# pritykinlab/guidescan-cli

Hardware: AMD Instinct MI355X
Metric: guides/sec off-target enum, <=3 mismatches (higher is better)
Workload: dtype u32

## Files before the change

guidescan-cli_amd/api.py:

```python
from __future__ import annotations

import ctypes as C
import os
import subprocess
from pathlib import Path

import numpy as np

PKG = Path(__file__).resolve().parent
LIB_PATH = Path(os.environ.get("GS_LIB_PATH", str(PKG / "libgsamd.so")))

GS_FLAG_PAM_AT_START = 1
GS_FLAG_FAITHFUL_WALK = 2
GS_FLAG_COUNT_REQUESTS = 4
GS_FLAG_RAW_COUNTS = 8
GS_FLAG_NO_NEW_TABLES = 16


class GsError(RuntimeError):
    def __init__(self, status, msg):
        super().__init__(f"gs_status {status}: {msg}")
        self.status = status


# ... 151 lines not shown
    L.gs_decode_sequence_ex.restype = i32
    L.gs_decode_sequence_ex.argtypes = [vp, C.c_char_p]
    L.gs_enumerate_general.restype = i32
    L.gs_enumerate_general.argtypes = [vp, vp, u64, u32, vp, u32, C.c_char_p, u32, u32, u32, u32, u32,
                                       C.POINTER(vp)]
    L.gs_enumerate_general_pams.restype = i32
    L.gs_enumerate_general_pams.argtypes = [vp, vp, u64, u32, vp, u32, C.c_char_p, vp, u32, u32, u32, u32, u32,
                                            C.POINTER(vp)]
    L.gs_debug_general_last.restype = i32
    L.gs_debug_general_last.argtypes = [vp, C.POINTER(u64)]
    L.gs_debug_bulge_last.restype = i32
    L.gs_debug_bulge_last.argtypes = [vp, C.POINTER(u64)]
    L.gs_debug_bulge_seeds.restype = i32
    L.gs_debug_bulge_seeds.argtypes = [C.c_char_p, u32, u32, u32, u32, u32, u32, u32, u32, vp, u64, C.POINTER(u64)]
    L.gs_debug_bulge_verify.restype = i32
    L.gs_debug_bulge_verify.argtypes = [u32, vp, u64, C.c_char_p, u32, C.c_char_p, u32, C.c_char_p, vp, u32, u32, u32, u32,
                                        u32, u32, vp, u64, C.POINTER(u64)]
    L.gs_index_last_guide_flags.restype = i32
    L.gs_index_last_guide_flags.argtypes = [vp, C.POINTER(vp), C.POINTER(u64)]
    L.gs_format_guide_ex.restype = i32
    L.gs_format_guide_ex.argtypes = [C.POINTER(GsGenomeStructure), C.POINTER(GsKmer), vp, u64, u32, u32,
                                     C.c_int64, C.POINTER(vp), C.POINTER(C.c_size_t)]
    L.gs_score_device.restype = i32
    L.gs_score_device.argtypes = [vp, vp, u64, u32, u32, u32, C.c_int64, C.POINTER(GsGenomeStructure), vp, vp,
                                  vp, vp, vp]
    L.gs_score.restype = i32
    L.gs_score.argtypes = [vp, vp, u64, u32, u32, u32, C.c_int64, C.POINTER(GsGenomeStructure), vp, vp, vp, vp]
    L.gs_format_device.restype = i32
    L.gs_format_device.argtypes = [vp, C.POINTER(GsGenomeStructure), vp, u64, u32, vp, u32, vp, vp, vp, vp, vp, vp, vp, u32, u32,
                                   C.c_int64, vp, C.POINTER(vp), C.POINTER(u64)]
    L.gs_enumerate_text.restype = i32
    L.gs_enumerate_text.argtypes = [vp, vp, u64, u32, vp, u32, C.c_char_p, u32, u32, u32, C.c_int64,
                                    C.POINTER(GsGenomeStructure), vp, vp, vp, vp, C.POINTER(vp), C.POINTER(u64),
                                    C.POINTER(GsResultView)]
    L.gs_index_last_text_offsets.restype = i32
    L.gs_index_last_text_offsets.argtypes = [vp, vp, u64]
    L.gs_kmers_generate.restype = i32
    L.gs_kmers_generate.argtypes = [i32, vp, u64, i32, C.c_char_p, u32, u32, vp, C.POINTER(vp)]
    L.gs_kmers_get.restype = i32
    L.gs_kmers_get.argtypes = [vp, i32, C.POINTER(u64), C.POINTER(vp), C.POINTER(vp), C.POINTER(vp),
                               C.POINTER(vp)]
    L.gs_kmers_free.argtypes = [vp]
    L.gs_format_device_ids.restype = i32
    L.gs_format_device_ids.argtypes = L.gs_format_device.argtypes
    L.gs_enumerate_text_device.restype = i32
    L.gs_enumerate_text_device.argtypes = [vp, vp, u64, u32, vp, u32, C.c_char_p, u32, u32, u32, C.c_int64,
                                           C.POINTER(GsGenomeStructure), vp, vp, vp, vp, C.POINTER(vp), C.POINTER(u64),
                                           C.POINTER(GsResultView), vp]
    L.gs_kmers_encode_ids.restype = i32
    L.gs_kmers_encode_ids.argtypes = [vp, C.c_char_p, C.c_char_p, vp]
    L.gs_kmers_get_ids.restype = i32
    L.gs_kmers_get_ids.argtypes = [vp, i32, C.POINTER(vp), C.POINTER(vp), C.POINTER(vp)]
    L.gs_kmers_csv.restype = i32
    L.gs_kmers_csv.argtypes = [vp, C.c_char_p, C.c_char_p, C.POINTER(vp), C.POINTER(u64)]
    L.gs_kmers_concat.restype = i32
    L.gs_kmers_concat.argtypes = [vp, u32, C.POINTER(vp)]
    L.gs_decoder_open.restype = i32
    L.gs_decoder_open.argtypes = [i32, vp, u64, C.POINTER(GsGenomeStructure), vp, vp, C.POINTER(vp)]
    L.gs_decoder_close.argtypes = [vp]
    L.gs_decode_records.restype = i32
    L.gs_decode_records.argtypes = [vp, C.POINTER(GsDecodeBatch), u32, u64, C.POINTER(vp), C.POINTER(u64), C.POINTER(u64)]
    L.gs_decode_records_device.restype = i32
    L.gs_decode_records_device.argtypes = L.gs_decode_records.argtypes
    L.gs_decode_sam.restype = i32
    L.gs_decode_sam.argtypes = [vp, vp, u64, u32, u64, C.POINTER(vp), C.POINTER(u64), C.POINTER(u64)]
    L.gs_debug_repr_doubles.restype = i32
    L.gs_debug_repr_doubles.argtypes = [vp, u64, vp]
    L.gs_bgzf_compress_device.restype = i32
    L.gs_bgzf_compress_device.argtypes = [vp, vp, u64, vp, C.POINTER(vp), C.POINTER(u64)]
    L.gs_bgzf_compress.restype = i32
    L.gs_bgzf_compress.argtypes = [vp, vp, u64, C.POINTER(vp), C.POINTER(u64)]
    L.gs_bgzf_inflate.restype = i32
    L.gs_bgzf_inflate.argtypes = [i32, vp, u64, C.POINTER(vp), C.POINTER(u64)]
    L.gs_bgzf_inflate_device.restype = i32
    L.gs_bgzf_inflate_device.argtypes = [vp, vp, u64, u64, C.POINTER(vp), C.POINTER(u64), C.POINTER(u64)]
    L.gs_bgzf_inflate_base.restype = i32
    L.gs_bgzf_inflate_base.argtypes = [vp, u64, u64]
    L.gs_debug_inflate_member.restype = i32
    L.gs_debug_inflate_member.argtypes = [vp, u64, vp, u64, C.POINTER(u64), C.POINTER(u32)]
    L.gs_debug_bgzf_members.restype = i32
    L.gs_debug_bgzf_members.argtypes = [vp, u64, vp, vp, u64, C.POINTER(u64), C.POINTER(u32)]
    L.gs_decode_bam.restype = i32
    L.gs_decode_bam.argtypes = [vp, vp, u64, u64, vp, u32, u32, u64, C.POINTER(vp), C.POINTER(u64), C.POINTER(u64), C.POINTER(u64)]
    L.gs_decode_bam_device.restype = i32
    L.gs_decode_bam_device.argtypes = L.gs_decode_bam.argtypes
    L.gs_debug_decode_bam_last.restype = i32
    L.gs_debug_decode_bam_last.argtypes = [vp, vp, vp]
    L.gs_debug_huffman_lengths.restype = i32
    L.gs_debug_huffman_lengths.argtypes = [vp, u32, u32, vp]
    L.gs_debug_sp_float.restype = C.c_float
    L.gs_debug_sp_float.argtypes = [u32]
    L.gs_debug_decode_tables.restype = i32
    L.gs_debug_decode_tables.argtypes = [vp, vp]
    L.gs_fasta_parse.restype = i32
    L.gs_fasta_parse.argtypes = [i32, vp, u64, u32, C.POINTER(vp)]
    L.gs_fasta_parse_file.restype = i32
    L.gs_fasta_parse_file.argtypes = [i32, C.c_char_p, u32, C.POINTER(vp)]
    L.gs_fasta_parse_device.restype = i32
    L.gs_fasta_parse_device.argtypes = [i32, vp, u64, u32, vp, C.POINTER(vp)]
    L.gs_fasta_info.restype = i32
    L.gs_fasta_info.argtypes = [vp, C.POINTER(u64), C.POINTER(u64), C.POINTER(u64)]
    L.gs_fasta_records.restype = i32
    L.gs_fasta_records.argtypes = [vp, vp, vp, vp, vp, vp, vp, vp]
    L.gs_fasta_text.restype = i32
    L.gs_fasta_text.argtypes = [vp, i32, C.POINTER(vp)]
    L.gs_fasta_free.restype = None
    L.gs_fasta_free.argtypes = [vp]
    L.gs_decoder_open_fasta.restype = i32
    L.gs_decoder_open_fasta.argtypes = [i32, vp, C.POINTER(GsGenomeStructure), C.POINTER(vp)]
    L.gs_debug_fasta_tile_bytes.restype = u64
    L.gs_debug_fasta_tile_bytes.argtypes = []
    L.gs_debug_fasta_host.restype = i32
    L.gs_debug_fasta_host.argtypes = [vp, u64, u32, u64, C.POINTER(vp)]
    L.gs_debug_fasta_chunk_bytes.restype = u64
    L.gs_debug_fasta_chunk_bytes.argtypes = [u64]
    L.gs_debug_fasta_ms.restype = i32
    L.gs_debug_fasta_ms.argtypes = [vp, vp]
    L.gs_kmers_parse.restype = i32
    L.gs_kmers_parse.argtypes = [i32, vp, u64, C.POINTER(vp), C.POINTER(GsKmersReport)]
    L.gs_kmers_parse_file.restype = i32
    L.gs_kmers_parse_file.argtypes = [i32, C.c_char_p, C.POINTER(vp), C.POINTER(GsKmersReport)]
    L.gs_kmers_parse_device.restype = i32
    L.gs_kmers_parse_device.argtypes = [i32, vp, u64, vp, C.POINTER(vp), C.POINTER(GsKmersReport)]
    L.gs_debug_kmers_tile_bytes.restype = u64
    L.gs_debug_kmers_tile_bytes.argtypes = []
    L.gs_debug_kmers_chunk_bytes.restype = u64
    L.gs_debug_kmers_chunk_bytes.argtypes = [u64]
    L.gs_debug_kmers_host.restype = i32
    L.gs_debug_kmers_host.argtypes = [vp, u64, u64, C.POINTER(vp), C.POINTER(GsKmersReport)]
    L.gs_status_string.restype = C.c_char_p
    L.gs_status_string.argtypes = [i32]
    L.gs_version.restype = C.c_char_p
    _lib = L
    return L


EXPORTS = ["gs_index_build", "gs_index_build_with_sa", "gs_index_open_sdsl", "gs_index_close",
           "gs_index_genome_length", "gs_index_device_bytes", "gs_enumerate", "gs_enumerate_device",
           "gs_result_get", "gs_result_free", "gs_decode_sequence", "gs_rank_bwt4", "gs_resolve",
           "gs_index_meta", "gs_index_copy_sa", "gs_calculate_cfd", "gs_status_string", "gs_version",
           "gs_format_guide", "gs_format_header", "gs_free", "gs_sdsl_extract_text",
           "gs_enumerate_bulges", "gs_result_ex_get", "gs_result_ex_free", "gs_decode_sequence_ex",
           "gs_format_guide_ex", "gs_score_device", "gs_score", "gs_kmers_generate", "gs_kmers_get",
           "gs_kmers_free", "gs_format_guide_scored", "gs_index_verify_sa", "gs_index_last_counters", "gs_index_last_launch", "gs_enumerate_general",
           "gs_index_last_guide_flags", "gs_enumerate_general_pams", "gs_index_save_sa", "gs_index_open_sa", "gs_format_guides_scored", "gs_result_ex_raw_hits",
           "gs_debug_seed_recipes", "gs_debug_choose_thresholds", "gs_debug_tile_plan", "gs_debug_search_form", "gs_debug_guide_descriptor", "gs_debug_general_last", "gs_index_lock", "gs_index_unlock",
           "gs_index_last_sharing", "gs_index_set_option", "gs_index_get_option", "gs_index_prepare",
           "gs_index_save_sdsl", "gs_debug_sdsl_sections", "gs_debug_sdsl_export_scratch",
           "gs_format_device", "gs_enumerate_text", "gs_index_last_text_offsets",
           "gs_format_device_ids", "gs_enumerate_text_device", "gs_kmers_encode_ids", "gs_kmers_get_ids", "gs_kmers_csv",
           "gs_kmers_concat", "gs_decoder_open", "gs_decoder_close", "gs_decode_records", "gs_decode_records_device",
           "gs_decode_sam", "gs_debug_repr_doubles", "gs_debug_decode_tables",
           "gs_index_last_spaced", "gs_debug_seed_recipes_a8", "gs_debug_spaced_rows",
           "gs_debug_bulge_last", "gs_debug_bulge_seeds", "gs_debug_bulge_verify",
           "gs_bgzf_compress_device", "gs_bgzf_compress", "gs_debug_huffman_lengths", "gs_debug_sp_float",
           "gs_bgzf_inflate", "gs_bgzf_inflate_device", "gs_bgzf_inflate_base", "gs_debug_inflate_member", "gs_debug_bgzf_members",
           "gs_decode_bam", "gs_decode_bam_device", "gs_debug_decode_bam_last",
           "gs_fasta_parse", "gs_fasta_parse_file", "gs_fasta_parse_device", "gs_fasta_info", "gs_fasta_records", "gs_fasta_text",
           "gs_fasta_free", "gs_decoder_open_fasta", "gs_debug_fasta_tile_bytes", "gs_debug_fasta_host",
           "gs_debug_fasta_chunk_bytes", "gs_debug_fasta_ms",
           "gs_kmers_parse", "gs_kmers_parse_file", "gs_kmers_parse_device", "gs_debug_kmers_tile_bytes",
           "gs_debug_kmers_chunk_bytes", "gs_debug_kmers_host"]


def _check(rc):
    if rc != 0:
        raise GsError(rc, lib().gs_status_string(rc).decode())


BULGE_SEED_DTYPE = np.dtype([("index", "<u4"), ("state", "<u4"), ("seq", "S32")])
BULGE_MATCH_DTYPE = np.dtype([("state", "<u4"), ("consumed", "<u4"), ("seq", "S32")])


def bulge_state(word):
    word = int(word)
    return dict(t=word & 63, mismatches=(word >> 6) & 7, dna_bulges=(word >> 9) & 7, rna_bulges=(word >> 12) & 7,
                bulge_state=(word >> 15) & 3, bulge_size=(word >> 17) & 1, seq_len=(word >> 18) & 63)


def bulge_seeds(guide, k, mismatches=0, rna_bulges=0, dna_bulges=0, start=False, prefix_len=0, prefix=0, count_only=False):
    g = guide.encode() if isinstance(guide, str) else bytes(guide)
    flags = GS_FLAG_PAM_AT_START if start else 0
    n = C.c_uint64(0)
    _check(lib().gs_debug_bulge_seeds(g, len(g), k, mismatches, rna_bulges, dna_bulges, flags, prefix_len, prefix, None, 0,
                                      C.byref(n)))
    if count_only:
        return int(n.value)
    out = np.zeros(n.value, dtype=BULGE_SEED_DTYPE)
    _check(lib().gs_debug_bulge_seeds(g, len(g), k, mismatches, rna_bulges, dna_bulges, flags, prefix_len, prefix,
                                      out.ctypes.data, out.size, C.byref(n)))
    assert n.value == out.size
    return out


def bulge_verify(state, seq, ctx_nibbles, guide, pam, k, alt_pams=(), mismatches=0, rna_bulges=0, dna_bulges=0, start=False):
    g = guide.encode() if isinstance(guide, str) else bytes(guide)
    p = pam.encode() if isinstance(pam, str) else bytes(pam)
    sq = np.frombuffer(bytes(seq).ljust(32, b"\0"), dtype=np.uint8).copy()
    alts = "".join(alt_pams).encode()
    lens = np.array([len(a) for a in alt_pams], dtype=np.uint32)
    flags = GS_FLAG_PAM_AT_START if start else 0

    def call(out, cap, n):
        _check(lib().gs_debug_bulge_verify(int(state), sq.ctypes.data, int(ctx_nibbles), g, len(g), p if p else None, len(p),
                                           alts if alt_pams else None, lens.ctypes.data if alt_pams else None,
                                           len(alt_pams), k, mismatches, rna_bulges, dna_bulges, flags, out, cap, C.byref(n)))
    n = C.c_uint64(0)
    call(None, 0, n)
    out = np.zeros(n.value, dtype=BULGE_MATCH_DTYPE)
    call(out.ctypes.data, out.size, n)
    assert n.value == out.size
    return out


def seed_recipes(k, L, P, m, n_x, astar=None, deep=False):
    L_ = lib()
    L_.gs_debug_seed_recipes.restype = C.c_int
    L_.gs_debug_seed_recipes.argtypes = [C.c_uint32] * 5 + [C.c_void_p, C.c_uint32, C.c_void_p, C.c_uint64, C.c_void_p]
    a = None
    if astar is not None:
        a = (C.c_uint32 * 8)(*(list(astar) + [15] * 8)[:8])
    counts = (C.c_uint64 * 3)()
    _check(L_.gs_debug_seed_recipes(k, L, P, m, n_x, a, 1 if deep else 0, None, 0, counts))
    n = sum(counts)
    out = np.zeros(n, dtype=np.uint64)
    _check(L_.gs_debug_seed_recipes(k, L, P, m, n_x, a, 1 if deep else 0, out.ctypes.data, n, counts))
    c0, c1 = int(counts[0]), int(counts[1])
    return out[:c0], out[c0:c0 + c1], out[c0 + c1:]


def seed_recipes_a8(k, m, n_x, astar, trimmed=False):
    L_ = lib()
    L_.gs_debug_seed_recipes_a8.restype = C.c_int
    L_.gs_debug_seed_recipes_a8.argtypes = [C.c_uint32] * 3 + [C.c_void_p, C.c_uint32, C.c_void_p, C.c_uint64, C.c_void_p]
    a = (C.c_uint32 * 8)(*(list(astar) + [15] * 8)[:8])
    n = C.c_uint64()
    _check(L_.gs_debug_seed_recipes_a8(k, m, n_x, a, 1 if trimmed else 0, None, 0, C.byref(n)))
    out = np.zeros(int(n.value), dtype=np.uint64)
    _check(L_.gs_debug_seed_recipes_a8(k, m, n_x, a, 1 if trimmed else 0, out.ctypes.data, out.shape[0], C.byref(n)))
    return out


def guide_descriptor(q: int, pams, L: int, P: int, k: int, x_len: int, codes=(0, 0xFFFFFFFF), n_pt: int = 1, valid: bool = True):
    L_ = lib()
    L_.gs_debug_guide_descriptor.restype = C.c_int
    L_.gs_debug_guide_descriptor.argtypes = [C.c_uint64, C.c_void_p, C.c_uint32, C.c_uint32, C.c_uint32, C.c_uint32, C.c_uint32,
                                             C.c_uint32, C.c_uint32, C.c_void_p, C.c_void_p]
    pam = (C.c_uint32 * 4)(*(list(pams) + [0] * (4 - len(pams))))
    code = (C.c_uint32 * 2)(*codes)
    out = (C.c_uint32 * 16)()
    _check(L_.gs_debug_guide_descriptor(q, pam, len(pams), 1 if valid else 0, L, P, k, x_len, n_pt, code, out))
    names = ("q_lo", "q_hi", "pam0", "pam1", "pam2", "pam3", "meta", "pidx0", "pidxg", "qrem_b", "bsel_z", "bsel_w", "qhot",
             "key_a", "key_b", "guide")
    return dict(zip(names, (int(x) for x in out)))


def choose_thresholds(m, n_x, n_o, n_r, pam_expansions=4.0, verify_a=1.5, verify_b=1.9):
    L_ = lib()
    L_.gs_debug_choose_thresholds.restype = None
    L_.gs_debug_choose_thresholds.argtypes = [C.c_uint32] * 4 + [C.c_double] * 3 + [C.c_void_p]
    out = (C.c_uint32 * 8)()
    L_.gs_debug_choose_thresholds(m, n_x, n_o, n_r, pam_expansions, verify_a, verify_b, out)
    return list(out)


def tile_plan(records):
    L_ = lib()
    L_.gs_debug_tile_plan.restype = None
    L_.gs_debug_tile_plan.argtypes = [C.c_uint32, C.c_void_p]
    out = (C.c_uint32 * 5)()
    L_.gs_debug_tile_plan(records, out)
    return dict(buckets=out[0], slot=out[1], per=out[2], wave_tile=out[3], max_buckets=out[4])


SEARCH_FORM_IN = ("items", "cus", "share_min", "backoff", "main", "walk", "one_chunk", "counting", "spec", "m", "est_heavy",
                  "est_max", "last_hpass", "last_items", "heavy", "split_share", "split_from", "seed_form")


def search_form(**kw):
    L_ = lib()
    L_.gs_debug_search_form.restype = None
    L_.gs_debug_search_form.argtypes = [C.c_void_p, C.c_void_p]
    vals = dict(heavy=-1, split_share=-1, seed_form=-1, split_from=1 << 19)
    vals.update(kw)
    unknown = set(vals) - set(SEARCH_FORM_IN)
    if unknown:
        raise TypeError(f"unknown inputs {sorted(unknown)}")
    inp = (C.c_int64 * len(SEARCH_FORM_IN))(*[int(vals.get(k, 0)) for k in SEARCH_FORM_IN])
    out = (C.c_uint32 * 6)()
    L_.gs_debug_search_form(inp, out)
    return dict(zip(("estimate", "thresh", "heavy", "split", "seed_form", "form"), (int(x) for x in out)))


def make_genome_structure(names, lengths):
    arr_n = (C.c_char_p * len(names))(*[n.encode() for n in names])
    arr_l = (C.c_uint64 * len(lengths))(*lengths)
    g = GsGenomeStructure(arr_n, arr_l, len(names))
    g._keep = (arr_n, arr_l)
    return g


def format_header(gs, sam=False, complete=True) -> str:
    out, n = C.c_void_p(), C.c_size_t()
    flags = (GS_TEXT_SAM if sam else 0) | (GS_TEXT_COMPLETE if complete else 0)
    _check(lib().gs_format_header(C.byref(gs), flags, C.byref(out), C.byref(n)))
    s = C.string_at(out, n.value).decode()
    lib().gs_free(out)
    return s


def format_guide(gs, gid, sequence, pam, sense_positive, hits, mismatches, sam=False, complete=True,
                 start=False, max_off_targets=-1, specificity=None) -> str:
    hits = np.ascontiguousarray(hits, dtype=HIT_DTYPE)
    k = GsKmer(gid.encode(), sequence.encode(), pam.encode(), int(sense_positive))
    out, n = C.c_void_p(), C.c_size_t()
    flags = ((GS_TEXT_SAM if sam else 0) | (GS_TEXT_COMPLETE if complete else 0) |
             (GS_FLAG_PAM_AT_START if start else 0))
    if specificity is None:
        _check(lib().gs_format_guide(C.byref(gs), C.byref(k), hits.ctypes.data, hits.shape[0], mismatches,
                                     flags, max_off_targets, C.byref(out), C.byref(n)))
    else:
        _check(lib().gs_format_guide_scored(C.byref(gs), C.byref(k), hits.ctypes.data, hits.shape[0],
                                            mismatches, flags, max_off_targets, float(specificity),
                                            C.byref(out), C.byref(n)))
    s = C.string_at(out, n.value).decode()
    lib().gs_free(out)
    return s


def format_guides(gs, ids, seqs, pams, senses_positive, offsets, hits, specificity, mismatches, sam=False,
                  complete=True, start=False, max_off_targets=-1, skip=None) -> bytes:
    n = len(ids)
    arr = (GsKmer * n)(*[GsKmer(ids[i].encode(), seqs[i].encode(), pams[i].encode(), int(senses_positive[i]))
                         for i in range(n)])
    offsets = np.ascontiguousarray(offsets, dtype=np.uint64)
    hits = np.ascontiguousarray(hits, dtype=HIT_DTYPE)
    spec = np.ascontiguousarray(specificity, dtype=np.float32)
    sk = None if skip is None else np.ascontiguousarray(skip, dtype=np.uint8)
    out, ln = C.c_void_p(), C.c_size_t()
    flags = ((GS_TEXT_SAM if sam else 0) | (GS_TEXT_COMPLETE if complete else 0) |
             (GS_FLAG_PAM_AT_START if start else 0))
    _check(lib().gs_format_guides_scored(C.byref(gs), arr, n, offsets.ctypes.data,
                                         hits.ctypes.data if hits.shape[0] else None, spec.ctypes.data,
                                         sk.ctypes.data if sk is not None else None, mismatches, flags,
                                         max_off_targets, C.byref(out), C.byref(ln)))
    s = C.string_at(out, ln.value)
    lib().gs_free(out)
    return s


def _id_blob(ids):
    enc = [i.encode() if isinstance(i, str) else bytes(i) for i in ids]
    off = np.zeros(len(enc) + 1, dtype=np.uint64)
    if enc:
        off[1:] = np.cumsum([len(e) for e in enc], dtype=np.uint64)
    return b"".join(enc), off


def _bytes_or_none(x, n):
    if x is None:
        return None
    a = np.ascontiguousarray(np.asarray(x) != 0, dtype=np.uint8)
    if a.shape != (n,):
        raise ValueError("one entry per guide")
    return a


class DeviceKmers:

    def __init__(self, handle, k, P):
        self._h, self.k, self.P = handle, k, P
        n, a, b, c, d = C.c_uint64(), C.c_void_p(), C.c_void_p(), C.c_void_p(), C.c_void_p()
        _check(lib().gs_kmers_get(handle, 1, C.byref(n), C.byref(a), C.byref(b), C.byref(c), C.byref(d)))
        self.n = int(n.value)
        self.seqs_ptr, self.pams_ptr, self.pos_ptr, self.sense_ptr = a.value, b.value, c.value, d.value

    @classmethod
    def parse(cls, src, device=0):
        h, rep = C.c_void_p(), GsKmersReport()
        if isinstance(src, (str, os.PathLike)):
            rc = lib().gs_kmers_parse_file(device, os.fsencode(src), C.byref(h), C.byref(rep))
        else:
            raw = np.frombuffer(src, dtype=np.uint8) if isinstance(src, (bytes, bytearray, memoryview)) else np.ascontiguousarray(src, dtype=np.uint8)
            rc = lib().gs_kmers_parse(device, raw.ctypes.data if raw.size else None, raw.size, C.byref(h), C.byref(rep))
        return cls._parsed(rc, h, rep)

    @classmethod
    def parse_device(cls, d_raw_ptr, length, device=0, stream=None):
        h, rep = C.c_void_p(), GsKmersReport()
        rc = lib().gs_kmers_parse_device(device, d_raw_ptr if length else None, length, stream, C.byref(h), C.byref(rep))
        return cls._parsed(rc, h, rep)

    @classmethod
# ... 872 lines not shown
```

guidescan-cli_amd/csrc/gs_common.h:

```cpp
#ifndef GS_COMMON_H
#define GS_COMMON_H

#include <hip/hip_runtime.h>
#include <stdint.h>
#include <string.h>

#include <array>
#include <atomic>
#include <map>
#include <mutex>
#include <string>
#include <vector>

#include "guidescan_amd.h"

#define ARENA_SHIFT 10u
#define ARENA_CHUNK (1u << ARENA_SHIFT)

#define GS_BLOCK_ROWS 128u
#define GS_BLOCK_SHIFT 7u

#define GS_PT_BIG 63u
struct gs_pairtab_dev {
  const uint2 *tab;
  const uint2 *rot;
  const uint16_t *c16;
  const uint32_t *ctx;
  const uint32_t *rowid;
  uint32_t rot_first;
  uint32_t code;
  const uint4 *deep;
  const uint32_t *sp_off;
  const uint2 *sp_rows;
  uint32_t sp_rem;
};
struct gs_strand_dev {
  const uint4 *blocks;
  const uint32_t *sa;
  const uint32_t *run_start;
  const uint32_t *run_cum;
  uint32_t n;
  uint32_t nruns;
  uint32_t C[4];
  uint32_t CN;
  uint32_t has_n;
  const uint4 *ptab;
  uint32_t mask_off;
  const uint4 *ptab_rot;
  uint32_t rot_first;
  const uint32_t *ctx;
  const uint16_t *ctx16;
  const uint32_t *isa;
  const uint32_t *exc_row;
  const uint64_t *exc_sym;
  uint32_t n_exc;
  const uint32_t *xr_start;
  const uint32_t *xr_cum;
  const uint2 *xr_seg;
  const uint32_t *C256;
};

struct gs_strand {
  gs_strand_dev d{};
  void *blocks = nullptr, *sa = nullptr, *run_start = nullptr, *run_cum = nullptr, *ptab = nullptr, *ctx = nullptr, *ctx16 = nullptr, *ptab_rot = nullptr, *isa = nullptr, *exc_row = nullptr, *exc_sym = nullptr, *xr_start = nullptr, *xr_cum = nullptr, *xr_seg = nullptr, *C256 = nullptr;
  bool has_sym[256] = {false};
  uint32_t rot_plan_first = 31, rot_plan_n = 0, rot_k = 0;
  uint64_t n = 0;
  uint64_t C_acgtn[5] = {0, 0, 0, 0, 0};
  uint64_t bytes = 0;
};

#define GS_NRUN_FLANK 40
struct gs_nrun {
  uint64_t start, len;
  uint8_t left[GS_NRUN_FLANK];
  uint8_t right[GS_NRUN_FLANK];
};

struct gs_buffer {
  void *p = nullptr;
  size_t cap = 0;
};

struct gs_pairtab_host {
  bool valid = false;
  uint32_t v_rem = 0, code = 0, rot_first = 31;
  gs_pairtab_dev d[2]{};
  void *mem[2][8] = {{nullptr}, {nullptr}};
  bool deep = false;
  uint32_t deep_P = 0, deep_kb = 0;
  bool spaced = false;
  uint32_t sp_x = 0, sp_g = 0;
  uint64_t sp_bytes = 0, sp_rows[2] = {0, 0};
  uint64_t n_slots[2] = {0, 0};
  double sp_build_ms = 0;
  uint64_t bytes = 0, used = 0;
};

struct gs_recipe_set {
  gs_buffer buf;
  uint64_t key[2] = {0, 0};
  bool valid = false;
  uint32_t n_full = 0, n_a = 0, n_b = 0, n_a8 = 0;
  uint32_t n_a8s = 0;
  uint32_t a_rot_first = 31;
};

struct gs_index {
  std::map<std::string, std::string> opts;
  mutable std::recursive_mutex mtx;
  int device = 0;
  uint64_t genome_length = 0;
  gs_strand strand[2];
  gs_buffer w_guides, w_slots, w_counts, w_nmatch, w_nhits, w_offsets, w_hits, w_misc, w_blocksums,
      w_grec, w_flags, w_raw, w_ovf_list, w_grec2, w_slots2, w_counts2, w_nmatch2, w_nhits2, w_h_off, w_h_tmp,
      w_b_src, w_b_cnt, w_b_prefix, w_b_recs, w_b_w0, w_b_w0b, w_b_idx, w_b_idxb, w_b_keep, w_b_keeps,
      w_b_rows, w_b_rowss, w_b_redo_pos, w_b_s, w_b_tab,
      w_score, w_score_io, w_score_tmp,
      w_arena, w_arena_meta, w_nchunk,
      w_shq, w_sh_meta,
      w_cls, w_desc, w_sched,
      w_t_plan, w_t_tiles, w_t_buckets, w_t_chunkof, w_t_big, w_t_rel, w_t_tab, w_t_excl, w_t_spill, w_b_redo_pos2,
      w_text_in, w_text_tmp, w_text_hex, w_text, w_text_spec, w_text_goff ,
      w_bgzf_in, w_bgzf_tmp, w_bgzf_out;
  uint32_t share_backoff = 0;
  bool share_timed_out = false;
  uint32_t opt_share_min = 512, opt_share_max = 2048;
  unsigned long long last_share[8] = {0, 0, 0, 0, 0, 0, 0, 0};
  uint64_t shq_packages = 16384;
  uint64_t arena_chunks = 4096;
  struct seen_t {
    double mean = -1, max = 0;
    uint64_t hpass = 0, items = 0;
    uint64_t key = 0;
  };
  std::array<seen_t, 8> seen;
  bool last_raw_valid = false;
  uint64_t last_unsupported = 0;
  hipEvent_t ev[4] = {nullptr, nullptr, nullptr, nullptr};
  hipEvent_t ev_tile = nullptr;
  hipStream_t st_help = nullptr;
  hipEvent_t ev_help[2] = {nullptr, nullptr};
  uint32_t *h_pin = nullptr;
  std::atomic<uint64_t> lock_owner{0};
  uint32_t lock_depth = 0;
  uint32_t pt_k = 0;
  unsigned long long last_counters[16] = {0};
  unsigned long long last_launch[8] = {0, 0, 0, 0, 0, 0, 0, 0};
  unsigned long long last_general[8] = {0, 0, 0, 0, 0, 0, 0, 0};
  unsigned long long last_bulge[8] = {0, 0, 0, 0, 0, 0, 0, 0};
  std::vector<gs_nrun> nruns_text;
  gs_buffer w_cand;
  uint64_t cand_key = ~0ull;
  uint32_t cand_n[2] = {0, 0};
  size_t cand_bidx[2] = {0, 0};
  gs_recipe_set rec[2];
  uint32_t rec_cur = 0;
  uint32_t pairtab_nofit = 0;
  gs_pairtab_host pairtab[2];
  bool pairtab_off = false;
  bool spaced_off = false;
  unsigned long long last_spaced[4] = {0, 0, 0, 0};
  bool rot_off = false;
  uint32_t dbg_nomem = 0;
  bool tile_order_off = false;
  uint64_t tile_order_off_key = 0;
  uint64_t tx_n = 0;
  bool big_long_runs = false;
};

gs_status gs_pairtab_ensure(gs_index *ix, uint32_t slot, uint32_t v_rem, uint32_t code, uint32_t rot_first, double share,
                            hipStream_t st);
gs_status gs_pairtab_ensure_deep(gs_index *ix, uint32_t slot, uint32_t P, uint32_t kb, hipStream_t st);
void gs_pairtab_free(gs_index *ix, uint32_t slot);
gs_status gs_pairtab_ensure_spaced(gs_index *ix, uint32_t slot, uint32_t x_len, uint32_t g, hipStream_t st);
bool gs_pairtab_free_spaced(gs_index *ix, uint32_t slot);
gs_status gs_strand_rot_ensure(gs_index *ix, hipStream_t st);
bool gs_strand_rot_release(gs_index *ix);

struct gs_tileorder_in {
  uint32_t n_set;
  const uint32_t *list;
  const uint32_t *redo_pos;
  const uint32_t *counts;
  const uint32_t *cls;
  const uint4 *slots;
  uint32_t cap;
  const uint4 *arena;
  const uint32_t *chunk_item, *chunk_seq;
  uint32_t n_used;
  uint32_t *nhits;
  const uint64_t *offsets;
  gs_hit *hits;
  uint32_t L, P, m, v_rem;
};
struct gs_tileorder_state {
  uint32_t n_it = 0, n_tiles = 0, n_btiles = 0, n_chunks = 0, n_big = 0, n_deal = 0;
  uint32_t spill_units = 0, spill_cap = 0;
  uint32_t n_excl = 0;
  uint64_t n_records = 0;
};
bool gs_tileorder_fits(uint32_t L, uint32_t P, uint32_t m);
gs_status gs_tileorder_plan(gs_index *ix, const gs_tileorder_in &in, hipStream_t st, gs_tileorder_state &S, bool *usable);
gs_status gs_tileorder_run(gs_index *ix, const gs_tileorder_in &in, gs_tileorder_state &S, hipStream_t st, uint32_t *violations);

#define GS_HANDLE_LOCK(ix)                               \
  std::unique_lock<std::recursive_mutex> handle_lock__; \
  if (ix) handle_lock__ = std::unique_lock<std::recursive_mutex>((ix)->mtx)

#define GS_HIP(expr)                                                              \
  do {                                                                            \
    hipError_t e__ = (expr);                                                      \
    if (e__ != hipSuccess) {                                                      \
      gs_set_error(std::string(#expr) + ": " + hipGetErrorString(e__));           \
      return GS_ERR_DEVICE;                                                       \
    }                                                                             \
  } while (0)

void gs_set_error(const std::string &s);
const char *gs_opt(const gs_index *ix, const char *key);
void gs_opts_from_env(gs_index *ix);
extern std::atomic<int> gs_debug_any;
gs_status gs_reserve(gs_buffer &b, size_t bytes);
gs_status gs_text_to_host(const void *d_text, uint64_t tl, char **text);
size_t gs_buffer_free(gs_buffer &b);

gs_status gs_device_suffix_array(const uint8_t *d_text, uint64_t n, uint32_t *d_sa, hipStream_t st);
gs_status gs_strand_from_device(const uint8_t *d_text, uint32_t *d_sa_owned, uint64_t n,
                                gs_strand *out, hipStream_t st);
void gs_strand_free(gs_strand *s);
gs_status gs_count_bad_sa_rows(const uint32_t *d_sa, uint64_t n, hipStream_t st, uint64_t *bad);

gs_status gs_sdsl_read(const char *path, std::vector<uint8_t> &bwt, std::vector<uint64_t> &sa_samples,
                       uint64_t C256[257]);

gs_status gs_device_suffix_array_discarding(const uint8_t *d_text, uint64_t n, uint32_t *d_sa, hipStream_t st, bool debug);

static inline __host__ __device__ uint32_t gs_lane_group(uint32_t n_guides) {
  uint32_t g = 64;
  while (g > 1 && (n_guides + g - 1) / g < 8192u) g >>= 1;
  return g;
}

#endif
```

guidescan-cli_amd/csrc/gs_enumerate.hip:

```cpp
#include "gs_kernels.h"

__global__ void k_estimate_heavy(const gs_guide_rec *guides, uint32_t n, const uint4 *ptab0, const uint4 *ptab1, uint32_t k,
                                 uint32_t thresh, uint32_t *out);

#include <cmath>

static uint64_t shape_key(uint32_t L, uint32_t P, uint32_t n_alt, uint32_t flags) {
  return ((uint64_t)L << 32) | ((uint64_t)P << 16) | (n_alt << 8) | (flags & GS_FLAG_PAM_AT_START);
}

struct switches {
  bool debug, no_form_estimate, no_bidir, no_pairtab, no_deep, no_spec, no_cand_buckets, no_tile_order, no_arena;
  bool dbg_share_timeout;
  uint32_t share_min, share_max;
  uint32_t max_pt;
  bool has_deep_symbols;
  uint32_t deep_symbols;
  uint32_t n_astar, astar[8];
  double pairtab_reserve;
  bool has_index_budget;
  double index_budget;
  uint32_t cand_from;
  bool has_arena_chunks;
  uint64_t arena_chunks;
// ... 601 lines not shown
}

struct search_pass {
  const gs_guide_rec *guides;
  uint32_t ng;
  uint4 *slots;
  uint32_t *counts;
  uint32_t cap;
  const uint64_t *slot_off;
  bool with_arena;
};
static void fill_search_args(const batch &b, const search_pass &p, gs_search_args &sa) {
  const gs_index *ix = b.ix;
  memset(&sa, 0, sizeof(sa));
  sa.sd[0] = ix->strand[0].d;
  sa.sd[1] = ix->strand[1].d;
  sa.slots = p.slots;
  sa.slot_off = p.slot_off;
  sa.counts = p.counts;
  sa.work = b.d_work;
  sa.stats = b.d_stats;
  sa.n_items = 2 * p.ng;
  sa.L = b.L;
  sa.P = b.P;
  sa.m = b.m;
  sa.cap = p.cap;
  if (p.with_arena) {
    sa.arena = (uint4 *)ix->w_arena.p;
    sa.arena_next = b.d_work + WK_ARENA_NEXT;
    sa.chunk_item = (uint32_t *)ix->w_arena_meta.p;
    sa.chunk_seq = sa.chunk_item + b.arena_chunks;
    sa.nchunk = (uint2 *)ix->w_nchunk.p;
    sa.cls = (uint32_t *)ix->w_cls.p;
    sa.arena_chunks = b.arena_chunks;
    sa.chunk_fill = sa.chunk_item + 2 * (size_t)b.arena_chunks;
  }
  const uint64_t waves = (uint64_t)b.cus * 32u;
  uint64_t take = (2ull * p.ng) / (waves * 64u);
  take = take < 1 ? 1 : take > 4 ? 4 : take;
  if (b.sw.search_take) take = b.sw.search_take;
  sa.take = (uint32_t)take;
  sa.max_iter = b.sw.max_iter;
  sa.err = b.d_work + WK_SEARCH_ERR;
  sa.hpass = b.d_work + WK_HPASS;
  sa.v_max = b.sw.v_max;
  sa.dbg_skip = b.sw.dbg_skip;
  sa.cnt_shift = b.sw.cnt_shift;
  sa.astar = 0xFFFFFFFFu;
  if (b.table_seeding) {
    sa.pt_k = ix->pt_k;
    sa.v_rem = b.v_rem;
    sa.x_len = b.x_len;
    sa.bdeep = b.deep ? 1u : 0u;
    const gs_recipe_set &R = ix->rec[ix->rec_cur];
    sa.rec_full = (const uint2 *)R.buf.p;
    sa.n_rec_full = R.n_full;
    if (b.bidir) {
      sa.bidir = 1;
      sa.astar = b.astar_packed;
      sa.rec_a = sa.rec_full + R.n_full;
      sa.n_rec_a = R.n_a;
      sa.rec_b = sa.rec_a + R.n_a;
      sa.n_rec_b = R.n_b;
      sa.rec_a8 = sa.rec_b + R.n_b;
      sa.n_rec_a8 = R.n_a8;
      sa.n_pt = b.n_pt;
      for (uint32_t i = 0; i < b.n_pt; i++) {
        sa.pt[i][0] = ix->pairtab[b.pt_slot[i]].d[0];
        sa.pt[i][1] = ix->pairtab[b.pt_slot[i]].d[1];
      }
      for (uint32_t s = 0; s < 2; s++) {
        sa.cand[s] = b.d_cand[s];
        sa.n_cand[s] = b.n_cand[s];
        sa.cand_off[s] = b.d_cand_off[s];
        sa.cand_ids[s] = b.d_cand_ids[s];
      }
    }
  }
  if (sa.dbg_skip & 4u) sa.n_rec_full = sa.n_rec_a = sa.n_rec_b = sa.n_rec_a8 = 0u;
}

static void launch_helpers(const gs_search_args &sh, uint32_t sh_grid, bool spec, hipStream_t hs) {
  if (spec)
    hipLaunchKernelGGL(k_search_heavy_pd, dim3(sh_grid), dim3(WAVE * SEARCH_WAVES), 0, hs, sh);
  else
    hipLaunchKernelGGL(k_search_heavy, dim3(sh_grid), dim3(WAVE * SEARCH_WAVES), 0, hs, sh);
}
static bool helper_stream(gs_index *ix) {
  if (ix->st_help) return true;
  int lo = 0, hi = 0;
  hipStream_t hs = nullptr;
  bool ok = hipDeviceGetStreamPriorityRange(&lo, &hi) == hipSuccess && hipStreamCreateWithPriority(&hs, hipStreamNonBlocking, lo) == hipSuccess;
  for (hipEvent_t &e : ix->ev_help) ok = ok && hipEventCreateWithFlags(&e, hipEventDisableTiming) == hipSuccess;
  if (ok) {
    ix->st_help = hs;
    return true;
  }
  (void)hipGetLastError();
  if (hs) (void)hipStreamDestroy(hs);
  for (hipEvent_t &e : ix->ev_help) {
    if (e) (void)hipEventDestroy(e);
    e = nullptr;
  }
  return false;
}
struct search_launch {
  bool walk, spec;
  uint32_t grid, seed_grid, heavy_per_cu;
  form_out f;
  gs_search_args sh_args;
  uint32_t sh_grid = 0;
};
static gs_status launch_search(batch &b, const search_pass &p, gs_search_args &sa, search_launch &k) {
  gs_index *ix = b.ix;
  hipStream_t st = b.st;
  const dim3 blk(WAVE * SEARCH_WAVES);
  for (uint32_t c = 0; c < b.n_chunks; c++) {
    sa.guides = p.guides + (size_t)c * p.ng;
    sa.append = c ? 1u : 0u;
    if (c) GS_HIP(hipMemsetAsync(b.d_work + WK_ITEMS, 0, 4, st));
    if (k.walk)
      hipLaunchKernelGGL(k_search_walk, dim3(k.grid), blk, 0, st, sa);
    else if (k.spec && b.count_req && !k.f.seed_form)
      hipLaunchKernelGGL(k_search_count_pd, dim3(k.grid), blk, 0, st, sa);
    else if (k.f.split && sa.shq != nullptr) {
      k.sh_args = sa;
      k.sh_args.helper_only = 1u;
      k.sh_args.work = b.d_work + WK_HELPER_ITEMS;
      k.sh_grid = (uint32_t)b.cus * k.heavy_per_cu;
      const bool side = k.f.split == 2u && helper_stream(ix);
      if (side) {
        GS_HIP(hipEventRecord(ix->ev_help[0], st));
        GS_HIP(hipStreamWaitEvent(ix->st_help, ix->ev_help[0], 0));
      }
      if (k.f.split == 3u) launch_helpers(k.sh_args, k.sh_grid, k.spec, st);
      if (k.spec)
        hipLaunchKernelGGL(k_search_pub_pd, dim3(k.grid), blk, 0, st, sa);
      else
        hipLaunchKernelGGL(k_search_pub, dim3(k.grid), blk, 0, st, sa);
      if (k.f.split != 3u) launch_helpers(k.sh_args, k.sh_grid, k.spec, side ? ix->st_help : st);
      if (side) {
        GS_HIP(hipEventRecord(ix->ev_help[1], ix->st_help));
        GS_HIP(hipStreamWaitEvent(st, ix->ev_help[1], 0));
      }
    } else if (k.spec && sa.shq != nullptr)
      hipLaunchKernelGGL(k_search_heavy_pd, dim3(k.grid), blk, 0, st, sa);
    else if (sa.shq != nullptr)
      hipLaunchKernelGGL(k_search_heavy, dim3(k.grid), blk, 0, st, sa);
    else if (k.f.seed_form) {
      gs_search_args sb;
      gs_status r2 = gs_seed_describe(ix, sa, p.ng, k.f.seed_form >= 2u && p.ng >= b.sw.seed_sort_from, st, &sb);
      sb.seed_opt = b.sw.seed_opt;
      sb.take = b.sw.seed_take;
      if (r2 == GS_OK) r2 = gs_seed_launch(sb, k.seed_grid, b.count_req, st);
      if (r2 != GS_OK) return r2;
    } else if (k.spec)
      hipLaunchKernelGGL(k_search_fast_pd, dim3(k.grid), blk, 0, st, sa);
    else if (b.count_req)
      hipLaunchKernelGGL(k_search_count, dim3(k.grid), blk, 0, st, sa);
    else
      hipLaunchKernelGGL(k_search_fast, dim3(k.grid), blk, 0, st, sa);
  }
  return GS_OK;
}
static gs_status share_fix(batch &b, const search_pass &p, const gs_search_args &sa, gs_misc_readback &rb) {
  gs_index *ix = b.ix;
  hipStream_t st = b.st;
  gs_share_args fa;
  memset(&fa, 0, sizeof(fa));
  fa.ctl = sa.shq_ctl;
  fa.sh_list = sa.sh_list;
  fa.sh_acc = sa.sh_acc;
  fa.counts = p.counts;
  fa.nchunk = sa.nchunk;
  fa.cls = sa.cls;
  fa.chunk_item = sa.chunk_item;
  fa.chunk_seq = sa.chunk_seq;
  fa.chunk_fill = sa.chunk_fill;
  fa.arena_next = b.d_work + WK_ARENA_NEXT;
  fa.slots = p.slots;
  fa.arena = sa.arena;
  fa.dbase = sa.sh_acc + 16 * (size_t)sa.sh_max;
  fa.dir = sa.chunk_item + 3 * (size_t)b.arena_chunks;
  fa.stats = b.d_stats;
  fa.sh_max = sa.sh_max;
  fa.cap = p.cap;
  fa.arena_chunks = b.arena_chunks;
  const uint32_t n_sh = (uint32_t)ix->last_share[0];
  hipLaunchKernelGGL(k_share_scan, dim3(1), dim3(1024), 0, st, fa);
  hipLaunchKernelGGL(k_share_dir, dim3((b.arena_chunks + 255) / 256), dim3(256), 0, st, fa);
  hipLaunchKernelGGL((k_share_fix<SH_SMALLSEG>), dim3(n_sh), dim3(256), 0, st, fa);
  hipLaunchKernelGGL((k_share_fix<SH_MAXSEG>), dim3(std::min<uint32_t>(n_sh, (uint32_t)b.cus * 3u)), dim3(256), 0, st, fa);
  GS_HIP(hipEventRecord(ix->ev[2], st));
  GS_HIP(hipMemcpyAsync(&rb, b.d_stats, sizeof(rb), hipMemcpyDeviceToHost, st));
  GS_HIP(hipStreamSynchronize(st));
  GS_HIP(hipGetLastError());
  return GS_OK;
}
static gs_status reserve_share_queue(batch &b, const search_pass &p, gs_search_args &sa, uint32_t grid) {
  gs_index *ix = b.ix;
  uint64_t qcap = b.sw.share_queue ? b.sw.share_queue : ix->shq_packages;
  if (qcap > (1ull << 20)) qcap = 1ull << 20;
  const uint32_t sh_max = std::min<uint32_t>(2 * p.ng, 1u << 18);
  const size_t meta = 512 + 4 * (size_t)qcap + 4 * (size_t)sh_max + 64 * (size_t)sh_max;
  if (gs_reserve(ix->w_shq, 16 * (size_t)SHQ_PKG * qcap) != GS_OK || gs_reserve(ix->w_sh_meta, meta + 4 * ((size_t)sh_max + 2)) != GS_OK) {
    (void)hipGetLastError();
    return GS_OK;
  }
  uint32_t *d_shctl = (uint32_t *)ix->w_sh_meta.p;
  sa.shq = (uint4 *)ix->w_shq.p;
  sa.shq_ctl = d_shctl;
  sa.shq_ready = d_shctl + 128;
  sa.sh_list = sa.shq_ready + qcap;
  sa.sh_acc = sa.sh_list + sh_max;
  sa.shq_cap = (uint32_t)qcap;
  sa.sh_max = sh_max;
  sa.share_min = b.sw.share_min;
  sa.share_max = std::max(128u, b.sw.share_max);
  sa.n_waves = grid * SEARCH_WAVES;
  sa.sh_prof = b.sw.debug ? 1u : 0u;
  GS_HIP(hipMemsetAsync(d_shctl, 0, meta, b.st));
  if (sa.sh_prof) GS_HIP(hipMemsetAsync(d_shctl + 104, 0xFF, 8, b.st));
  return GS_OK;
}
static gs_status pick_form(batch &b, const search_pass &p, bool walk, bool spec, form_out &f) {
  gs_index *ix = b.ix;
  const gs_index::seen_t &seen = ix->seen[b.m < 8 ? b.m : 0];
  const bool seen_last = b.m < 8 && seen.key == shape_key(b.L, b.P, b.n_alt, b.flags) && seen.hpass != 0;
  form_in fi;
  fi.items = 2 * p.ng;
  fi.cus = (uint32_t)b.cus;
  fi.share_min = b.sw.share_min;
  fi.backoff = ix->share_backoff;
  fi.main = p.with_arena;
  fi.walk = walk;
  fi.one_chunk = b.n_chunks == 1;
  fi.counting = b.count_req;
  fi.spec = spec;
  fi.m = b.m;
  fi.est[0] = fi.est[1] = 0;
  fi.last_hpass = seen_last ? seen.hpass : 0;
  fi.last_items = seen_last ? seen.items : 0;
  fi.heavy = b.sw.heavy;
  fi.split_share = b.sw.split_share;
  fi.seed_form = b.sw.seed_form;
  fi.split_from = b.sw.split_from;
  if (p.with_arena && ix->share_backoff != 0) ix->share_backoff--;
  f = choose_form(fi);
  if (f.want_estimate && !b.sw.no_form_estimate) {
    if (b.pre_est_ran && p.with_arena) {
      fi.est[0] = b.pre_est[0];
      fi.est[1] = b.pre_est[1];
    } else {
      const gs_status er = gs_estimate_heavy(ix, p.guides, p.ng, f.est_thresh, b.d_work + WK_SCRATCH2, b.st, fi.est);
      if (er != GS_OK) return er;
    }
    if (b.sw.debug) fprintf(stderr, "[gs] form estimate: %u guides with a heavy k-mer of their own, the largest interval %u rows\n", fi.est[0], fi.est[1]);
    f = choose_form(fi);
  }
  ix->last_share[7] = fi.est[0];
  return GS_OK;
}
static gs_status run_search(batch &b, const search_pass &p, unsigned long long h_stats[2]) {
  gs_index *ix = b.ix;
  hipStream_t st = b.st;
  GS_HIP(hipMemsetAsync(ix->w_misc.p, 0, 16, st));
  GS_HIP(hipMemsetAsync(b.d_stats + ST_ARENA_FAIL, 0, 8, st));
  GS_HIP(hipMemsetAsync(b.d_work + WK_ITEMS, 0, 4, st));
  GS_HIP(hipMemsetAsync(b.d_work + WK_SEARCH_ERR, 0, 4, st));
  GS_HIP(hipMemsetAsync(b.d_work + WK_HPASS, 0, 4, st));
  GS_HIP(hipMemsetAsync(b.d_work + WK_HELPER_ITEMS, 0x80, 4, st));
  if (p.with_arena) {
    GS_HIP(hipMemsetAsync(b.d_work + WK_ARENA_NEXT, 0, 4, st));
    GS_HIP(hipMemsetAsync((uint32_t *)ix->w_arena_meta.p + b.arena_chunks, 0xFF, 4 * (size_t)b.arena_chunks, st));
    GS_HIP(hipMemsetAsync(ix->w_arena_meta.p, 0, 4 * (size_t)b.arena_chunks, st));
    for (int i = 0; i < 7; i++) ix->last_share[i] = 0;
  }
  gs_search_args sa;
  fill_search_args(b, p, sa);
  search_launch k;
  k.walk = sa.pt_k == 0 || sa.v_rem == 0;
  const size_t lds_wg = sizeof(uint4) * (k.walk ? WAVE_LDS_ENTRIES : WAVE_LDS_FAST) * SEARCH_WAVES;
  uint32_t per_cu = (uint32_t)(160u * 1024u / lds_wg);
  k.spec = !k.walk && sa.bidir && sa.bdeep && b.n_pt != 0 && b.n_pt == b.n_codes && b.h_pairs[16] == 0 && !b.sw.no_spec;
  sa.share_min = b.sw.share_min ? b.sw.share_min : 0xFFFFFFFFu;
  gs_status rc;
  if ((rc = pick_form(b, p, k.walk, k.spec, k.f)) != GS_OK) return rc;
  const bool sharing = k.f.heavy || k.f.split;
  const uint32_t weu = k.walk ? GS_WAVES_EU : k.f.heavy ? GS_WAVES_EU_HEAVY : k.spec ? GS_WAVES_EU_PD : GS_WAVES_EU_FAST;
  if (per_cu > weu) per_cu = weu;
  k.heavy_per_cu = std::min<uint32_t>((uint32_t)(160u * 1024u / lds_wg), GS_WAVES_EU_HEAVY);
  if (sharing) {
    int occ = 0;
    hipError_t oe = k.spec ? hipOccupancyMaxActiveBlocksPerMultiprocessor(&occ, k_search_heavy_pd, WAVE * SEARCH_WAVES, 0)
                           : hipOccupancyMaxActiveBlocksPerMultiprocessor(&occ, k_search_heavy, WAVE * SEARCH_WAVES, 0);
    if (oe != hipSuccess) (void)hipGetLastError();
    if (oe == hipSuccess && occ > 0 && (uint32_t)occ < k.heavy_per_cu) k.heavy_per_cu = (uint32_t)occ;
    if (k.f.heavy && per_cu > k.heavy_per_cu) per_cu = k.heavy_per_cu;
  }
  k.grid = (uint32_t)b.cus * per_cu;
  const uint32_t need = (2 * p.ng + SEARCH_WAVES - 1) / SEARCH_WAVES;
  if (k.grid > need) k.grid = need;
  if (b.sw.debug) {
    int occ = 0;
    (void)hipOccupancyMaxActiveBlocksPerMultiprocessor(&occ, k.walk ? k_search_walk : k_search_fast, WAVE * SEARCH_WAVES, 0);
    fprintf(stderr, "[gs] k_search (%s): grid %u x %u threads, LDS %zu B per workgroup, %d workgroups per CU resident\n",
            k.walk ? "walk" : "table", k.grid, WAVE * SEARCH_WAVES, lds_wg, occ);
  }
  if (sharing && (rc = reserve_share_queue(b, p, sa, k.grid)) != GS_OK) return rc;
  const uint32_t *d_shctl = sa.shq_ctl;
  k.seed_grid = 0;
  if (k.f.seed_form) {
    const size_t lds_seed = sizeof(uint4) * (VQ_CAP + 32 + 24 + 6) * SEARCH_WAVES;
    k.seed_grid = (uint32_t)b.cus * std::min<uint32_t>((uint32_t)(160u * 1024u / lds_seed), GS_WAVES_EU_SEED);
    if (k.seed_grid > need) k.seed_grid = need;
  }
  if (p.with_arena) ix->last_share[6] = sharing && d_shctl == nullptr ? 0u : k.f.form;
  if (p.with_arena) {
    const bool seed_launches = k.f.seed_form != 0u && !k.walk && sa.shq == nullptr;
    const unsigned long long ll[8] = {k.walk ? 1u : 0u, k.spec ? 1u : 0u, sa.bdeep, sa.take, seed_launches ? b.sw.seed_take : 0u, sa.n_pt, sa.x_len,
                                      ix->strand[0].ptab_rot ? ix->strand[0].rot_plan_n : 0u};
    memcpy(ix->last_launch, ll, sizeof(ll));
  }
  bool spaced = b.spaced_wanted && k.f.seed_form != 0u && !k.walk && sa.shq == nullptr;
  if (spaced) {
    const bool frozen = (b.flags & GS_FLAG_NO_NEW_TABLES) != 0;
    for (uint32_t i = 0; i < b.n_pt; i++) {
      if (!frozen && !ix->spaced_off && (rc = gs_pairtab_ensure_spaced(ix, b.pt_slot[i], b.x_len, b.L - ix->pt_k, st)) != GS_OK) return rc;
      const gs_pairtab_host &pt = ix->pairtab[b.pt_slot[i]];
      spaced = spaced && pt.spaced && pt.sp_x == b.x_len && pt.sp_g == b.L - ix->pt_k;
      sa.pt[i][0] = pt.d[0];
      sa.pt[i][1] = pt.d[1];
    }
  }
  if (spaced) {
    const gs_recipe_set &R = ix->rec[ix->rec_cur];
    sa.spaced = 1u;
    sa.spaced_ctr = b.d_work + WK_SPACED;
    sa.rec_a8 = sa.rec_a8 + R.n_a8;
    sa.n_rec_a8 = (sa.dbg_skip & 4u) ? 0u : R.n_a8s;
  }
  GS_HIP(hipEventRecord(ix->ev[1], st));
  if ((rc = launch_search(b, p, sa, k)) != GS_OK) return rc;
  GS_HIP(hipEventRecord(ix->ev[2], st));
  gs_misc_readback rb;
  uint32_t h_ctl[128] = {0};
  GS_HIP(hipMemcpyAsync(&rb, b.d_stats, sizeof(rb), hipMemcpyDeviceToHost, st));
  if (d_shctl) GS_HIP(hipMemcpyAsync(h_ctl, d_shctl, sizeof(h_ctl), hipMemcpyDeviceToHost, st));
  GS_HIP(hipStreamSynchronize(st));
  GS_HIP(hipGetLastError());
  if (d_shctl && k.f.split && k.sh_grid != 0u && h_ctl[32] < std::min(h_ctl[0], sa.shq_cap) && rb.work[WK_SEARCH_ERR] == 0u) {
    launch_helpers(k.sh_args, k.sh_grid, k.spec, st);
    GS_HIP(hipEventRecord(ix->ev[2], st));
    GS_HIP(hipMemcpyAsync(&rb, b.d_stats, sizeof(rb), hipMemcpyDeviceToHost, st));
    GS_HIP(hipMemcpyAsync(h_ctl, d_shctl, sizeof(h_ctl), hipMemcpyDeviceToHost, st));
    GS_HIP(hipStreamSynchronize(st));
    GS_HIP(hipGetLastError());
    ix->last_share[5]++;
  }
  if (d_shctl && sa.sh_prof) {
    const unsigned long long *pr = (const unsigned long long *)(h_ctl + 104);
    const double us = 0.01, nw = (double)sa.n_waves;
    fprintf(stderr, "[gs] heavy launch: %u waves; the last wave left its items after %.0f us, the last exit after %.0f us; per wave: items %.0f us, "
            "helper episodes %.0f us (%.1f episodes), waiting for a package %.0f us; shared items %u, packages %u (queue %u)\n",
            sa.n_waves, us * (double)(pr[1] - pr[0]), us * (double)(pr[2] - pr[0]), us * (double)pr[3] / nw, us * (double)pr[4] / nw,
            (double)pr[6] / nw, us * (double)pr[5] / nw, h_ctl[96], h_ctl[0], sa.shq_cap);
  }
  if (d_shctl) {
    ix->last_share[0] = std::min(h_ctl[96], sa.sh_max);
    ix->last_share[1] = h_ctl[0];
    ix->last_share[2] = sa.shq_cap;
    ix->last_share[3] = h_ctl[32];
    if (!b.sw.share_queue && (uint64_t)h_ctl[0] + h_ctl[0] / 4 + 64 > ix->shq_packages) ix->shq_packages = (uint64_t)h_ctl[0] + h_ctl[0] / 4 + 64;
    if (h_ctl[96] != 0u && rb.work[WK_SEARCH_ERR] == 0u && (rc = share_fix(b, p, sa, rb)) != GS_OK) return rc;
  }
  h_stats[0] = rb.stats[0];
  h_stats[1] = rb.stats[1];
  if (p.with_arena) b.arena_fail = rb.stats[ST_ARENA_FAIL];
  if (p.with_arena) b.arena_raw = rb.work[WK_ARENA_NEXT];
  if (p.with_arena && b.m < 8) {
    ix->seen[b.m].hpass = rb.work[WK_HPASS];
    ix->seen[b.m].items = 2 * (uint64_t)p.ng;
  }
  if (sa.shq != nullptr && b.sw.dbg_share_timeout) rb.work[WK_SEARCH_ERR] |= 2u;
  if (rb.work[WK_SEARCH_ERR] != 0u) {
    if ((rb.work[WK_SEARCH_ERR] & 2u) != 0u && sa.shq != nullptr) {
      ix->share_timed_out = true;
      gs_set_error("internal: a wave gave up waiting for a shared verification pass (the launch was not resident as a whole)");
      return GS_ERR_DEVICE;
    }
    gs_set_error("internal: an item of the search passed its iteration bound (GS_SEARCH_MAX_ITER)");
    return GS_ERR_DEVICE;
  }
  float ms = 0.f;
  hipEventElapsedTime(&ms, ix->ev[1], ix->ev[2]);
  b.ms_search += ms;
  return GS_OK;
}

static gs_status run_order(const batch &b, uint4 *slots, const uint32_t *counts, uint32_t *nmatch, uint32_t *nhits, uint32_t ng,
                           uint32_t cap_, uint32_t max_item) {
  gs_order_args oa;
  oa.slots = slots;
  oa.counts = counts;
  oa.nmatch = nmatch;
  oa.nhits = nhits;
  oa.stats = b.d_stats;
  oa.n = ng;
  oa.cap = cap_;
  if (cap_ > 128) {
    uint32_t nmax = 256;
    while (nmax < 2u * max_item && nmax < 2u * cap_) nmax <<= 1;
    const size_t lds = sizeof(uint4) * (size_t)nmax;
    if (lds > 64 * 1024)
      GS_HIP(hipFuncSetAttribute((const void *)k_order_wg, hipFuncAttributeMaxDynamicSharedMemorySize, (int)lds));
    uint32_t grid = ng;
    const uint32_t gmax = (uint32_t)b.cus * (uint32_t)(lds > 80 * 1024 ? 1 : lds > 40 * 1024 ? 3 : 6);
    if (grid > gmax) grid = gmax;
    if (grid == 0) grid = 1;
    hipLaunchKernelGGL(k_order_wg, dim3(grid), dim3(256), lds, b.st, oa, nmax);
    return GS_OK;
  }
  const uint32_t ow = ORDER_WAVES;
  const size_t lds = sizeof(uint4) * (2 * (size_t)cap_ + ORDER_SMALL) * ow;
  const uint32_t gsz = gs_lane_group(ng);
  uint32_t grid = ((ng + gsz - 1) / gsz + ow - 1) / ow;
  const uint32_t gmax = (uint32_t)b.cus * 16u;
  if (grid > gmax) grid = gmax;
  if (grid == 0) grid = 1;
  hipLaunchKernelGGL(k_order, dim3(grid), dim3(WAVE * ow), lds, b.st, oa);
  return GS_OK;
}
static void run_locate(const batch &b, const uint4 *matches, const uint32_t *nmatch, const uint32_t *gmap, uint32_t ng, uint32_t cap_) {
  const gs_index *ix = b.ix;
  gs_locate_args la;
  la.sd[0] = ix->strand[0].d;
  la.sd[1] = ix->strand[1].d;
  la.matches = matches;
  la.nmatch = nmatch;
  la.offsets = (const uint64_t *)ix->w_offsets.p;
  la.gmap = gmap;
  la.hits = (gs_hit *)ix->w_hits.p;
  la.genome_length = ix->genome_length;
  la.n = ng;
  la.cap = cap_;
  la.v_rem = b.v_rem;
  const size_t lds = sizeof(uint32_t) * (2 * (size_t)cap_ + 1);
  const uint32_t gsz = gs_lane_group(ng);
  hipLaunchKernelGGL(k_locate, dim3((ng + gsz - 1) / gsz), dim3(WAVE), lds, b.st, la);
}

static gs_status main_pass(batch &b) {
  gs_index *ix = b.ix;
  hipStream_t st = b.st;
  gs_status rc;
  if ((rc = gs_reserve(ix->w_slots, sizeof(uint4) * (size_t)b.cap * 2 * b.n)) != GS_OK) return rc;
  const search_pass p = {(const gs_guide_rec *)ix->w_grec.p, b.n32, (uint4 *)ix->w_slots.p, (uint32_t *)ix->w_counts.p, b.cap,
                         nullptr, b.arena_chunks != 0};
  if ((rc = run_search(b, p, b.h_stats)) != GS_OK) return rc;
  if (b.arena_chunks == 0 || b.arena_fail == 0 || b.sw.has_arena_chunks || b.n_chunks != 1) return GS_OK;
  uint32_t *d_need = b.d_work + WK_SCRATCH2, h_need = 0;
  GS_HIP(hipMemsetAsync(d_need, 0, 4, st));
  hipLaunchKernelGGL(k_need_chunks, dim3(std::min<uint32_t>((2 * b.n32 + 255) / 256, 1024u)), dim3(256), 0, st,
                     (const uint32_t *)ix->w_counts.p, 2 * b.n32, b.cap, d_need);
  GS_HIP(hipMemcpyAsync(&h_need, d_need, 4, hipMemcpyDeviceToHost, st));
  GS_HIP(hipStreamSynchronize(st));
// ... 605 lines not shown
```

guidescan-cli_amd/csrc/gs_index.hip:

```cpp
#include "gs_common.h"
#include "gs_scratch.h"

#include <rocprim/rocprim.hpp>

#include <algorithm>
#include <functional>
#include <system_error>
#include <thread>
#include <cstdlib>
#include <cstring>

__device__ __forceinline__ uint32_t sym_class(uint8_t c) {
  switch (c) {
    case 'A': return 0;
    case 'C': return 1;
    case 'G': return 2;
    case 'T': return 3;
    case 'N': return 4;
    default: return 5;
  }
}
__device__ __forceinline__ uint8_t bwt_at(const uint8_t *text, const uint32_t *sa, uint64_t n,
                                          uint64_t row) {
  const uint32_t s = sa[row];
// ... 720 lines not shown
extern "C" gs_status gs_index_build(const uint8_t *text, uint64_t len, int device, gs_index **out) {
  try {
    return build_common(text, len, nullptr, nullptr, device, out);
  } catch (const std::bad_alloc &) {
    return GS_ERR_NOMEM;
  }
}
gs_status gs_build_from_device_sa(const uint8_t *text, uint64_t len, const uint32_t *d_sa_fwd, const uint32_t *d_sa_rev, int device, gs_index **out) {
  if (!d_sa_fwd || !d_sa_rev) return GS_ERR_ARG;
  try {
    return build_common(text, len, d_sa_fwd, d_sa_rev, device, out, GS_ERR_FORMAT, true);
  } catch (const std::bad_alloc &) {
    return GS_ERR_NOMEM;
  }
}
extern "C" gs_status gs_index_build_with_sa(const uint8_t *text, uint64_t len, const uint32_t *sa_fwd,
                                            const uint32_t *sa_rev, int device, gs_index **out) {
  if (!sa_fwd || !sa_rev) return GS_ERR_ARG;
  try {
    return build_common(text, len, sa_fwd, sa_rev, device, out);
  } catch (const std::bad_alloc &) {
    return GS_ERR_NOMEM;
  }
}

struct gs_sa_header {
  char magic[8];
  uint64_t n;
  uint64_t text_hash;
  uint64_t sa_hash[2];
  uint64_t reserved[3];
};
static uint64_t sa_hash_update(uint64_t h, const uint32_t *p, size_t m) {
  size_t i = 0;
  for (; i + 2 <= m; i += 2) {
    uint64_t w;
    memcpy(&w, p + i, 8);
    h = (h ^ w) * 0xFF51AFD7ED558CCDull;
    h ^= h >> 32;
  }
  if (i < m) h = (h ^ p[i]) * 1099511628211ull;
  return h;
}
static uint64_t text_fingerprint(const uint8_t *text, uint64_t len) {
  uint64_t h = 0x9E3779B97F4A7C15ull ^ len;
  uint64_t i = 0;
  for (; i + 8 <= len; i += 8) {
    uint64_t w;
    memcpy(&w, text + i, 8);
    h = (h ^ w) * 0xFF51AFD7ED558CCDull;
    h ^= h >> 32;
  }
  for (; i < len; i++) h = (h ^ text[i]) * 1099511628211ull;
  return h;
}
extern "C" gs_status gs_index_save_sa(gs_index *ix, const uint8_t *text, uint64_t len, const char *path) {
  GS_HANDLE_LOCK(ix);
  if (!ix || !text || !path || len != ix->genome_length) return GS_ERR_ARG;
  GS_HIP(hipSetDevice(ix->device));
  FILE *f = fopen(path, "wb");
  if (!f) {
    gs_set_error(std::string("cannot write ") + path);
    return GS_ERR_IO;
  }
  gs_sa_header h;
  memset(&h, 0, sizeof(h));
  memcpy(h.magic, "GSAMDSA2", 8);
  h.n = ix->strand[0].n;
  h.text_hash = text_fingerprint(text, len);
  h.sa_hash[0] = h.sa_hash[1] = 0x9E3779B97F4A7C15ull;
  bool ok = fwrite(&h, sizeof(h), 1, f) == 1;
  const size_t chunk = 64u << 20;
  std::vector<uint32_t> buf;
  try {
    buf.resize(chunk);
  } catch (const std::bad_alloc &) {
    fclose(f);
    return GS_ERR_NOMEM;
  }
  for (int s = 0; s < 2 && ok; s++)
    for (uint64_t at = 0; at < h.n && ok; at += chunk) {
      const size_t m = (size_t)std::min<uint64_t>(chunk, h.n - at);
      if (hipMemcpy(buf.data(), (const uint32_t *)ix->strand[s].sa + at, 4 * m, hipMemcpyDeviceToHost) != hipSuccess) {
        fclose(f);
        gs_set_error("copying the suffix array back failed");
        return GS_ERR_DEVICE;
      }
      ok = fwrite(buf.data(), 4, m, f) == m;
      h.sa_hash[s] = sa_hash_update(h.sa_hash[s], buf.data(), m);
    }
  ok = ok && fseek(f, 0, SEEK_SET) == 0 && fwrite(&h, sizeof(h), 1, f) == 1;
  ok = fclose(f) == 0 && ok;
  if (!ok) {
    gs_set_error(std::string("short write to ") + path);
    return GS_ERR_IO;
  }
  return GS_OK;
}
extern "C" gs_status gs_index_open_sa(const uint8_t *text, uint64_t len, const char *path, int device,
                                      gs_index **out) {
  if (!text || !path || !out || len < 1) return GS_ERR_ARG;
  FILE *f = fopen(path, "rb");
  if (!f) {
    gs_set_error(std::string("cannot read ") + path);
    return GS_ERR_IO;
  }
  gs_sa_header h;
  const uint64_t n = len + 1;
  bool ok = fread(&h, sizeof(h), 1, f) == 1 && (!memcmp(h.magic, "GSAMDSA2", 8) || !memcmp(h.magic, "GSAMDSA1", 8)) &&
            h.n == n && h.text_hash == text_fingerprint(text, len);
  const bool summed = ok && h.magic[7] == '2';
  std::vector<uint32_t> sa[2];
  try {
    for (int s = 0; s < 2 && ok; s++) {
      sa[s].resize(n);
      ok = fread(sa[s].data(), 4, n, f) == n;
    }
  } catch (const std::bad_alloc &) {
    fclose(f);
    return GS_ERR_NOMEM;
  }
  fclose(f);
  if (ok && summed) {
    uint64_t got[2] = {0, 0};
    auto sum = [&](int s) { got[s] = sa_hash_update(0x9E3779B97F4A7C15ull, sa[s].data(), (size_t)n); };
    try {
      std::thread t1(sum, 1);
      sum(0);
      t1.join();
    } catch (const std::system_error &) {
      sum(0);
      sum(1);
    }
    ok = got[0] == h.sa_hash[0] && got[1] == h.sa_hash[1];
  }
  if (!ok) {
    gs_set_error(std::string(path) + " is not the suffix-array file of this genome text (or is damaged)");
    return GS_ERR_FORMAT;
  }
  return build_common(text, len, sa[0].data(), sa[1].data(), device, out, GS_ERR_FORMAT);
}

extern "C" void gs_index_close(gs_index *ix) {
  if (!ix) return;
  hipSetDevice(ix->device);
  gs_strand_free(&ix->strand[0]);
  gs_strand_free(&ix->strand[1]);
  gs_buffer *bufs[] = {&ix->w_guides, &ix->w_slots, &ix->w_counts, &ix->w_nmatch, &ix->w_nhits,
                       &ix->w_offsets, &ix->w_hits, &ix->w_misc, &ix->w_blocksums, &ix->w_grec, &ix->w_flags, &ix->w_raw,
                       &ix->w_ovf_list, &ix->w_grec2, &ix->w_slots2, &ix->w_counts2, &ix->w_nmatch2,
                       &ix->w_nhits2, &ix->w_h_off, &ix->w_h_tmp, &ix->w_b_src, &ix->w_b_cnt, &ix->w_b_prefix,
                       &ix->w_b_recs, &ix->w_b_w0, &ix->w_b_w0b, &ix->w_b_idx, &ix->w_b_idxb,
                       &ix->w_b_keep, &ix->w_b_keeps, &ix->w_b_rows, &ix->w_b_rowss, &ix->w_b_redo_pos, &ix->w_b_s, &ix->w_b_tab,
                       &ix->w_cand, &ix->rec[0].buf, &ix->rec[1].buf, &ix->w_score, &ix->w_score_io, &ix->w_score_tmp, &ix->w_arena, &ix->w_arena_meta, &ix->w_nchunk, &ix->w_shq, &ix->w_sh_meta,
                       &ix->w_cls, &ix->w_desc, &ix->w_sched, &ix->w_t_plan, &ix->w_t_tiles, &ix->w_t_buckets, &ix->w_t_chunkof, &ix->w_t_big, &ix->w_t_rel, &ix->w_t_tab, &ix->w_t_excl, &ix->w_t_spill, &ix->w_b_redo_pos2,
                       &ix->w_text_in, &ix->w_text_tmp, &ix->w_text_hex, &ix->w_text, &ix->w_text_spec, &ix->w_text_goff,
                       &ix->w_bgzf_in, &ix->w_bgzf_tmp, &ix->w_bgzf_out};
  for (gs_buffer *b : bufs) gs_buffer_free(*b);
  for (int i = 0; i < 4; i++)
    if (ix->ev[i]) hipEventDestroy(ix->ev[i]);
  if (ix->ev_tile) hipEventDestroy(ix->ev_tile);
  for (hipEvent_t e : ix->ev_help)
    if (e) hipEventDestroy(e);
  if (ix->st_help) hipStreamDestroy(ix->st_help);
  if (ix->h_pin) hipHostFree(ix->h_pin);
  gs_pairtab_free(ix, 0);
  gs_pairtab_free(ix, 1);
  delete ix;
}
static uint64_t this_thread_tag() { return (uint64_t)std::hash<std::thread::id>()(std::this_thread::get_id()) | 1ull; }
extern "C" gs_status gs_index_lock(gs_index *ix) {
  if (!ix) return GS_ERR_ARG;
  ix->mtx.lock();
  ix->lock_owner.store(this_thread_tag());
  ix->lock_depth++;
  return GS_OK;
}
extern "C" gs_status gs_index_unlock(gs_index *ix) {
  if (!ix) return GS_ERR_ARG;
  if (ix->lock_owner.load() != this_thread_tag() || ix->lock_depth == 0) return GS_ERR_ARG;
  if (--ix->lock_depth == 0) ix->lock_owner.store(0);
  ix->mtx.unlock();
  return GS_OK;
}
extern "C" gs_status gs_index_last_guide_flags(const gs_index *ix, const void **d_flags, uint64_t *n_unsupported) {
  GS_HANDLE_LOCK(ix);
  if (!ix) return GS_ERR_ARG;
  if (d_flags) *d_flags = ix->w_flags.p;
  if (n_unsupported) *n_unsupported = ix->last_unsupported;
  return GS_OK;
}
extern "C" gs_status gs_index_last_counters(const gs_index *ix, uint64_t out[16]) {
  GS_HANDLE_LOCK(ix);
  if (!ix || !out) return GS_ERR_ARG;
  for (int i = 0; i < 16; i++) out[i] = ix->last_counters[i];
  return GS_OK;
}
extern "C" gs_status gs_index_last_launch(const gs_index *ix, uint64_t out[8]) {
  GS_HANDLE_LOCK(ix);
  if (!ix || !out) return GS_ERR_ARG;
  for (int i = 0; i < 8; i++) out[i] = ix->last_launch[i];
  return GS_OK;
}
extern "C" gs_status gs_index_last_spaced(const gs_index *ix, uint64_t out[6]) {
  GS_HANDLE_LOCK(ix);
  if (!ix || !out) return GS_ERR_ARG;
  for (int i = 0; i < 4; i++) out[i] = ix->last_spaced[i];
  out[4] = ix->pairtab[0].sp_bytes + ix->pairtab[1].sp_bytes;
  out[5] = (uint64_t)(1e3 * (ix->pairtab[0].sp_build_ms + ix->pairtab[1].sp_build_ms));
  return GS_OK;
}
extern "C" uint64_t gs_index_genome_length(const gs_index *ix) { return ix ? ix->genome_length : 0; }
extern "C" uint64_t gs_index_device_bytes(const gs_index *ix) {
  return ix ? ix->strand[0].bytes + ix->strand[1].bytes + ix->pairtab[0].bytes + ix->pairtab[1].bytes : 0;
}
extern "C" gs_status gs_index_meta(const gs_index *ix, int strand, uint64_t C_acgtn[5],
                                   uint64_t *size) {
  if (!ix || strand < 0 || strand > 1) return GS_ERR_ARG;
  if (C_acgtn)
    for (int k = 0; k < 5; k++) C_acgtn[k] = ix->strand[strand].C_acgtn[k];
  if (size) *size = ix->strand[strand].n;
  return GS_OK;
}
extern "C" gs_status gs_index_copy_sa(gs_index *ix, int strand, uint32_t *out) {
  GS_HANDLE_LOCK(ix);
  if (!ix || strand < 0 || strand > 1 || !out) return GS_ERR_ARG;
  GS_HIP(hipSetDevice(ix->device));
  GS_HIP(hipMemcpy(out, ix->strand[strand].sa, 4 * ix->strand[strand].n, hipMemcpyDeviceToHost));
  return GS_OK;
}

gs_status gs_reserve(gs_buffer &b, size_t bytes) {
  if (b.cap >= bytes && b.p) return GS_OK;
  if (bytes > ((size_t)1 << 30) && gs_debug_any.load(std::memory_order_relaxed))
    fprintf(stderr, "[gs] workspace buffer grows from %.2f to %.2f GiB\n", (double)b.cap / (1 << 30), (double)bytes / (1 << 30));
  const bool again = b.p != nullptr && b.cap > ((size_t)1 << 30);
  if (b.p) hipFree(b.p);
  b.p = nullptr;
  b.cap = 0;
  size_t want = bytes + (bytes > ((size_t)1 << 30) ? (again ? bytes / 8 : bytes / 16) : bytes / 4) + 256;
  if (hipMalloc(&b.p, want) != hipSuccess) {
    (void)hipGetLastError();
    if (hipMalloc(&b.p, bytes) != hipSuccess) {
      (void)hipGetLastError();
      b.p = nullptr;
      gs_set_error("out of device memory");
      return GS_ERR_NOMEM;
    }
    want = bytes;
  }
  b.cap = want;
  return GS_OK;
}
size_t gs_buffer_free(gs_buffer &b) {
  const size_t freed = b.p ? b.cap : 0;
  if (b.p) (void)hipFree(b.p);
  b.p = nullptr;
  b.cap = 0;
  return freed;
}
```

guidescan-cli_amd/csrc/gs_kernels.h:

```cpp
#pragma once
#include "gs_device.h"

#define SEARCH_WAVES 4
#ifndef STACK_ENTRIES
#define STACK_ENTRIES 224
#endif
#ifndef VQ_CAP
#define VQ_CAP 128
#endif
#ifndef VQ_DRAIN
#define VQ_DRAIN 64
#endif
#define WAVE_LDS_FAST (VQ_CAP + 32 + DTAB + 5)
#define WAVE_LDS_ENTRIES (STACK_ENTRIES + WAVE_LDS_FAST)
#define MAX_FANOUT 5

#define META_T(m) ((uint32_t)((m) >> 59))
#define META_K(m) ((uint32_t)(((m) >> 56) & 7))
#define META_FAN(m) ((uint32_t)(((m) >> 54) & 1))
#define META_PAM(m) ((uint32_t)(((m) >> 52) & 3))
#define PATH_MASK ((1ull << 52) - 1)

enum : uint32_t {
  ST_MATCHES = 2,
  ST_ARENA_FAIL = 6,
  ST_COUNT_SUM = 14,
  WK_ITEMS = 0,
  WK_INVALID = 1,
  WK_NLIST = 2,
  WK_BIG_ERR = 3,
  WK_ARENA_NEXT = 4,
  WK_SEARCH_ERR = 5,
  WK_BIG_SCRATCH = 6,
  WK_HPASS = 8,
  WK_HELPER_ITEMS = 9,
  WK_SCRATCH2 = 10,
  WK_SPACED = 12,
  MISC_PAIR_HIST = 256,
};
static inline unsigned long long *gs_misc_stats(void *misc) { return (unsigned long long *)misc; }
static inline uint32_t *gs_misc_work(void *misc) { return (uint32_t *)((char *)misc + 128); }
struct gs_misc_readback {
  unsigned long long stats[16];
  uint32_t work[16];
};


struct gs_search_args {
  gs_strand_dev sd[2];
  const gs_guide_rec *guides;
  uint4 *slots;
  const uint64_t *slot_off;
  uint32_t *counts;
  uint4 *arena;
  uint32_t *arena_next;
  uint32_t *chunk_item, *chunk_seq;
  uint2 *nchunk;
  uint32_t arena_chunks;
  uint32_t *cls;
  uint32_t max_iter;
  uint32_t *err;
  uint32_t *work;
  uint32_t take;
  unsigned long long *stats;
  uint32_t n_items, L, P, m, cap;
  const uint2 *rec_full, *rec_a, *rec_b;
  uint32_t n_rec_full, n_rec_a, n_rec_b;
  const uint2 *rec_a8;
  uint32_t n_rec_a8;
  gs_pairtab_dev pt[2][2];
  uint32_t n_pt;
  uint32_t bdeep, x_len;
  uint32_t pt_k;
  uint32_t v_rem;
  uint32_t v_max;
  uint32_t dbg_skip;
  uint32_t cnt_shift;
  uint32_t append;
  uint32_t bidir, astar;
  const uint4 *cand[2];
  uint32_t n_cand[2];
  const uint32_t *cand_off[2], *cand_ids[2];
  uint4 *shq;
  uint32_t *shq_ctl;
  uint32_t *shq_ready;
  uint32_t *sh_list;
  uint32_t *sh_acc;
  uint32_t *chunk_fill;
  uint32_t shq_cap, sh_max, share_min, share_max, n_waves;
  uint32_t *hpass;
  uint32_t sh_prof;
  uint32_t helper_only;
  const struct gs_guide_desc *desc_a, *desc_b;
  uint32_t *xwork;
  uint32_t seed_opt;
  uint32_t spaced;
  uint32_t *spaced_ctr;
};
struct gs_guide_desc {
  uint32_t q_lo, q_hi;
  uint32_t pam[4];
  uint32_t meta;
  uint32_t pidx0;
  uint32_t pidxg;
  uint32_t qrem_b;
  uint32_t bsel_z, bsel_w;
  uint32_t qhot;
  uint32_t key_a, key_b;
  uint32_t guide;
};
struct gs_describe_args {
  const gs_guide_rec *guides;
  gs_guide_desc *desc;
  uint32_t *hist;
  uint32_t n, L, P, k, x_len, n_pt;
  uint32_t code[2];
  const uint4 *cand[2];
  const uint32_t *cand_off[2], *cand_ids[2];
  uint32_t n_cand[2];
  uint32_t m;
};
#define SHQ_PKG 72u
#define SH_NONE 0xFFFFFFFFu
#define SH_HELPER_SEQ 0x40000000u
typedef uint32_t __attribute__((address_space(1))) gs_gu32;
typedef unsigned long long __attribute__((address_space(1))) gs_gu64;
__device__ __forceinline__ uint32_t ld_agent(const uint32_t *p) {
  return __hip_atomic_load((const gs_gu32 *)p, __ATOMIC_RELAXED, __HIP_MEMORY_SCOPE_AGENT);
}
__device__ __forceinline__ void st_agent(uint32_t *p, uint32_t v) {
  __hip_atomic_store((gs_gu32 *)p, v, __ATOMIC_RELAXED, __HIP_MEMORY_SCOPE_AGENT);
}
__device__ __forceinline__ void st16_agent(uint4 *p, const uint4 v) {
  __hip_atomic_store((gs_gu64 *)p, ((unsigned long long)v.y << 32) | v.x, __ATOMIC_RELAXED, __HIP_MEMORY_SCOPE_AGENT);
  __hip_atomic_store((gs_gu64 *)p + 1, ((unsigned long long)v.w << 32) | v.z, __ATOMIC_RELAXED, __HIP_MEMORY_SCOPE_AGENT);
}
__device__ __forceinline__ uint4 ld16_agent(const uint4 *p) {
  const unsigned long long lo = __hip_atomic_load((const gs_gu64 *)p, __ATOMIC_RELAXED, __HIP_MEMORY_SCOPE_AGENT);
  const unsigned long long hi = __hip_atomic_load((const gs_gu64 *)p + 1, __ATOMIC_RELAXED, __HIP_MEMORY_SCOPE_AGENT);
  return make_uint4((uint32_t)lo, (uint32_t)(lo >> 32), (uint32_t)hi, (uint32_t)(hi >> 32));
}
#define DSC_LO 27u
#define DSC_EXC 30u

#define VERIFY_MAX_DEFAULT 1023u
#define DTAB 88u

#ifndef GS_VU
#define GS_VU 4u
#endif
#define SEED_LOW_MAX 128


#ifndef GS_WAVES_EU
#define GS_WAVES_EU 5
#endif
#ifndef GS_WAVES_EU_FAST
#define GS_WAVES_EU_FAST 8
#endif
#ifndef GS_WAVES_EU_PD
#define GS_WAVES_EU_PD 8
#endif
#ifndef GS_WAVES_EU_HEAVY
#define GS_WAVES_EU_HEAVY 8
#endif
#ifndef GS_WAVES_EU_SEED
#define GS_WAVES_EU_SEED 8
#endif

struct gs_order_args {
  uint4 *slots;
  const uint32_t *counts;
  uint32_t *nmatch;
  uint32_t *nhits;
  unsigned long long *stats;
  uint32_t n, cap;
};
#define ORDER_WAVES 4
#define ORDER_SMALL 128u
#define SCAN_BLOCK 1024
struct gs_locate_args {
  gs_strand_dev sd[2];
  const uint4 *matches;
  const uint32_t *nmatch;
  const uint64_t *offsets;
  const uint32_t *gmap;
  gs_hit *hits;
  uint64_t genome_length;
  uint32_t n, cap;
  uint32_t v_rem;
};
struct gs_agather_args {
  const uint4 *slots, *arena;
  const uint32_t *counts;
  const uint32_t *chunk_item, *chunk_seq;
  const uint32_t *list;
  const uint32_t *redo_pos;
  const uint64_t *dst_off;
  uint4 *dst;
  uint32_t n_o, cap, cap2, n_used;
};
struct gs_share_args {
  const uint32_t *ctl;
  const uint32_t *sh_list;
  const uint32_t *sh_acc;
  uint32_t *counts;
  uint2 *nchunk;
  uint32_t *cls;
  const uint32_t *chunk_item;
  uint32_t *chunk_seq;
  const uint32_t *chunk_fill;
  const uint32_t *arena_next;
  uint4 *slots, *arena;
  uint32_t *dbase;
  uint32_t *dir;
  unsigned long long *stats;
  uint32_t sh_max, cap, arena_chunks;
};
#define SH_MAXSEG 4096u
#define SH_SMALLSEG 254u
__global__ void k_order(gs_order_args a);
__global__ void k_order_wg(gs_order_args a, uint32_t nmax);
__global__ void k_scan_partial(const uint32_t *in, uint64_t *blocksum,
                                                             uint32_t n);
__global__ void k_scan_blocksums(uint64_t *blocksum, uint32_t nb);
__global__ void k_scan_final(const uint32_t *in, const uint64_t *blocksum,
                                                           uint64_t *out, uint32_t n, uint32_t nb);
__global__ void k_locate(gs_locate_args a);
__global__ void k_rank4(gs_strand_dev sd, const uint64_t *rows, uint64_t n, uint64_t *out);
__global__ void k_resolve(gs_strand_dev sd, const uint64_t *rows, uint64_t n, uint64_t *out);
__global__ void k_collect_overflow(const uint32_t *counts, uint32_t n, uint32_t cap, uint32_t *list,
                                   uint32_t *n_list);
__global__ void k_gather_guides(const gs_guide_rec *in, const uint32_t *list, uint32_t n_o,
                                gs_guide_rec *out);
__global__ void k_gather_counts(const uint32_t *counts, const uint32_t *list, uint32_t n_o, uint32_t *out);
__global__ void k_patch_overflow(const uint32_t *list, uint32_t n_o, const uint32_t *nhits2,
                                 uint32_t *nhits);
__global__ void k_arena_gather(gs_agather_args a);
__global__ void k_share_scan(gs_share_args a);
__global__ void k_share_dir(gs_share_args a);
template <uint32_t MAXSEG>
__global__ void k_share_fix(gs_share_args a);
__global__ void k_raw_counts(const uint4 *slots, const uint32_t *counts, uint32_t n, uint32_t cap,
                                                    uint32_t *raw);
__global__ void k_count_stats(const uint32_t *counts, uint32_t n_items, unsigned long long *out);
__global__ void k_need_chunks(const uint32_t *counts, uint32_t n_items, uint32_t cap, uint32_t *out);

struct gs_big_src {
  uint64_t off;
  uint32_t alt;
};
struct gs_big2_tab {
  unsigned long long n[32][8];
  unsigned long long base[16];
};
struct gs_big2_compact_args {
  const uint4 *slots_main, *slots_alt;
  const gs_big_src *src;
  const uint4 *arena;
  const uint32_t *chunk_item, *chunk_seq, *counts;
  const uint32_t *list, *redo_pos;
  uint32_t cap, n_used, from_arena;
  const unsigned long long *prefix;
  const gs_big2_tab *tab;
  uint4 *recs;
  unsigned long long *W;
  uint32_t *rowkey, *idx;
  unsigned long long pam_mul;
  uint32_t n_items, L, P, rbits;
  uint32_t row_bits;
  uint32_t row_off;
};
struct gs_blocate3_args {
  gs_strand_dev sd[2];
  const uint4 *S2;
  const unsigned long long *W;
  const uint32_t *keep;
  const unsigned long long *row_scan;
  const unsigned long long *prefix;
  const uint32_t *gmap;
  const uint64_t *offsets;
  gs_hit *hits;
  uint64_t genome_length, T;
  uint32_t v_rem, gshift;
};
__global__ void k_big_totals(const unsigned long long *prefix, const uint32_t *keep_scan,
                             const unsigned long long *row_scan, uint32_t n_set, uint32_t *nmatch,
                             uint32_t *nhits, uint32_t *err);
__global__ void k_big2_compact(gs_big2_compact_args a);
__global__ void k_big2_counts(const uint32_t *counts, const uint32_t *list, uint32_t n_items, unsigned long long *cnt64);
__global__ void k_big2_gather(const uint4 *recs, const uint32_t *idx, uint64_t T, uint4 *out);
__global__ void k_big2_gather_w(const unsigned long long *W, const uint32_t *idx, uint64_t T, unsigned long long *out);
__global__ void k_big2_runs(const unsigned long long *W, const uint32_t *idx_in, const uint4 *recs,
                                                   uint64_t T, uint32_t short_max, uint32_t *idx_out, uint32_t *long_run);
__global__ void k_max_u64(const unsigned long long *v, uint32_t n, unsigned long long *out);
__global__ void k_big2_comp(const unsigned long long *W, const uint32_t *rowkey, uint64_t T, uint32_t row_bits,
                            uint32_t row_off, unsigned long long *Wc);
__global__ void k_big2_wraps(const uint4 *S2, const unsigned long long *Wc, uint64_t T, uint32_t row_bits, uint32_t *list,
                             uint32_t *n_list);
__global__ void k_big2_fixruns(uint4 *S2, uint4 *tmp, const unsigned long long *Wc, uint64_t T,
                                                      uint32_t row_bits, uint32_t row_off, const uint32_t *list, uint32_t n,
                                                      uint32_t *claimed);
__global__ void k_iota_u32(uint32_t *p, uint64_t n);
__global__ void k_big2_flags(const uint4 *S2, const unsigned long long *W, uint64_t T, uint32_t *keep,
                             unsigned long long *rows, uint32_t wshift);
__global__ void k_big2_locate(gs_blocate3_args a);
__global__ void k_big_sources(const uint32_t *counts_main, const uint32_t *redo_pos, const uint64_t *slot_off2,
                              const uint32_t *counts2, uint32_t n_items, uint32_t cap, gs_big_src *src,
                              unsigned long long *cnt64);
__global__ void k_fill_u32(uint32_t *p, uint32_t v, uint32_t n);
__global__ void k_mark_redo(const uint32_t *list, uint32_t n_o, uint32_t *redo_pos);

struct gs_bigorder_in {
  uint32_t n_set;
  const uint32_t *counts_main, *redo_pos, *counts2;
  uint32_t cap_main;
  const uint64_t *slot_off2;
  bool from_arena;
  const uint32_t *arena_list, *arena_redo_pos;
  uint32_t n_used, arena_chunks, cap;
  uint32_t *nmatch, *nhits;
  uint32_t L, P, m;
};
struct gs_bigorder_out {
  uint64_t T = 0;
  void *s2 = nullptr;
  const unsigned long long *wfinal = nullptr;
  uint32_t gshift = 0;
  bool comp = false;
  uint32_t fixed = 0;
};
bool gs_bigorder_fits(uint32_t L, uint32_t P, uint32_t m, uint32_t n_set);
gs_status gs_bigorder_run(gs_index *ix, const gs_bigorder_in &in, hipStream_t st, gs_bigorder_out &out);
void gs_bigorder_locate(gs_index *ix, const gs_bigorder_out &o, const uint32_t *gmap, uint32_t v_rem, hipStream_t st);
gs_status gs_add_matches(gs_index *ix, unsigned long long add);

__global__ void k_search_walk(gs_search_args a);
__global__ void k_search_fast(gs_search_args a);
__global__ void k_search_count(gs_search_args a);
__global__ void k_search_fast_pd(gs_search_args a);
__global__ void k_search_count_pd(gs_search_args a);
__global__ void k_search_heavy(gs_search_args a);
__global__ void k_search_heavy_pd(gs_search_args a);
__global__ void k_search_pub(gs_search_args a);
__global__ void k_search_pub_pd(gs_search_args a);
__global__ void k_prepare(gs_prep_args a);

__global__ void k_seed_b(gs_search_args a);
__global__ void k_seed_a(gs_search_args a);
__global__ void k_seed_count_b(gs_search_args a);
__global__ void k_seed_count_a(gs_search_args a);
gs_status gs_seed_describe(gs_index *ix, const gs_search_args &sa, uint32_t ng, bool sorted, hipStream_t st, gs_search_args *out);
gs_status gs_seed_launch(const gs_search_args &sa, uint32_t grid, bool count_req, hipStream_t st);
gs_status gs_estimate_heavy(gs_index *ix, const gs_guide_rec *guides, uint32_t n, uint32_t thresh, uint32_t *d_out, hipStream_t st,
                            uint32_t n_heavy[2]);

void gs_choose_astar(uint32_t m, uint32_t nX, uint32_t nO, uint32_t nR, double epam, uint32_t astar[8], double verify_a = 1.5,
                     double verify_b = 1.9);
gs_status gs_recipes_for(gs_index *ix, uint32_t L, uint32_t P, uint32_t m, uint32_t v_rem, const uint32_t *astar, bool deep,
                         hipStream_t st);
```

guidescan-cli_amd/csrc/gs_recipes.hip:

```cpp
#include "gs_kernels.h"

#include <algorithm>
#include <cmath>
#include <vector>

void gs_choose_astar(uint32_t m, uint32_t nX, uint32_t nO, uint32_t nR, double epam, uint32_t astar[8], double verify_a,
                     double verify_b) {
  auto binom3 = [](uint32_t n, uint32_t j) -> double {
    if (j > n) return 0.0;
    double v = 1;
    for (uint32_t i = 0; i < j; i++) v = v * (n - i) / (i + 1) * 3.0;
    return v;
  };
  static const double pass[4] = {0.17, 0.86, 1.0, 1.0};
  auto seed_cost = [&](uint32_t budget_left, double verify) -> double {
    return 0.35 + pass[budget_left < 3 ? budget_left : 3] * verify;
  };
  for (uint32_t o = 0; o < 8; o++) {
    astar[o] = 15;
    if (o > m || o > nO) continue;
    const uint32_t M = m - o;
    double best = -1;
    for (uint32_t as = 0; as <= M + 1; as++) {
      double c = 0;
// ... 52 lines not shown
        continue;
      }
      uint32_t eb = 0;
      while (eb < 2 && j + eb + 1 <= m && mine(ax, o0 + eb + 1)) eb++;
      uint32_t steps[8], ns = 0, plast = 0;
      for (uint32_t t = 0; t < kp; t++)
        if ((mk >> t) & 1u) steps[ns++] = plast = t;
      uint32_t ndig = 1;
      for (uint32_t i = 0; i < j; i++) ndig *= 3;
      for (uint32_t dc = 0; dc < ndig; dc++) {
        uint32_t f[8], x = dc;
        for (uint32_t i = j; i-- > 0;) {
          f[i] = (steps[i] << 2) | (x % 3);
          x /= 3;
        }
        auto emit = [&](uint32_t e2, uint32_t e1, bool r, uint32_t rs) {
          uint32_t n = j;
          if (e2) f[n++] = ((k - 2) << 2) | (e2 - 1);
          if (e1) f[n++] = ((k - 1) << 2) | (e1 - 1);
          if (n > m || n > 7 || !mine(ax, o0 + (n - j))) return;
          if (no_xo && ax == 0u && n == m) return;
          out.push_back(recipe_word(n, 0, r, rs, f));
        };
        if (eb >= 2) {
          for (uint32_t e2 = 0; e2 < 4; e2++)
            for (uint32_t e1 = 0; e1 < 4; e1++) emit(e2, e1, false, 0);
        } else if (eb == 1) {
          for (uint32_t e1 = 0; e1 < 4; e1++) emit(0, e1, false, 0);
          for (uint32_t e2 = 1; e2 < 4; e2++) emit(e2, 0, rot && !pair8, k - 2);
        } else {
          emit(0, 0, rot && j >= 1, plast);
        }
      }
    }
}
static void build_recipes_b(std::vector<uint64_t> &out, uint32_t k, uint32_t L, uint32_t P, uint32_t m, uint32_t nX,
                            const uint32_t *astar, bool rot, bool deep) {
  const uint32_t nO = k - nX, nR = L - k, ylo = L - k, nY = L - nX, step0 = deep ? 0 : P, kd = deep ? nY : k;
  for (uint32_t o = 0; o <= m && o <= nO && o < 8; o++)
    for (uint32_t b = 0; b <= nR && astar[o] + o + b <= m; b++) {
      if (astar[o] > nX || o + b > 7) continue;
      const uint32_t jb = o + b;
      uint32_t ndig = 1;
      for (uint32_t i = 0; i < jb; i++) ndig *= 3;
      for (uint32_t mo = 0; mo < (1u << nO); mo++) {
        if ((uint32_t)__builtin_popcount(mo) != o) continue;
        for (uint32_t mr = 0; mr < (1u << nR); mr++) {
          if ((uint32_t)__builtin_popcount(mr) != b) continue;
          const uint32_t mk = (mo << ylo) | mr;
          uint32_t ys[8], ns = 0, ymax = 0;
          for (uint32_t y = 0; y < nY; y++)
            if ((mk >> y) & 1u) ys[ns++] = ymax = y;
          const uint32_t slast = step0 + ymax;
          const bool r = rot && !deep && jb >= 1 && slast + 2 <= kd;
          for (uint32_t dc = 0; dc < ndig; dc++) {
            uint32_t f[8], x = dc;
            for (uint32_t i = jb; i-- > 0;) {
              f[i] = (ys[i] << 2) | (x % 3);
              x /= 3;
            }
            out.push_back(recipe_word(jb, astar[o] > 7 ? 7u : astar[o], r, slast, f));
          }
        }
      }
    }
}
extern "C" gs_status gs_debug_seed_recipes(uint32_t k, uint32_t L, uint32_t P, uint32_t m, uint32_t n_x,
                                           const uint32_t *astar, uint32_t deep, uint64_t *out, uint64_t cap,
                                           uint64_t counts[3]) {
  if (k < 4 || k > 16 || L < k || L > 31 || m > 7 || n_x + 1 > k || !counts) return GS_ERR_ARG;
  try {
    std::vector<uint64_t> all;
    build_recipes_a(all, k, m, n_x, nullptr, true);
    counts[0] = all.size();
    counts[1] = counts[2] = 0;
    if (astar) {
      build_recipes_a(all, k, m, n_x, astar, true);
      counts[1] = all.size() - counts[0];
      build_recipes_b(all, k, L, P, m, n_x, astar, true, deep != 0);
      counts[2] = all.size() - counts[0] - counts[1];
    }
    for (uint64_t i = 0; i < all.size() && i < cap && out; i++) out[i] = all[i];
  } catch (const std::bad_alloc &) {
    return GS_ERR_NOMEM;
  }
  return GS_OK;
}
extern "C" gs_status gs_debug_seed_recipes_a8(uint32_t k, uint32_t m, uint32_t n_x, const uint32_t *astar, uint32_t trimmed, uint64_t *out,
                                              uint64_t cap, uint64_t *count) {
  if (k < 4 || k > 16 || m > 7 || n_x + 1 > k || !astar || !count) return GS_ERR_ARG;
  try {
    std::vector<uint64_t> all;
    build_recipes_a(all, k, m, n_x, astar, true, true, trimmed != 0);
    *count = all.size();
    for (uint64_t i = 0; i < all.size() && i < cap && out; i++) out[i] = all[i];
  } catch (const std::bad_alloc &) {
    return GS_ERR_NOMEM;
  }
  return GS_OK;
}
extern "C" void gs_debug_choose_thresholds(uint32_t m, uint32_t n_x, uint32_t n_o, uint32_t n_r, double pam_expansions,
                                           double verify_a, double verify_b, uint32_t astar[8]) {
  gs_choose_astar(m, n_x, n_o, n_r, pam_expansions, astar, verify_a, verify_b);
}

gs_status gs_recipes_for(gs_index *ix, uint32_t L, uint32_t P, uint32_t m, uint32_t v_rem, const uint32_t *astar,
                                bool deep, hipStream_t st) {
  const uint32_t k = ix->pt_k;
  const bool rot = true;
  uint64_t key[2] = {((uint64_t)L << 48) | ((uint64_t)P << 40) | ((uint64_t)m << 32) | ((uint64_t)k << 24) |
                         ((uint64_t)v_rem << 16) | (deep ? 4u : 0u) | (rot ? 2u : 0u) | (astar ? 1u : 0u),
                     0};
  if (astar)
    for (uint32_t o = 0; o < 8; o++) key[1] |= (uint64_t)(astar[o] > 15 ? 15u : astar[o]) << (4 * o);
  for (uint32_t i = 0; i < 2; i++)
    if (ix->rec[i].valid && ix->rec[i].key[0] == key[0] && ix->rec[i].key[1] == key[1]) {
      ix->rec_cur = i;
      return GS_OK;
    }
  std::vector<uint64_t> all;
  build_recipes_a(all, k, m, v_rem, nullptr, rot);
  const size_t n_full = all.size();
  size_t n_a = 0, n_b = 0;
  size_t n_a8 = 0;
  if (astar) {
    build_recipes_a(all, k, m, v_rem, astar, rot);
    n_a = all.size() - n_full;
    build_recipes_b(all, k, L, P, m, v_rem, astar, rot, deep);
    n_b = all.size() - n_full - n_a;
    build_recipes_a(all, k, m, v_rem, astar, rot, true);
    n_a8 = all.size() - n_full - n_a - n_b;
    if (m < 8 && astar[m] > 0) build_recipes_a(all, k, m, v_rem, astar, rot, true, true);
  }
  const size_t n_a8s = all.size() - n_full - n_a - n_b - n_a8;
  if (all.size() >= (1ull << 31)) {
    gs_set_error("seed plan too large for this mismatch budget");
    return GS_ERR_UNSUPPORTED;
  }
  const uint32_t slot = !ix->rec[ix->rec_cur].valid ? ix->rec_cur : ix->rec_cur ^ 1u;
  gs_recipe_set &R = ix->rec[slot];
  R.valid = false;
  gs_status rc = gs_reserve(R.buf, 8 * all.size() + 64);
  if (rc != GS_OK) return rc;
  GS_HIP(hipMemcpyAsync(R.buf.p, all.data(), 8 * all.size(), hipMemcpyHostToDevice, st));
  GS_HIP(hipStreamSynchronize(st));
  R.n_full = (uint32_t)n_full;
  R.n_a = (uint32_t)n_a;
  R.n_b = (uint32_t)n_b;
  R.n_a8 = (uint32_t)n_a8;
  R.n_a8s = (uint32_t)n_a8s;
  R.a_rot_first = 31;
  for (size_t i = n_full + n_a + n_b; i < n_full + n_a + n_b + n_a8; i++)
    if (all[i] & 64u) R.a_rot_first = std::min(R.a_rot_first, (uint32_t)(all[i] >> 7) & 31u);
  R.key[0] = key[0];
  R.key[1] = key[1];
  R.valid = true;
  ix->rec_cur = slot;
  if (gs_opt(ix, "GS_DEBUG"))
    fprintf(stderr, "[gs] seed recipes: %zu one-sided, %zu + %zu two-sided (%.1f MB)\n", n_full, n_a, n_b, 8e-6 * all.size());
  return GS_OK;
}
```

guidescan-cli_amd/csrc/gs_seed.hip:

```cpp
#include "gs_kernels.h"

#define SEED_VQ VQ_CAP
#define SEED_LDS (SEED_VQ + 32 + 24 + 6)

__device__ __forceinline__ uint32_t seed_xcc_id() {
  return (uint32_t)__builtin_amdgcn_s_getreg(20 | (0 << 6) | ((4 - 1) << 11)) & 7u;
}
template <typename T>
__device__ __forceinline__ const T *seed_sgprs(const T *p) {
  uint32_t lo = __builtin_amdgcn_readfirstlane((uint32_t)(uintptr_t)p);
  uint32_t hi = __builtin_amdgcn_readfirstlane((uint32_t)((uintptr_t)p >> 32));
  asm volatile("" : "+s"(lo), "+s"(hi));
  return (const T *)(const T __attribute__((address_space(1))) *)(((uint64_t)hi << 32) | lo);
}
__device__ __forceinline__ uint32_t seed_codes16(const uint32_t T, const uint32_t Q) {
  const uint32_t x = T ^ Q;
  const uint32_t ne = (x | (x >> 1)) & 0x55555555u;
  const uint32_t nq = ~T & Q;
  const uint32_t lt = ((nq >> 1) | ((~x >> 1) & nq)) & 0x55555555u;
  return (T + lt) & (ne * 3u);
}
__device__ __forceinline__ uint32_t seed_rev16(const uint32_t x) {
  const uint32_t r = __brev(x);
  return ((r >> 1) & 0x55555555u) | ((r & 0x55555555u) << 1);
}

struct gs_describe_shape {
  uint32_t L, P, k, x_len, n_pt;
  uint32_t code[2];
};
__host__ __device__ inline gs_guide_desc gs_describe_one(const gs_guide_rec &r, const gs_describe_shape &a, uint32_t g) {
  gs_guide_desc d;
  const uint64_t q = r.q;
  const uint32_t L = a.L, P = a.P, k = a.k, sx = a.x_len, nYb = L - sx;
  auto sym = [&](uint32_t t) -> uint32_t { return (uint32_t)(q >> (2u * t)) & 3u; };
  d.q_lo = (uint32_t)q;
  d.q_hi = (uint32_t)(q >> 32);
  for (uint32_t j = 0; j < 4; j++) d.pam[j] = r.pam[j];
  const uint32_t npams = r.valid ? (r.npams < 4u ? r.npams : 4u) : 0u;
  uint32_t pslots = 0, bits = 0;
  for (uint32_t pj = 0; pj < npams; pj++) {
    const uint32_t pw = r.pam[pj];
    const uint32_t c0 = (pw >> (3u * (P - 2u))) & 7u, c1 = (pw >> (3u * (P - 1u))) & 7u, cn = pw & 7u;
    const uint32_t code = c0 | (c1 << 2);
    const uint32_t bslot = (a.n_pt > 1u && code == a.code[1]) ? 1u : 0u;
    pslots |= 1u << bslot;
    bits |= bslot << (8u + pj);
    bits |= (cn == 4u ? 15u : 1u << (3u - cn)) << (12u + 4u * pj);
  }
  uint32_t bsel_z = 0, bsel_w = 0, n_bpairs = 0;
  for (uint32_t j = 0; j < 4u; ++j) {
    const uint32_t o = 2u * j;
    if (o + 1u < sx) {
      const uint32_t v = (3u - sym(sx - 1u - o)) | ((3u - sym(sx - 2u - o)) << 2);
      if (j < 2u)
        bsel_z |= 1u << (16u * j + v);
      else
        bsel_w |= 1u << (16u * (j - 2u) + v);
      n_bpairs++;
    }
  }
  d.meta = npams | (pslots << 3) | (n_bpairs << 5) | bits;
  uint32_t pidx0 = 0;
  for (uint32_t t = 0; t < k; ++t) pidx0 |= sym(t) << (2u * (k - 1u - t));
  d.pidx0 = pidx0;
  uint32_t pidxg = 0;
  for (uint32_t y = 0; y < nYb; ++y) pidxg |= (3u - sym(L - 1u - y)) << (2u * (nYb - 1u - y));
  d.pidxg = pidxg;
  uint32_t qrem_b = 0;
  for (uint32_t j = 0; j < sx; ++j) qrem_b |= (3u - sym(sx - 1u - j)) << (2u * j);
  d.qrem_b = qrem_b;
  d.bsel_z = bsel_z;
  d.bsel_w = bsel_w;
  const uint32_t gA = L - k, gmaskA = gA >= 16u ? 0xFFFFFFFFu : ((1u << (2u * gA)) - 1u);
  const uint32_t qremA = (uint32_t)(q >> (2u * k)) & gmaskA;
  uint32_t qhot = 0;
  for (uint32_t j = 0; j < 6u && j < gA; ++j) qhot |= 1u << (4u * j + ((qremA >> (2u * j)) & 3u));
  d.qhot = qhot;
  const uint32_t xa = sx < 8u ? sx : 8u, rb = (L - k) < 8u ? (L - k) : 8u;
  d.key_a = xa ? pidx0 >> (2u * (k - xa)) : 0u;
  d.key_b = (rb && rb <= nYb) ? pidxg >> (2u * (nYb - rb)) : 0u;
  d.guide = g;
  return d;
}
__global__ void k_describe(gs_describe_args a) {
  const uint32_t g = blockIdx.x * blockDim.x + threadIdx.x;
  if (g >= a.n) return;
  gs_describe_shape sh;
  sh.L = a.L;
  sh.P = a.P;
  sh.k = a.k;
  sh.x_len = a.x_len;
  sh.n_pt = a.n_pt;
  sh.code[0] = a.code[0];
  sh.code[1] = a.code[1];
  gs_guide_desc d = gs_describe_one(a.guides[g], sh, g);
  if ((d.meta & 7u) != 0u) {
    const uint64_t q = ((uint64_t)d.q_hi << 32) | d.q_lo, lmask = (1ull << (2u * a.L)) - 1ull;
    for (uint32_t s = 0; s < 2u; ++s) {
      bool any = false;
      const uint32_t nc = a.n_cand[s];
      if (a.cand_ids[s] != nullptr) {
        for (uint32_t sg = 0; sg < 4u && !any; ++sg) {
          const uint32_t *off = a.cand_off[s] + 1025u * sg + ((uint32_t)(q >> (10u * sg)) & 1023u);
          for (uint32_t c = off[0]; c < off[1] && !any; ++c) {
            const uint4 ce = a.cand[s][a.cand_ids[s][(size_t)sg * nc + c]];
            const uint64_t x = ((((uint64_t)ce.y << 32) | ce.x) ^ q);
            any = (uint32_t)__popcll((x | (x >> 1)) & 0x5555555555555555ull & lmask) <= a.m;
          }
        }
      } else {
        for (uint32_t c = 0; c < nc && !any; ++c) {
          const uint4 ce = a.cand[s][c];
          const uint64_t x = ((((uint64_t)ce.y << 32) | ce.x) ^ q);
          any = (uint32_t)__popcll((x | (x >> 1)) & 0x5555555555555555ull & lmask) <= a.m;
        }
      }
      if (any) d.meta |= 1u << (28u + s);
    }
  }
  a.desc[g] = d;
  if (a.hist != nullptr) {
    atomicAdd(&a.hist[d.key_a], 1u);
    atomicAdd(&a.hist[65536u + d.key_b], 1u);
  }
}
extern "C" gs_status gs_debug_guide_descriptor(uint64_t q, const uint32_t pam[4], uint32_t npams, uint32_t valid, uint32_t L, uint32_t P,
                                               uint32_t k, uint32_t x_len, uint32_t n_pt, const uint32_t code[2], uint32_t out[16]) {
  if (!pam || !code || !out || L < 1 || L > 31 || k < 4 || k > 16 || k > L || x_len < 1 || x_len >= L || P < 2 || P > 8) return GS_ERR_ARG;
  gs_guide_rec r;
  r.q = q;
  for (int j = 0; j < 4; j++) r.pam[j] = pam[j];
  r.npams = npams;
  r.valid = valid;
  gs_describe_shape sh;
  sh.L = L;
  sh.P = P;
  sh.k = k;
  sh.x_len = x_len;
  sh.n_pt = n_pt;
  sh.code[0] = code[0];
  sh.code[1] = code[1];
  const gs_guide_desc d = gs_describe_one(r, sh, 0u);
  static_assert(sizeof(gs_guide_desc) == 64, "one descriptor is sixteen words");
  memcpy(out, &d, 64);
  return GS_OK;
}
__global__ void __launch_bounds__(1024) k_sched_scan(uint32_t *hist) {
  __shared__ uint32_t part[1024];
  uint32_t *h = hist + 65536u * blockIdx.x;
  const uint32_t t = threadIdx.x;
  uint32_t s = 0;
  for (uint32_t i = 0; i < 64u; i++) s += h[64u * t + i];
  part[t] = s;
  __syncthreads();
  for (uint32_t o = 1; o < 1024u; o <<= 1) {
    const uint32_t v = t >= o ? part[t - o] : 0u;
    __syncthreads();
    part[t] += v;
    __syncthreads();
  }
  uint32_t run = part[t] - s;
  for (uint32_t i = 0; i < 64u; i++) {
    const uint32_t c = h[64u * t + i];
    h[64u * t + i] = run;
    run += c;
  }
}
__global__ void k_sched_scatter(const gs_guide_desc *desc, uint32_t n, uint32_t *cursor, gs_guide_desc *desc_a, gs_guide_desc *desc_b) {
  const uint32_t g = blockIdx.x * blockDim.x + threadIdx.x;
  if (g >= n) return;
  const gs_guide_desc d = desc[g];
  desc_a[atomicAdd(&cursor[d.key_a], 1u)] = d;
  desc_b[atomicAdd(&cursor[65536u + d.key_b], 1u)] = d;
}

__global__ void k_estimate_heavy(const gs_guide_rec *guides, uint32_t n, const uint4 *ptab0, const uint4 *ptab1, uint32_t k,
                                 uint32_t thresh, uint32_t *out) {
  const uint32_t g = blockIdx.x * blockDim.x + threadIdx.x;
  bool heavy = false;
  uint32_t most = 0;
  if (g < n && guides[g].valid) {
    const uint64_t q = guides[g].q;
    uint32_t pidx = 0;
    for (uint32_t t = 0; t < k; ++t) pidx |= ((uint32_t)(q >> (2u * t)) & 3u) << (2u * (k - 1u - t));
    const uint32_t c0 = ptab0[pidx].y & 0x7FFFFFFFu, c1 = ptab1[pidx].y & 0x7FFFFFFFu;
    heavy = c0 >= thresh || c1 >= thresh;
    most = c0 > c1 ? c0 : c1;
  }
  const uint64_t b = __ballot(heavy);
  if (b) {
    if (lane_id() == 0) atomicAdd(out, (uint32_t)__popcll(b));
    if (heavy) atomicMax(out + 1, most);
  }
}
gs_status gs_estimate_heavy(gs_index *ix, const gs_guide_rec *guides, uint32_t n, uint32_t thresh, uint32_t *d_out, hipStream_t st,
                            uint32_t n_heavy[2]) {
  n_heavy[0] = n_heavy[1] = 0;
  if (!ix->pt_k || !ix->strand[0].ptab || !ix->strand[1].ptab || !n) return GS_OK;
  GS_HIP(hipMemsetAsync(d_out, 0, 8, st));
  hipLaunchKernelGGL(k_estimate_heavy, dim3((n + 255) / 256), dim3(256), 0, st, guides, n, (const uint4 *)ix->strand[0].ptab,
                     (const uint4 *)ix->strand[1].ptab, ix->pt_k, thresh, d_out);
  GS_HIP(hipMemcpyAsync(n_heavy, d_out, 8, hipMemcpyDeviceToHost, st));
  GS_HIP(hipStreamSynchronize(st));
  return GS_OK;
}

template <bool CNT, int SIDE>
__device__ __forceinline__ void k_seed_body(const gs_search_args &a, uint4 *lds) {
  constexpr bool modeB = SIDE == 0;
  constexpr uint32_t PB = 7u, KSH = 61u, PSG = 50u + PB, PSP = 49u + PB;
  constexpr uint64_t PMASK = (1ull << (52u + PB)) - 1ull;
  const uint32_t lane = lane_id();
  uint4 *const vq = lds;
  uint2 *const own2 = (uint2 *)(vq + SEED_VQ);
  uint32_t *const own = (uint32_t *)own2;
  uint32_t *const dtab = (uint32_t *)(vq + SEED_VQ + 32);
  uint32_t *const wmisc = dtab + 96;
  const uint32_t L = a.L, P = a.P, m = a.m, k = a.pt_k, sx = a.x_len;
  const bool k_arena = a.arena != nullptr;
  const bool k_append = modeB ? a.append != 0u : true;
  const uint64_t *const k_slot_off = a.slot_off;
  const uint32_t k_cap = a.cap, n_items = a.n_items, ng = n_items >> 1;
  uint32_t *const xwork = a.xwork + (modeB ? 0u : 256u);
  unsigned long long n_ovf = 0;
  uint32_t n_fail = 0, n_hpass = 0, n_two = 0;
  bool bailed = false;
  uint32_t n_sp_items = 0, n_sp_rows = 0, n_sp_max = 0, n_sp_hits = 0;
  uint32_t c_tab = 0, c_c16 = 0, c_ctx = 0, c_isa = 0, c_rec = 0;
  auto count_lines = [&](uint32_t &acc, bool act, const void *p) __attribute__((always_inline)) {
    if constexpr (CNT) {
      const uint32_t line = (uint32_t)((uintptr_t)p >> a.cnt_shift);
      const uint32_t prev = (uint32_t)__shfl_up((int)line, 1);
      const int pact = __shfl_up((int)act, 1);
      const bool fresh = act && (lane == 0u || !pact || prev != line);
      acc += (uint32_t)__popcll(__ballot(fresh));
    }
  };
  if (lane == 0) {
    wmisc[16] = 0u;
    wmisc[17] = 0u;
    wmisc[18] = 1u;
  }
  __builtin_amdgcn_fence(__ATOMIC_RELEASE, "wavefront");

  const gs_guide_desc *const descs = modeB ? a.desc_b : a.desc_a;
  uint32_t cur = seed_xcc_id(), tried = 0;
  uint32_t item_next = 0, item_end = 0;
  uint32_t pend = 0xFFFFFFFFu;
  bool pending = false;
  for (;;) {
    if (item_next == item_end) {
      bool none = false;
      for (;;) {
        const uint32_t lo = (uint32_t)(((uint64_t)cur * n_items) >> 3), hi = (uint32_t)(((uint64_t)(cur + 1u) * n_items) >> 3);
        if (!pending) {
          pend = 0xFFFFFFFFu;
          if (lane == 0 && (tried == 0u || ld_agent(&xwork[32u * cur]) < hi - lo)) pend = atomicAdd(&xwork[32u * cur], a.take);
        }
        pending = false;
        const uint32_t base = __builtin_amdgcn_readfirstlane(pend);
        if (base < hi - lo) {
          item_next = lo + base;
          item_end = (hi - lo) - base < a.take ? hi : item_next + a.take;
          break;
        }
        cur = (cur + 1u) & 7u;
        if (++tried == 8u) {
          none = true;
          break;
        }
      }
      if (none) break;
    }
    const uint32_t pos = item_next++;
    if (item_next == item_end) {
      pend = 0xFFFFFFFFu;
      if (lane == 0) pend = atomicAdd(&xwork[32u * cur], a.take);
      pending = true;
    }
    const uint32_t strand = pos >= ng ? 1u : 0u;
    typedef uint32_t seed_u32x16 __attribute__((ext_vector_type(16)));
    const seed_u32x16 dp = *(const seed_u32x16 __attribute__((address_space(4))) *)(uintptr_t)(descs + (pos - strand * ng));
    const uint32_t guide = dp[15];
    const uint32_t slot = 2u * guide + strand;
    const uint32_t gw0 = dp[0], gw1 = dp[1];
    const uint64_t gr_q = ((uint64_t)gw1 << 32) | gw0;
    const uint32_t gr_pam0 = dp[2], gr_pam1 = dp[3], gr_pam2 = dp[4], gr_pam3 = dp[5];
    const uint32_t meta = dp[6];
    const uint32_t npams = meta & 7u;
    if (npams == 0u || bailed) {
      if (modeB && !a.append) {
        if (lane == 0) a.counts[slot] = 0;
        if (k_arena && lane < 8u) a.cls[(size_t)slot * 8u + lane] = 0u;
        if (k_arena && lane == 8u) a.nchunk[slot] = make_uint2(0u, 0u);
      }
      continue;
    }
    uint32_t guard_left = a.max_iter;
    const gs_strand_dev &sd = a.sd[strand];
    const gs_strand_dev &sv = a.sd[strand ^ 1u];
    uint4 *out = a.slots + (k_slot_off ? (size_t)k_slot_off[slot] : (size_t)slot * k_cap);
    const uint32_t item_cap = k_slot_off ? (uint32_t)(k_slot_off[slot + 1] - k_slot_off[slot]) : k_cap;
    uint32_t n_match = 0;
    if (k_append) n_match = __builtin_amdgcn_readfirstlane(a.counts[slot]);
    if (k_arena) {
      uint2 nc = make_uint2(0u, 0u);
      if (k_append) nc = a.nchunk[slot];
      if (lane < 3u) wmisc[lane] = lane == 0u ? nc.x : lane == 1u ? nc.y : 0u;
      if (lane >= 4u && lane < 12u) wmisc[lane] = k_append ? a.cls[(size_t)slot * 8u + (lane - 4u)] : 0u;
      __builtin_amdgcn_fence(__ATOMIC_RELEASE, "wavefront");
    }

    auto emit = [&](const bool em, const uint32_t row, const uint64_t cmeta, const uint32_t vflag) __attribute__((always_inline)) {
      const uint64_t be = __ballot(em);
      if (!be) return;
      const uint32_t hi = n_match + (uint32_t)__popcll(be);
      if (k_arena) {
        const uint32_t kk = (uint32_t)((cmeta >> KSH) & 7ull);
        uint32_t add = 0;
        for (uint32_t d = 0; d <= m; ++d) {
          const uint32_t c = (uint32_t)__popcll(__ballot(em && kk == d));
          add = lane == d ? c : add;
        }
        if (add) atomicAdd(&wmisc[4u + lane], add);
      }
      if (hi > item_cap && k_arena) {
        __builtin_amdgcn_fence(__ATOMIC_ACQUIRE, "wavefront");
        uint32_t nch = __builtin_amdgcn_readfirstlane(wmisc[0]);
        const uint32_t need = (hi - item_cap + ARENA_CHUNK - 1u) >> ARENA_SHIFT;
        while (nch < need) {
          uint32_t id = 0;
          if (lane == 0) {
            uint32_t rn = wmisc[16];
            if (rn == wmisc[17]) {
              const uint32_t g = wmisc[18];
              rn = atomicAdd(a.arena_next, g);
              wmisc[17] = rn + g;
              wmisc[18] = g < 16u ? 2u * g : 16u;
            }
            id = rn;
            wmisc[16] = rn + 1u;
          }
          id = __builtin_amdgcn_readfirstlane(id);
          if (id >= a.arena_chunks) break;
          if (lane == 0) {
            a.chunk_item[id] = slot;
            a.chunk_seq[id] = nch;
            wmisc[2] = wmisc[1];
            wmisc[1] = id;
          }
          nch++;
        }
        if (lane == 0) wmisc[0] = nch;
        __builtin_amdgcn_fence(__ATOMIC_RELEASE, "wavefront");
      }
      if (em) {
        const uint32_t idx = n_match + lanes_below(be);
        const uint64_t key = ((uint64_t)((cmeta >> KSH) & 7ull) << 61) | ((uint64_t)strand << 60) | ((cmeta & PMASK) << (8u - PB)) | vflag;
        const uint4 rec = make_uint4((uint32_t)key, (uint32_t)(key >> 32), row, row);
        if (idx < item_cap) {
          out[idx] = rec;
        } else if (k_arena) {
          __builtin_amdgcn_fence(__ATOMIC_ACQUIRE, "wavefront");
          const uint32_t e = idx - item_cap, sq = e >> ARENA_SHIFT;
          const uint32_t nch = wmisc[0];
          if (sq < nch) {
            const uint32_t id = sq + 1u == nch ? wmisc[1] : wmisc[2];
            a.arena[((size_t)id << ARENA_SHIFT) | (e & (ARENA_CHUNK - 1u))] = rec;
          }
        }
      }
      n_match = hi;
    };

    const uint2 *const recs = modeB ? a.rec_b : a.rec_a8;
    const uint32_t nrec = modeB ? a.n_rec_b : a.n_rec_a8;
    auto seed_path = [&](const uint32_t sid) __attribute__((always_inline)) -> uint64_t {
      const uint2 rc = recs[sid & 0xFFFFFFu];
      const uint32_t n = rc.x & 7u;
      uint64_t f = (((uint64_t)rc.y << 32) | rc.x) >> 12;
      uint64_t path = 0;
      for (uint32_t i = 0; i < n; ++i) {
        const uint32_t fld = (uint32_t)f & 127u, s = fld >> 2, d = fld & 3u;
        f >>= 7;
        const uint32_t t = modeB ? L - 1u - s : s;
        const uint32_t qc = (uint32_t)(gr_q >> (2u * t)) & 3u;
        const uint32_t sym = (qc + 1u + d) & 3u;
        path |= (uint64_t)(1u + sym - (sym > qc ? 1u : 0u)) << (PSG - 2u * t);
      }
      if (modeB) {
        const uint32_t bx = (sid >> 24) & 3u, pj = (sid >> 26) & 3u;
        const uint32_t pw = pj == 0 ? gr_pam0 : pj == 1 ? gr_pam1 : pj == 2 ? gr_pam2 : gr_pam3;
        path |= (uint64_t)(bx != 0u ? 3u - bx : 4u) << (PSP - 2u * L);
        for (uint32_t u = 1; u < P; ++u) path |= (uint64_t)(((pw >> (3u * u)) & 7u) < 3u ? ((pw >> (3u * u)) & 7u) : 4u) << (PSP - 2u * L - 3u * u);
      }
      return path;
    };

    const uint16_t *v16 = modeB ? seed_sgprs(sv.ctx16) : nullptr;
    const uint32_t *vctx = modeB ? seed_sgprs(sv.ctx) : nullptr;
    const uint32_t *arow = nullptr;
    const uint32_t g = modeB ? sx : L - k;
    const uint32_t gmask = g >= 16u ? 0xFFFFFFFFu : ((1u << (2u * g)) - 1u);
    const uint32_t qrem = modeB ? dp[9] : ((uint32_t)(gr_q >> (2u * k)) & gmask);

    constexpr uint32_t SEED_HAS_PATH = 0xFFFFFFFFu;
    auto resolve = [&](const bool on, const uint32_t e_x, const uint32_t e_y, const uint32_t w, const uint32_t e_w, const uint64_t given) __attribute__((always_inline)) {
      const uint32_t n = (uint32_t)__popcll(__ballot(on));
      struct {
        uint32_t x, w;
      } const e = {e_x, e_w};
      if constexpr (modeB) {
        uint64_t mmeta = 0;
        uint32_t rowA = 0;
        if (on) {
          const uint32_t pB = sv.sa[e.x];
          const uint64_t sp = seed_path(e_y);
          rowA = sd.isa[(sd.n - 1u) - (pB - g) - (L + P)];
          const uint64_t gpath = (uint64_t)seed_codes16(~w & gmask, ~qrem & gmask) << (52u + PB - 2u * g);
          mmeta = ((uint64_t)e.w << KSH) | sp | gpath;
        }
        if constexpr (CNT) c_isa += 2u * n;
        emit(on, rowA, mmeta, 0u);
      } else {
        uint32_t orow = 0;
        uint64_t base_meta = 0;
        if (on) {
          orow = arow[e.x];
          const uint64_t gpath = ((uint64_t)seed_rev16(seed_codes16(w & gmask, qrem)) << 32) >> (12u - PB + 2u * k);
          const uint64_t sp = e_y == SEED_HAS_PATH ? given : seed_path(e_y);
          base_meta = ((uint64_t)e.w << KSH) | sp | gpath;
        }
        if constexpr (CNT) c_isa += n;
        for (uint32_t pj = 0; pj < npams; ++pj) {
          const uint32_t pw = pj == 0 ? gr_pam0 : pj == 1 ? gr_pam1 : pj == 2 ? gr_pam2 : gr_pam3;
          bool ok = on;
          uint64_t ppath = 0;
          for (uint32_t u = 0; u < P; ++u) {
            const uint32_t pc = (pw >> (3u * u)) & 7u;
            const uint32_t tb = (w >> (2u * (g + u))) & 3u;
            ok = ok && (pc == 4u || pc == tb);
            ppath |= (uint64_t)(tb < 3u ? tb : 4u) << (PSP - 2u * L - 3u * u);
          }
          if (!__ballot(ok)) continue;
          emit(ok, orow, base_meta | ppath, 1u);
        }
      }
    };

    auto verify = [&](const uint32_t take, uint4 *dsrc) __attribute__((always_inline)) {
      __builtin_amdgcn_fence(__ATOMIC_ACQUIRE, "wavefront");
      uint4 mine = make_uint4(0u, 0u, 0u, 0u);
      if (lane < take) mine = dsrc[lane];
      const uint32_t vcnt = (mine.y >> 17) & 0x3FFu;
      const uint32_t vgrp = (vcnt + 7u) >> 3;
      const uint32_t incl = wave_incl_sum(vgrp);
      const uint32_t R = __builtin_amdgcn_readlane(incl, WAVE - 1);
      if (!R) return;
      const uint32_t excl = incl - vgrp;
      if (R >= a.share_min) n_hpass++;
      if (lane < take) dsrc[lane].y = mine.y | excl;
      const uint32_t g8 = g < 8u ? g : 8u;
      const uint32_t gm8 = (1u << (2u * g8)) - 1u;
      const uint32_t q2x = (qrem & gm8) * 0x00010001u, gm2x = gm8 * 0x00010001u;
      for (uint32_t base = 0; base < R; base += 2u * WAVE) {
        own2[lane] = make_uint2(0u, 0u);
        __builtin_amdgcn_fence(__ATOMIC_RELEASE, "wavefront");
        if (vgrp) {
          if (excl >= base && excl < base + 2u * WAVE) own[excl - base] = lane + 1u;
          if (excl < base && excl + vgrp > base) own[0] = lane + 1u;
        }
        __builtin_amdgcn_fence(__ATOMIC_RELEASE, "wavefront");
        __builtin_amdgcn_fence(__ATOMIC_ACQUIRE, "wavefront");
        const uint2 mk = own2[lane];
        uint32_t o0 = mk.x, o1 = mk.y > o0 ? mk.y : o0;
        const uint32_t run = wave_incl_max(o1);
        const uint32_t prev = dpp_or_zero<0x138>(run);
        o0 = o0 > prev ? o0 : prev;
        o1 = o1 > prev ? o1 : prev;
        const uint32_t ow[2] = {o0, o1};
        uint4 wq[2], dsc[2];
        uint32_t row0[2], nrow[2], kkv[2], okm[2];
#pragma unroll
        for (uint32_t jj = 0; jj < 2u; ++jj) {
          const uint32_t grp = base + 2u * lane + jj;
          const bool on = grp < R;
          dsc[jj] = make_uint4(0u, 0u, 0u, 0u);
          if (on) dsc[jj] = dsrc[ow[jj] - 1u];
          const uint32_t r0 = (grp - (dsc[jj].y & 0x3FFFu)) << 3;
          const uint32_t cnt = (dsc[jj].y >> 17) & 0x3FFu;
          row0[jj] = dsc[jj].x + r0;
          nrow[jj] = on ? (cnt - r0 < 8u ? cnt - r0 : 8u) : 0u;
          kkv[jj] = (dsc[jj].y >> 14) & 7u;
          const uint32_t lo = (dsc[jj].y >> DSC_LO) & 7u;
          const uint32_t lo8 = lo > g - g8 ? lo - (g - g8) : 0u;
          okm[jj] = on ? (((2u << (m - kkv[jj])) - 1u) & ~((1u << lo8) - 1u)) : 0u;
          wq[jj] = make_uint4(0u, 0u, 0u, 0u);
          if (on) wq[jj] = load16_a2(v16 + row0[jj]);
        }
        if constexpr (CNT) {
          const bool on0 = nrow[0] != 0u, on1 = nrow[1] != 0u;
          const uint32_t f0 = (uint32_t)((uintptr_t)(v16 + row0[0]) >> 6), l0 = (uint32_t)(((uintptr_t)(v16 + row0[0]) + 15u) >> 6);
          const uint32_t f1 = (uint32_t)((uintptr_t)(v16 + row0[1]) >> 6), l1 = (uint32_t)(((uintptr_t)(v16 + row0[1]) + 15u) >> 6);
          const uint32_t mylast = on1 ? l1 : l0;
          const uint32_t pl = (uint32_t)__shfl_up((int)mylast, 1);
          const int pact = __shfl_up((int)(on0 || on1), 1);
          uint32_t add = 0;
          if (on0) add += ((lane == 0u || !pact || pl != f0) ? 1u : 0u) + (l0 != f0 ? 1u : 0u);
          if (on1) add += ((!on0 || l0 != f1) ? 1u : 0u) + (l1 != f1 ? 1u : 0u);
          for (int o = 32; o > 0; o >>= 1) add += (uint32_t)__shfl_xor((int)add, o);
          c_c16 += add;
        }
        uint32_t cm = 0u;
#pragma unroll
        for (uint32_t jj = 0; jj < 2u; ++jj) {
          const uint32_t wv[4] = {wq[jj].x, wq[jj].y, wq[jj].z, wq[jj].w};
#pragma unroll
          for (uint32_t h = 0; h < 4u; ++h) {
            const uint32_t x = (wv[h] ^ q2x) & gm2x;
            const uint32_t y = (x | (x >> 1)) & 0x55555555u;
            const uint32_t m0 = __popc(y & 0xFFFFu), m1 = __popc(y >> 16);
            cm |= (((okm[jj] >> m0) & 1u) | (((okm[jj] >> m1) & 1u) << 1)) << (8u * jj + 2u * h);
          }
        }
        cm &= ((1u << nrow[0]) - 1u) | (((1u << nrow[1]) - 1u) << 8);
        while (__ballot(cm != 0u)) {
          const bool has = cm != 0u;
          const uint32_t pick = has ? (uint32_t)__builtin_ctz(cm) : 0u;
          cm &= cm - 1u;
          const bool hi = (pick >> 3) != 0u;
          const uint4 dd = hi ? dsc[1] : dsc[0];
          const uint32_t row = (hi ? row0[1] : row0[0]) + (pick & 7u);
          const uint32_t kv = hi ? kkv[1] : kkv[0];
          uint32_t w = 0u;
          if (has) w = vctx[row];
          if constexpr (CNT) c_ctx += (uint32_t)__popcll(__ballot(has));
          bool excbad = false;
          if constexpr (modeB) {
            const bool fl = has && ((dd.y >> DSC_EXC) & 1u) != 0u;
            if (__ballot(fl)) {
              if (fl) {
                uint32_t el = 0, eh = sv.n_exc;
                while (el < eh) {
                  const uint32_t mid = (el + eh) >> 1;
                  if (sv.exc_row[mid] < row)
                    el = mid + 1;
                  else
                    eh = mid;
                }
                if (el < sv.n_exc && sv.exc_row[el] == row) {
                  const uint64_t nb = sv.exc_sym[el];
                  for (uint32_t j = 0; j < g; ++j)
                    if (((uint32_t)(nb >> (4u * j)) & 15u) > 3u) excbad = true;
                }
              }
            }
          }
          const uint32_t xf = (w ^ qrem) & gmask;
          const uint32_t mmv = __popc((xf | (xf >> 1)) & 0x55555555u);
          const bool gok = has && !excbad && kv + mmv <= m && mmv >= ((dd.y >> DSC_LO) & 7u);
          const uint64_t bh = __ballot(gok);
          if (!bh) continue;
          resolve(gok, row, dd.z, w, kv + mmv, 0ull);
        }
      }
    };

    uint32_t qn = 0;
    const uint32_t v_max = a.v_max;
    auto queue_step = [&](uint32_t rem, uint32_t first, const uint32_t ymeta, const uint32_t sid, const bool drain_all) __attribute__((always_inline)) {
      for (;;) {
        if (guard_left == 0u) {
          bailed = true;
          break;
        }
        guard_left--;
        const uint64_t bq = __ballot(rem != 0u);
        if (bq && qn + WAVE <= SEED_VQ) {
          const uint32_t rows = rem < v_max ? rem : v_max;
          if (rem != 0u) {
            uint32_t *e = (uint32_t *)(vq + qn + lanes_below(bq));
            *(uint2 *)e = make_uint2(first, ymeta | (rows << 17));
            e[2] = sid;
          }
          qn += __popcll(bq);
          first += rows;
          rem -= rows;
          __builtin_amdgcn_fence(__ATOMIC_RELEASE, "wavefront");
          continue;
        }
        if (qn >= VQ_DRAIN || (bq && qn != 0u) || (drain_all && qn != 0u)) {
          const uint32_t take = qn < WAVE ? qn : WAVE;
          qn -= take;
          verify(take, vq + qn);
          continue;
        }
        break;
      }
    };
    auto fill_dtab = [&]() __attribute__((always_inline)) {
      const uint32_t nst = modeB ? L - sx : k;
      for (uint32_t e = lane; e < 4u * nst; e += WAVE) {
        const uint32_t s = e >> 2, d = e & 3u;
        const uint32_t t = modeB ? L - 1u - s : s;
        const uint32_t qc = (uint32_t)(gr_q >> (2u * t)) & 3u;
        const uint32_t sym = (qc + 1u + d) & 3u;
        dtab[e] = d == 3u ? 0u : (qc ^ sym) << (2u * (nst - 1u - s));
      }
      __builtin_amdgcn_fence(__ATOMIC_RELEASE, "wavefront");
      __builtin_amdgcn_fence(__ATOMIC_ACQUIRE, "wavefront");
    };
    auto apply_recipe = [&](const uint2 rc, uint32_t pidx) __attribute__((always_inline)) -> uint32_t {
      const uint32_t w0 = __builtin_amdgcn_alignbit(rc.y, rc.x, 12);
      pidx ^= dtab[w0 & 127u] ^ dtab[(w0 >> 7) & 127u] ^ dtab[(w0 >> 14) & 127u];
      if (m > 3u && __ballot((rc.x & 7u) > 3u) != 0ull) {
        const uint32_t w1 = rc.y >> 1;
        pidx ^= dtab[w1 & 127u] ^ dtab[(w1 >> 7) & 127u] ^ dtab[(w1 >> 14) & 127u] ^ dtab[(w1 >> 21) & 127u];
      }
      return pidx;
    };
    const uint32_t keep = (a.dbg_skip & 3u) ? 0u : 0xFFFFFFFFu;

    if constexpr (modeB) {
      {
        const uint32_t ncand = a.n_cand[strand];
        const uint64_t lmask = (1ull << (2u * L)) - 1ull;
        const uint32_t *cids = a.cand_ids[strand];
        const uint32_t nseg = !((meta >> (28u + strand)) & 1u) ? 0u : cids != nullptr ? 4u : 1u;
        for (uint32_t sg = 0; sg < nseg; ++sg) {
          uint32_t s0 = 0, s1 = ncand;
          if (cids != nullptr) {
            const uint32_t *off = a.cand_off[strand] + 1025u * sg + ((uint32_t)(gr_q >> (10u * sg)) & 1023u);
            s0 = __builtin_amdgcn_readfirstlane(off[0]);
            s1 = __builtin_amdgcn_readfirstlane(off[1]);
          }
          for (uint32_t c0 = s0; c0 < s1; c0 += WAVE) {
            bool in = c0 + lane < s1;
            uint4 ce = make_uint4(0u, 0u, 0u, 0u);
            if (in) ce = a.cand[strand][cids != nullptr ? cids[(size_t)sg * ncand + c0 + lane] : c0 + lane];
            const uint64_t cq = ((uint64_t)ce.y << 32) | ce.x;
            const uint64_t x = cq ^ gr_q;
            for (uint32_t e = 0; e < sg; ++e) in = in && ((uint32_t)(x >> (10u * e)) & 1023u) != 0u;
            const uint64_t nz = (x | (x >> 1)) & 0x5555555555555555ull & lmask;
            const uint32_t tot = __popcll(nz);
            const bool mine = in && tot <= m;
            if (!__ballot(mine)) continue;
            uint64_t gpath = 0;
            for (uint32_t t = 0; t < L; ++t) {
              const uint32_t qc = (uint32_t)(gr_q >> (2u * t)) & 3u, tb = (uint32_t)(cq >> (2u * t)) & 3u;
              const uint32_t code = tb == qc ? 0u : 1u + tb - (tb > qc ? 1u : 0u);
              gpath |= (uint64_t)code << (PSG - 2u * t);
            }
            uint32_t rowA = 0;
            if (mine) rowA = sd.isa[ce.w];
            if constexpr (CNT) c_isa += (uint32_t)__popcll(__ballot(mine));
            for (uint32_t pj = 0; pj < npams; ++pj) {
              const uint32_t pw = pj == 0 ? gr_pam0 : pj == 1 ? gr_pam1 : pj == 2 ? gr_pam2 : gr_pam3;
              bool ok = mine;
              uint64_t ppath = 0;
              for (uint32_t u = 0; u < P; ++u) {
                const uint32_t pc = (pw >> (3u * u)) & 7u, tb = (ce.z >> (3u * u)) & 7u;
                ok = ok && (tb == 4u ? pc == 4u : (pc == 4u || pc == tb));
                ppath |= (uint64_t)(tb == 4u ? 3u : (tb < 3u ? tb : 4u)) << (PSP - 2u * L - 3u * u);
              }
              emit(ok, rowA, ((uint64_t)tot << KSH) | gpath | ppath, 0u);
            }
          }
        }
      }
      const uint32_t pidxg = dp[8], bsel_z = dp[10], bsel_w = dp[11], n_bpairs = (meta >> 5) & 7u;
      const uint32_t nlanes = 4u * nrec;
      fill_dtab();
      uint2 rc_next = make_uint2(0u, 0u);
      if (lane < nlanes) rc_next = recs[lane >> 2];
      for (uint32_t bpj = 0; bpj < npams && !bailed; ++bpj) {
        const uint32_t bslot = (meta >> (8u + bpj)) & 1u, bxset = (meta >> (12u + 4u * bpj)) & 15u;
        const uint4 *bdeep = seed_sgprs(a.pt[bslot][strand ^ 1u].deep);
        for (uint32_t bc0 = 0; bc0 < nlanes; bc0 += WAVE) {
          const uint32_t idx = bc0 + lane, ri = idx >> 2, bx = idx & 3u;
          const bool act = idx < nlanes && ((bxset >> bx) & 1u) != 0u;
          const uint2 rc = rc_next;
          {
            const uint32_t nidx = (bc0 + WAVE >= nlanes ? 0u : bc0 + WAVE) + lane;
            rc_next = make_uint2(0u, 0u);
            if (nidx < nlanes) rc_next = recs[nidx >> 2];
          }
          count_lines(c_rec, idx < nlanes, recs + ri);
          const uint32_t jb = rc.x & 7u, lo = (rc.x >> 3) & 7u;
          const uint32_t pidx = apply_recipe(rc, pidxg);
          const uint4 *ep = bdeep + ((size_t)pidx << 2) + bx;
          uint4 ent = make_uint4(0u, 0u, 0u, 0u);
          if (act) ent = *ep;
          count_lines(c_tab, act, ep);
          const uint32_t need = n_bpairs > m - jb ? n_bpairs - (m - jb) : 0u;
          const uint32_t intact = (uint32_t)__popc(ent.z & bsel_z) + (uint32_t)__popc(ent.w & bsel_w);
          const uint32_t y = ((int32_t)ent.y < 0 || intact >= need) ? ent.y & keep : 0u;
          queue_step(y & 0x7FFFFFFFu, ent.x, (jb << 14) | (lo << DSC_LO) | ((y >> 31) << DSC_EXC), ri | (bx << 24) | (bpj << 26),
                     bc0 + WAVE >= nlanes && bpj + 1u == npams);
          if (bailed) break;
        }
      }
    } else {
      const uint32_t pidx0 = dp[7], qhot = dp[12];
      const uint32_t gmask13 = g >= 13u ? 0x3FFFFFFu : gmask;
      uint32_t pslots = (meta >> 3) & 3u;
      const uint32_t obits = 2u * (k - sx), omask = (1u << obits) - 1u;
      const uint32_t sp_key = a.spaced ? ((pidx0 >> obits) << (2u * g)) | qrem : 0u;
      uint2 sp_o0 = make_uint2(0u, 0u), sp_o1 = make_uint2(0u, 0u);
      if (a.spaced) {
        if (pslots & 1u) {
          const uint32_t *o = seed_sgprs(a.pt[0][strand].sp_off) + (sp_key >> a.pt[0][strand].sp_rem);
          sp_o0 = make_uint2(o[0], o[1]);
        }
        if (pslots & 2u) {
          const uint32_t *o = seed_sgprs(a.pt[1][strand].sp_off) + (sp_key >> a.pt[1][strand].sp_rem);
          sp_o1 = make_uint2(o[0], o[1]);
        }
        if constexpr (CNT) c_tab += (pslots & 1u) + (pslots >> 1);
      }
      fill_dtab();
      uint2 rc_ahead = make_uint2(0u, 0u);
      if (lane < nrec) rc_ahead = recs[lane];
      while (pslots != 0u && !bailed) {
        const uint32_t s = (pslots & 1u) ? 0u : 1u;
        pslots &= ~(1u << s);
        const gs_pairtab_dev &p = a.pt[s][strand];
        const uint2 *atab8 = seed_sgprs(p.tab), *arot8 = seed_sgprs(p.rot);
        const uint32_t arot_first = p.rot_first;
        v16 = seed_sgprs(p.c16);
        vctx = seed_sgprs(p.ctx);
        arow = seed_sgprs(p.rowid);
        for (uint32_t spos = 0; spos < nrec; spos += WAVE) {
          const uint32_t l = spos + lane;
          const bool act = l < nrec;
          const uint2 rc = rc_ahead;
          {
            const uint32_t nl = (spos + WAVE >= nrec ? 0u : spos + WAVE) + lane;
            rc_ahead = make_uint2(0u, 0u);
            if (nl < nrec) rc_ahead = recs[nl];
          }
          count_lines(c_rec, act, recs + l);
          const uint32_t kk = rc.x & 7u;
          const uint32_t pidx = apply_recipe(rc, pidx0);
          const uint2 *ep = atab8 + pidx;
          const uint32_t rs = (rc.x >> 7) & 31u;
          const bool rot = (rc.x & 64u) != 0u && rs >= arot_first;
          if (__ballot(rot) != 0ull) {
            if (rot) {
              const uint32_t sh = 2u * (k - 1u - rs);
              const uint32_t ridx = ((pidx >> (sh + 2u)) << (sh + 2u)) | ((pidx & ((1u << sh) - 1u)) << 2) | ((pidx >> sh) & 3u);
              ep = arot8 + (((size_t)(rs - arot_first) << (2u * k)) + ridx);
            }
          }
          uint2 e8 = make_uint2(0u, 0u);
          if (act) e8 = *ep;
          count_lines(c_tab, act, ep);
          uint32_t first = e8.x, ecnt = e8.y & 63u;
          const uint32_t filt = e8.y >> 6, bl = m - kk;
          const uint32_t xf = (filt ^ qrem) & gmask13;
          const uint32_t tw = ecnt == 1u ? ((xf | (xf >> 1)) & 0x55555555u) : (qhot & ~filt);
          const bool hopeless = (uint32_t)__popc(tw) > bl;
          if (__ballot(ecnt == GS_PT_BIG && !hopeless) != 0ull) {
            if (ecnt == GS_PT_BIG && !hopeless) {
              ecnt = arow[first];
              first += 1u;
            }
            if constexpr (CNT) c_isa += (uint32_t)__popcll(__ballot(true));
          }
          const uint32_t rem = hopeless ? 0u : ecnt & keep;
          queue_step(rem, first, kk << 14, l, spos + WAVE >= nrec);
          if (bailed) break;
        }
      }
      if (a.spaced) {
        pslots = (meta >> 3) & 3u;
        for (uint32_t s = 0; s < 2u && !bailed; ++s) {
          if (!((pslots >> s) & 1u)) continue;
          const gs_pairtab_dev &p = a.pt[s][strand];
          const uint32_t lo = __builtin_amdgcn_readfirstlane(s ? sp_o1.x : sp_o0.x), hi = __builtin_amdgcn_readfirstlane(s ? sp_o1.y : sp_o0.y);
          const uint32_t rem = p.sp_rem, remmask = (1u << rem) - 1u;
          const uint2 *sprows = seed_sgprs(p.sp_rows);
          vctx = seed_sgprs(p.ctx);
          arow = seed_sgprs(p.rowid);
          n_sp_items++;
          if (hi > lo) {
            n_sp_rows += hi - lo;
            n_sp_max = hi - lo > n_sp_max ? hi - lo : n_sp_max;
            if (((hi - lo) >> 3) >= a.share_min) n_hpass++;
          }
          for (uint32_t base = lo; base < hi; base += WAVE) {
            if (guard_left == 0u) {
              bailed = true;
              break;
            }
            guard_left--;
            const bool in = base + lane < hi;
            uint2 pr = make_uint2(0u, 0u);
            if (in) pr = sprows[base + lane];
            count_lines(c_ctx, in, sprows + base + lane);
            const uint32_t ox = ((pr.y >> rem) ^ pidx0) & omask;
            const bool hit = in && ((pr.y ^ sp_key) & remmask) == 0u && (uint32_t)__popc((ox | (ox >> 1)) & 0x55555555u) == m;
            const uint64_t bh = __ballot(hit);
            if (!bh) continue;
            uint32_t w = 0u;
            if (hit) w = vctx[pr.x];
            n_sp_hits += (uint32_t)__popcll(bh);
            if constexpr (CNT) c_isa += (uint32_t)__popcll(bh);
            const uint64_t opath = (uint64_t)seed_codes16((pr.y >> rem) & omask, pidx0 & omask) << (PSG + 2u - 2u * k);
            resolve(hit, pr.x, SEED_HAS_PATH, w, m, opath);
          }
        }
      }
      n_two++;
    }

    if (lane == 0) a.counts[slot] = n_match;
    if (!modeB && n_match > item_cap) n_ovf++;
    if (k_arena) {
      __builtin_amdgcn_fence(__ATOMIC_ACQUIRE, "wavefront");
      const uint32_t nch = __builtin_amdgcn_readfirstlane(wmisc[0]), last = __builtin_amdgcn_readfirstlane(wmisc[1]);
      if (lane == 0) a.nchunk[slot] = make_uint2(nch, last);
      if (lane < 8u) a.cls[(size_t)slot * 8u + lane] = wmisc[4u + lane];
      if (!modeB && n_match > item_cap && n_match - item_cap > (nch << ARENA_SHIFT)) n_fail++;
    }
  }
  if (lane == 0) {
    if (n_ovf) atomicAdd(&a.stats[1], n_ovf);
    if (n_fail) atomicAdd(&a.stats[6], (unsigned long long)n_fail);
    if (n_hpass) atomicAdd(a.hpass, n_hpass);
    if (bailed) atomicOr(a.err, 1u);
    if (n_sp_items) {
      atomicAdd(&a.spaced_ctr[0], n_sp_items);
      atomicAdd(&a.spaced_ctr[1], n_sp_rows);
      atomicMax(&a.spaced_ctr[2], n_sp_max);
      atomicAdd(&a.spaced_ctr[3], n_sp_hits);
    }
    if (n_two) {
      atomicAdd(&a.stats[4], (unsigned long long)n_two);
      atomicAdd(&a.stats[7], (unsigned long long)n_two);
    }
    if constexpr (CNT) {
      atomicAdd(&a.stats[8], (unsigned long long)c_tab);
      atomicAdd(&a.stats[9], (unsigned long long)c_c16);
      atomicAdd(&a.stats[10], (unsigned long long)c_ctx);
      atomicAdd(&a.stats[11], (unsigned long long)c_isa);
      atomicAdd(&a.stats[3], (unsigned long long)c_rec);
    }
  }
}

#define GS_DEF_SEED(NAME, CNT, SIDE)                                                                                \
  __global__ __launch_bounds__(WAVE *SEARCH_WAVES) __attribute__((amdgpu_waves_per_eu(GS_WAVES_EU_SEED, GS_WAVES_EU_SEED))) void NAME( \
      gs_search_args a) {                                                                                           \
    __shared__ uint4 s_lds[SEARCH_WAVES][SEED_LDS];                                                                 \
    k_seed_body<CNT, SIDE>(a, s_lds[threadIdx.x / WAVE]);                                                           \
  }
GS_DEF_SEED(k_seed_b, false, 0)
GS_DEF_SEED(k_seed_a, false, 1)
GS_DEF_SEED(k_seed_count_b, true, 0)
GS_DEF_SEED(k_seed_count_a, true, 1)

gs_status gs_seed_describe(gs_index *ix, const gs_search_args &sa, uint32_t ng, bool sorted, hipStream_t st, gs_search_args *out) {
  gs_status rc;
  if ((rc = gs_reserve(ix->w_desc, sizeof(gs_guide_desc) * ((size_t)ng + 1) * (sorted ? 3u : 1u))) != GS_OK) return rc;
  if ((rc = gs_reserve(ix->w_sched, 4 * (2 * 65536 + 512 + 16))) != GS_OK) return rc;
  uint32_t *base = (uint32_t *)ix->w_sched.p;
  uint32_t *xwork = base, *hist = base + 512;
  gs_guide_desc *desc = (gs_guide_desc *)ix->w_desc.p, *desc_a = desc + ng, *desc_b = desc_a + ng;
  gs_describe_args da;
  memset(&da, 0, sizeof(da));
  da.guides = sa.guides;
  da.desc = desc;
  da.n = ng;
  da.L = sa.L;
  da.P = sa.P;
  da.k = sa.pt_k;
  da.x_len = sa.x_len;
  da.n_pt = sa.n_pt;
  da.code[0] = sa.pt[0][0].code;
  da.code[1] = sa.n_pt > 1 ? sa.pt[1][0].code : 0xFFFFFFFFu;
  da.hist = sorted ? hist : nullptr;
  da.m = sa.m;
  for (uint32_t s = 0; s < 2; s++) {
    da.cand[s] = sa.cand[s];
    da.cand_off[s] = sa.cand_off[s];
    da.cand_ids[s] = sa.cand_ids[s];
    da.n_cand[s] = sa.n_cand[s];
  }
  if (sorted) GS_HIP(hipMemsetAsync(hist, 0, 4 * 2 * 65536, st));
  hipLaunchKernelGGL(k_describe, dim3((ng + 255) / 256), dim3(256), 0, st, da);
  if (sorted) {
    hipLaunchKernelGGL(k_sched_scan, dim3(2), dim3(1024), 0, st, hist);
    hipLaunchKernelGGL(k_sched_scatter, dim3((ng + 255) / 256), dim3(256), 0, st, (const gs_guide_desc *)desc, ng, hist, desc_a, desc_b);
  }
  *out = sa;
  out->desc_a = sorted ? desc_a : desc;
  out->desc_b = sorted ? desc_b : desc;
  out->xwork = xwork;
  return GS_OK;
}
gs_status gs_seed_launch(const gs_search_args &sa, uint32_t grid, bool count_req, hipStream_t st) {
  GS_HIP(hipMemsetAsync(sa.xwork, 0, 4 * 512, st));
  if (count_req) {
    hipLaunchKernelGGL(k_seed_count_b, dim3(grid), dim3(WAVE * SEARCH_WAVES), 0, st, sa);
    hipLaunchKernelGGL(k_seed_count_a, dim3(grid), dim3(WAVE * SEARCH_WAVES), 0, st, sa);
  } else {
    hipLaunchKernelGGL(k_seed_b, dim3(grid), dim3(WAVE * SEARCH_WAVES), 0, st, sa);
    hipLaunchKernelGGL(k_seed_a, dim3(grid), dim3(WAVE * SEARCH_WAVES), 0, st, sa);
  }
  return GS_OK;
}
```

include/guidescan_amd.h:

```cpp
#ifndef GUIDESCAN_AMD_H
#define GUIDESCAN_AMD_H

#include <stddef.h>
#include <stdint.h>

#ifdef __cplusplus
extern "C" {
#endif

typedef enum {
  GS_OK = 0,
  GS_ERR_ARG = 1,
  GS_ERR_DEVICE = 2,
  GS_ERR_UNSUPPORTED = 3,
  GS_ERR_NOMEM = 4,
  GS_ERR_IO = 5,
  GS_ERR_FORMAT = 6
} gs_status;

typedef struct gs_index gs_index;

typedef struct {
  int64_t pos;
  uint64_t key;
} gs_hit;

#define GS_KEY_MISMATCHES(key) ((uint32_t)((key) >> 61))
#define GS_KEY_INDEX(key) ((uint32_t)(((key) >> 60) & 1))

#define GS_FLAG_PAM_AT_START 1u
#define GS_FLAG_FAITHFUL_WALK 2u
#define GS_FLAG_COUNT_REQUESTS 4u
#define GS_FLAG_RAW_COUNTS 8u
#define GS_FLAG_NO_NEW_TABLES 16u

typedef struct {
  uint64_t n_guides;
  uint64_t n_hits;
  const uint64_t *guide_offsets;
  const gs_hit *hits;
  uint64_t n_ext;
  uint64_t n_matches;
  float ms_search;
  float ms_total;
  uint64_t n_unsupported;
  const uint8_t *guide_flags;
  const uint32_t *raw_hits;
} gs_result_view;
#define GS_GUIDE_NEEDS_GENERAL 1u

typedef struct gs_result gs_result;


gs_status gs_index_build(const uint8_t *text, uint64_t len, int device, gs_index **out);

gs_status gs_index_build_with_sa(const uint8_t *text, uint64_t len, const uint32_t *sa_fwd,
                                 const uint32_t *sa_rev, int device, gs_index **out);

gs_status gs_index_open_sdsl(const char *prefix, int device, gs_index **out);
gs_status gs_sdsl_extract_text(const char *index_file, uint8_t **text, uint64_t *len);

gs_status gs_index_save_sa(gs_index *ix, const uint8_t *text, uint64_t len, const char *path);
gs_status gs_index_save_sdsl(gs_index *ix, const uint8_t *text, uint64_t len, const char *prefix);
gs_status gs_debug_sdsl_sections(const uint64_t counts[256], uint8_t **tree, uint64_t *tree_len, uint8_t **alphabet,
                                 uint64_t *alphabet_len);
uint64_t gs_debug_sdsl_export_scratch(void);
gs_status gs_index_open_sa(const uint8_t *text, uint64_t len, const char *path, int device, gs_index **out);

void gs_index_close(gs_index *ix);
gs_status gs_index_last_counters(const gs_index *ix, uint64_t out[16]);
gs_status gs_index_last_launch(const gs_index *ix, uint64_t out[8]);
gs_status gs_index_last_spaced(const gs_index *ix, uint64_t out[6]);
gs_status gs_index_last_sharing(const gs_index *ix, uint64_t out[8]);
gs_status gs_index_set_option(gs_index *ix, const char *key, const char *value);
gs_status gs_index_get_option(const gs_index *ix, const char *key, char *out, uint64_t cap);
gs_status gs_index_lock(gs_index *ix);
gs_status gs_index_unlock(gs_index *ix);
uint64_t gs_index_genome_length(const gs_index *ix);
uint64_t gs_index_device_bytes(const gs_index *ix);


gs_status gs_enumerate(gs_index *ix, const char *guides, uint64_t n, uint32_t L,
                       const char *guide_pams, uint32_t P, const char *alt_pams, uint32_t n_alt,
                       uint32_t mismatches, uint32_t flags, gs_result **out);

gs_status gs_enumerate_device(gs_index *ix, const void *d_guides, uint64_t n, uint32_t L,
                              const void *d_guide_pams, uint32_t P, const char *alt_pams,
                              uint32_t n_alt, uint32_t mismatches, uint32_t flags, void *stream,
                              const void **d_offsets, const void **d_hits, gs_result_view *stats);
gs_status gs_index_prepare(gs_index *ix, uint64_t n, uint32_t L, const char *pam, uint32_t P, const char *alt_pams,
                           uint32_t n_alt, uint32_t mismatches, uint32_t flags);

gs_status gs_index_last_guide_flags(const gs_index *ix, const void **d_flags, uint64_t *n_unsupported);
gs_status gs_result_get(const gs_result *r, gs_result_view *view);
void gs_result_free(gs_result *r);

gs_status gs_decode_sequence(const char *guide, uint32_t L, uint32_t P, uint32_t flags,
                             uint64_t key, char *out);


gs_status gs_rank_bwt4(gs_index *ix, int strand, const uint64_t *rows, uint64_t n, uint64_t *out);
gs_status gs_resolve(gs_index *ix, int strand, const uint64_t *rows, uint64_t n, uint64_t *out);
gs_status gs_index_meta(const gs_index *ix, int strand, uint64_t C_acgtn[5], uint64_t *size);
gs_status gs_index_copy_sa(gs_index *ix, int strand, uint32_t *out);
gs_status gs_debug_seed_recipes(uint32_t k, uint32_t L, uint32_t P, uint32_t m, uint32_t n_x, const uint32_t *astar,
                                uint32_t deep, uint64_t *out, uint64_t cap, uint64_t counts[3]);
void gs_debug_choose_thresholds(uint32_t m, uint32_t n_x, uint32_t n_o, uint32_t n_r, double pam_expansions,
                                double verify_a, double verify_b, uint32_t astar[8]);
gs_status gs_debug_seed_recipes_a8(uint32_t k, uint32_t m, uint32_t n_x, const uint32_t *astar, uint32_t trimmed, uint64_t *out,
                                   uint64_t cap, uint64_t *count);
gs_status gs_debug_spaced_rows(gs_index *ix, uint32_t slot, int strand, uint32_t key, uint32_t *out, uint64_t cap, uint64_t *n,
                               uint32_t info[8]);
gs_status gs_debug_guide_descriptor(uint64_t q, const uint32_t pam[4], uint32_t npams, uint32_t valid, uint32_t L, uint32_t P,
                                    uint32_t k, uint32_t x_len, uint32_t n_pt, const uint32_t code[2], uint32_t out[16]);
void gs_debug_tile_plan(uint32_t records, uint32_t out[5]);
void gs_debug_search_form(const int64_t in[18], uint32_t out[6]);
gs_status gs_debug_general_last(const gs_index *ix, uint64_t out[8]);
gs_status gs_debug_bulge_last(const gs_index *ix, uint64_t out[8]);
typedef struct gs_bulge_seed {
  uint32_t index, state;
  uint8_t seq[32];
} gs_bulge_seed;
gs_status gs_debug_bulge_seeds(const char *guide, uint32_t L, uint32_t k, uint32_t mismatches, uint32_t rna_bulges,
                               uint32_t dna_bulges, uint32_t flags, uint32_t prefix_len, uint32_t prefix, gs_bulge_seed *out,
                               uint64_t cap, uint64_t *n);
typedef struct gs_bulge_match {
  uint32_t state, consumed;
  uint8_t seq[32];
} gs_bulge_match;
gs_status gs_debug_bulge_verify(uint32_t state, const uint8_t seq[32], uint64_t ctx_nibbles, const char *guide, uint32_t L,
                                const char *guide_pam, uint32_t P, const char *alt_pams, const uint32_t *alt_lens,
                                uint32_t n_alt, uint32_t k, uint32_t mismatches, uint32_t rna_bulges, uint32_t dna_bulges,
                                uint32_t flags, gs_bulge_match *out, uint64_t cap, uint64_t *n);

typedef struct {
  uint64_t rows;
  uint64_t not_permutation;
  uint64_t sampled;
  uint64_t out_of_order;
  uint64_t undecided;
  uint64_t bwt_mismatch;
} gs_sa_report;
gs_status gs_index_verify_sa(gs_index *ix, int strand, const uint8_t *text, uint64_t len,
                             uint64_t n_samples, uint64_t seed, gs_sa_report *report);
#define GS_VERIFY_ALL_ROWS (~0ull)


typedef struct {
  const char *const *chr_names;
  const uint64_t *chr_lengths;
  uint32_t n_chr;
} gs_genome_structure;

typedef struct {
  const char *id;
  const char *sequence;
  const char *pam;
  int sense_positive;
} gs_kmer;

#define GS_TEXT_SAM 0x100u
#define GS_TEXT_COMPLETE 0x200u
#define GS_TEXT_BAM 0x800u
#define GS_TEXT_BGZF 0x1000u

gs_status gs_format_guide(const gs_genome_structure *gs, const gs_kmer *k, const gs_hit *hits,
                          uint64_t n_hits, uint32_t mismatches, uint32_t flags,
                          int64_t max_off_targets, char **out_text, size_t *out_len);
gs_status gs_format_guide_scored(const gs_genome_structure *gs, const gs_kmer *k, const gs_hit *hits,
                                 uint64_t n_hits, uint32_t mismatches, uint32_t flags,
                                 int64_t max_off_targets, float specificity, char **out_text,
                                 size_t *out_len);
gs_status gs_format_guides_scored(const gs_genome_structure *gs, const gs_kmer *kmers, uint64_t n,
                                  const uint64_t *offsets, const gs_hit *hits, const float *specificity,
                                  const uint8_t *skip, uint32_t mismatches, uint32_t flags,
                                  int64_t max_off_targets, char **out_text, size_t *out_len);
gs_status gs_format_header(const gs_genome_structure *gs, uint32_t flags, char **out_text,
                           size_t *out_len);
void gs_free(void *p);


typedef struct {
  int64_t pos;
  char seq[32];
  uint32_t mismatches;
  uint8_t dna_bulges, rna_bulges;
  uint8_t index;
  uint8_t seq_len;
} gs_hit_ex;

typedef struct gs_result_ex gs_result_ex;

gs_status gs_enumerate_general(gs_index *ix, const char *guides, uint64_t n, uint32_t L,
                               const char *guide_pams, uint32_t P, const char *alt_pams, uint32_t n_alt,
                               uint32_t mismatches, uint32_t rna_bulges, uint32_t dna_bulges,
                               uint32_t flags, gs_result_ex **out);
gs_status gs_enumerate_general_pams(gs_index *ix, const char *guides, uint64_t n, uint32_t L,
                                    const char *guide_pams, uint32_t P, const char *alt_pams,
                                    const uint32_t *alt_lens, uint32_t n_alt, uint32_t mismatches,
                                    uint32_t rna_bulges, uint32_t dna_bulges, uint32_t flags, gs_result_ex **out);
gs_status gs_enumerate_bulges(gs_index *ix, const char *guides, uint64_t n, uint32_t L,
                              const char *guide_pams, uint32_t P, const char *alt_pams, uint32_t n_alt,
                              uint32_t mismatches, uint32_t rna_bulges, uint32_t dna_bulges,
                              uint32_t flags, gs_result_ex **out);
gs_status gs_result_ex_get(const gs_result_ex *r, uint64_t *n_guides, const uint64_t **guide_offsets,
                           const gs_hit_ex **hits);
gs_status gs_result_ex_raw_hits(const gs_result_ex *r, const uint32_t **raw_hits);
void gs_result_ex_free(gs_result_ex *r);
gs_status gs_decode_sequence_ex(const gs_hit_ex *hit, char *out);
gs_status gs_format_guide_ex(const gs_genome_structure *gs, const gs_kmer *k, const gs_hit_ex *hits,
                             uint64_t n_hits, uint32_t mismatches, uint32_t flags,
                             int64_t max_off_targets, char **out_text, size_t *out_len);

float gs_calculate_cfd(const char *sgrna, const char *match_sequence, const char *pam);


gs_status gs_score_device(gs_index *ix, const void *d_guides, uint64_t n, uint32_t L, uint32_t P,
                          uint32_t flags, int64_t max_off_targets, const gs_genome_structure *gs,
                          const void *d_offsets, const void *d_hits, void *stream, void *d_cfd,
                          void *d_specificity);
gs_status gs_score(gs_index *ix, const char *guides, uint64_t n, uint32_t L, uint32_t P, uint32_t flags,
                   int64_t max_off_targets, const gs_genome_structure *gs, const uint64_t *offsets,
                   const gs_hit *hits, float *cfd, float *specificity);


gs_status gs_format_device(gs_index *ix, const gs_genome_structure *gs, const void *d_guides, uint64_t n, uint32_t L,
                           const void *d_guide_pams, uint32_t P, const char *ids, const uint64_t *id_offsets,
                           const uint8_t *senses, const uint8_t *skip, const void *d_offsets, const void *d_hits,
                           const void *d_specificity, uint32_t mismatches, uint32_t flags, int64_t max_off_targets,
                           void *stream, const void **d_text, uint64_t *text_len);
gs_status gs_format_device_ids(gs_index *ix, const gs_genome_structure *gs, const void *d_guides, uint64_t n, uint32_t L,
                               const void *d_guide_pams, uint32_t P, const void *d_ids, const void *d_id_offsets,
                               const void *d_senses, const uint8_t *skip, const void *d_offsets, const void *d_hits,
                               const void *d_specificity, uint32_t mismatches, uint32_t flags, int64_t max_off_targets,
                               void *stream, const void **d_text, uint64_t *text_len);
gs_status gs_index_last_text_offsets(gs_index *ix, uint64_t *out, uint64_t n);
gs_status gs_enumerate_text(gs_index *ix, const char *guides, uint64_t n, uint32_t L, const char *guide_pams, uint32_t P,
                            const char *alt_pams, uint32_t n_alt, uint32_t mismatches, uint32_t flags,
                            int64_t max_off_targets, const gs_genome_structure *gs, const char *ids,
                            const uint64_t *id_offsets, const uint8_t *senses, const uint8_t *skip, char **text,
                            uint64_t *len, gs_result_view *stats);

gs_status gs_enumerate_text_device(gs_index *ix, const void *d_guides, uint64_t n, uint32_t L, const void *d_guide_pams,
                                   uint32_t P, const char *alt_pams, uint32_t n_alt, uint32_t mismatches, uint32_t flags,
                                   int64_t max_off_targets, const gs_genome_structure *gs, const void *d_ids,
                                   const void *d_id_offsets, const void *d_senses, const uint8_t *skip, char **text,
                                   uint64_t *len, gs_result_view *stats, uint32_t *raw_hits);


gs_status gs_bgzf_compress_device(gs_index *ix, const void *d_raw, uint64_t raw_len, void *stream, const void **d_out,
                                  uint64_t *out_len);
gs_status gs_bgzf_compress(gs_index *ix, const void *raw, uint64_t raw_len, uint8_t **out, uint64_t *out_len);
gs_status gs_debug_huffman_lengths(const uint32_t *freq, uint32_t n, uint32_t max_len, uint8_t *len);
float gs_debug_sp_float(uint32_t q);


typedef struct gs_kmers gs_kmers;

gs_status gs_kmers_generate(int device, const uint8_t *chr, uint64_t chr_len, int chr_on_device,
                            const char *pam, uint32_t k, uint32_t flags, void *stream, gs_kmers **out);
gs_status gs_kmers_get(gs_kmers *km, int on_device, uint64_t *n, const void **seqs, const void **pams,
                       const void **positions, const void **senses);
gs_status gs_kmers_encode_ids(gs_kmers *km, const char *prefix, const char *chr_name, void *stream);
// ... 104 lines not shown
```

Before: 63.43 million.

## Precompute seed recipe probes as XOR deltas and per-rotation table copies

Seed recipes are now converted on the host into compact probe words: an XOR delta on the pair-table index plus packed metadata. Rotation handling is folded into the delta and a small per-wave LDS table of base pointers and rotated guide indices. This removes the per-lane dtab lookups, the ballot-guarded rotation index math and the dtab fill from the seed kernel, and adds one-step deeper prefetch of probes and table entries. The cost is extra device buffers, host-side probe generation with synchronous copies when recipes or rotation settings change, and more complex index bookkeeping.

```diff
diff --git a/guidescan-cli_amd/api.py b/guidescan-cli_amd/api.py
--- a/guidescan-cli_amd/api.py
+++ b/guidescan-cli_amd/api.py
@@ -327,6 +327,7 @@
            "gs_kmers_concat", "gs_decoder_open", "gs_decoder_close", "gs_decode_records", "gs_decode_records_device",
            "gs_decode_sam", "gs_debug_repr_doubles", "gs_debug_decode_tables",
            "gs_index_last_spaced", "gs_debug_seed_recipes_a8", "gs_debug_spaced_rows",
+           "gs_debug_seed_probes", "gs_debug_seed_path", "gs_debug_rot_index",
            "gs_debug_bulge_last", "gs_debug_bulge_seeds", "gs_debug_bulge_verify",
            "gs_bgzf_compress_device", "gs_bgzf_compress", "gs_debug_huffman_lengths", "gs_debug_sp_float",
            "gs_bgzf_inflate", "gs_bgzf_inflate_device", "gs_bgzf_inflate_base", "gs_debug_inflate_member", "gs_debug_bgzf_members",
@@ -414,6 +415,37 @@
     out = np.zeros(int(n.value), dtype=np.uint64)
     _check(L_.gs_debug_seed_recipes_a8(k, m, n_x, a, 1 if trimmed else 0, out.ctypes.data, out.shape[0], C.byref(n)))
     return out
+
+
+def seed_probes(k, L, P, m, n_x, astar, side, rot_first=31):
+    L_ = lib()
+    L_.gs_debug_seed_probes.restype = C.c_int
+    L_.gs_debug_seed_probes.argtypes = [C.c_uint32] * 5 + [C.c_void_p, C.c_uint32, C.c_uint32, C.c_void_p, C.c_uint64, C.c_void_p]
+    a = (C.c_uint32 * 8)(*(list(astar) + [15] * 8)[:8])
+    n = C.c_uint64()
+    _check(L_.gs_debug_seed_probes(k, L, P, m, n_x, a, side, rot_first, None, 0, C.byref(n)))
+    out = np.zeros((int(n.value), 2), dtype=np.uint32)
+    _check(L_.gs_debug_seed_probes(k, L, P, m, n_x, a, side, rot_first, out.ctypes.data, out.shape[0], C.byref(n)))
+    return out
+
+
+def seed_path(q: int, word: int, L: int, P: int, nst: int, side_b: bool = False, sid: int = 0, pams=(0, 0, 0, 0)):
+    L_ = lib()
+    L_.gs_debug_seed_path.restype = C.c_int
+    L_.gs_debug_seed_path.argtypes = [C.c_uint64, C.c_void_p, C.c_uint64] + [C.c_uint32] * 5 + [C.c_void_p]
+    pam = (C.c_uint32 * 4)(*(list(pams) + [0] * 4)[:4])
+    out = (C.c_uint64 * 2)()
+    _check(L_.gs_debug_seed_path(q, pam, int(word), sid, 1 if side_b else 0, L, P, nst, out))
+    return int(out[0]), int(out[1])
+
+
+def rot_index(pidx: int, k: int, rs: int) -> int:
+    L_ = lib()
+    L_.gs_debug_rot_index.restype = C.c_int
+    L_.gs_debug_rot_index.argtypes = [C.c_uint32] * 3 + [C.c_void_p]
+    out = C.c_uint32()
+    _check(L_.gs_debug_rot_index(pidx, k, rs, C.byref(out)))
+    return int(out.value)
 
 
 def guide_descriptor(q: int, pams, L: int, P: int, k: int, x_len: int, codes=(0, 0xFFFFFFFF), n_pt: int = 1, valid: bool = True):
diff --git a/guidescan-cli_amd/csrc/gs_common.h b/guidescan-cli_amd/csrc/gs_common.h
--- a/guidescan-cli_amd/csrc/gs_common.h
+++ b/guidescan-cli_amd/csrc/gs_common.h
@@ -104,6 +104,13 @@
   uint32_t n_full = 0, n_a = 0, n_b = 0, n_a8 = 0;
   uint32_t n_a8s = 0;
   uint32_t a_rot_first = 31;
+  gs_buffer prb_b;
+  struct {
+    gs_buffer buf;
+    uint32_t rot_first = 31;
+    bool valid = false;
+  } prb_a[2];
+  std::vector<uint64_t> host_ba;
 };
 
 struct gs_index {
diff --git a/guidescan-cli_amd/csrc/gs_enumerate.hip b/guidescan-cli_amd/csrc/gs_enumerate.hip
--- a/guidescan-cli_amd/csrc/gs_enumerate.hip
+++ b/guidescan-cli_amd/csrc/gs_enumerate.hip
@@ -777,6 +777,7 @@
       gs_status r2 = gs_seed_describe(ix, sa, p.ng, k.f.seed_form >= 2u && p.ng >= b.sw.seed_sort_from, st, &sb);
       sb.seed_opt = b.sw.seed_opt;
       sb.take = b.sw.seed_take;
+      if (r2 == GS_OK) r2 = gs_probes_attach(ix, sb, st);
       if (r2 == GS_OK) r2 = gs_seed_launch(sb, k.seed_grid, b.count_req, st);
       if (r2 != GS_OK) return r2;
     } else if (k.spec)
@@ -936,7 +937,7 @@
   const uint32_t *d_shctl = sa.shq_ctl;
   k.seed_grid = 0;
   if (k.f.seed_form) {
-    const size_t lds_seed = sizeof(uint4) * (VQ_CAP + 32 + 24 + 6) * SEARCH_WAVES;
+    const size_t lds_seed = sizeof(uint4) * SEED_LDS * SEARCH_WAVES;
     k.seed_grid = (uint32_t)b.cus * std::min<uint32_t>((uint32_t)(160u * 1024u / lds_seed), GS_WAVES_EU_SEED);
     if (k.seed_grid > need) k.seed_grid = need;
   }
diff --git a/guidescan-cli_amd/csrc/gs_index.hip b/guidescan-cli_amd/csrc/gs_index.hip
--- a/guidescan-cli_amd/csrc/gs_index.hip
+++ b/guidescan-cli_amd/csrc/gs_index.hip
@@ -896,7 +896,8 @@
                        &ix->w_nhits2, &ix->w_h_off, &ix->w_h_tmp, &ix->w_b_src, &ix->w_b_cnt, &ix->w_b_prefix,
                        &ix->w_b_recs, &ix->w_b_w0, &ix->w_b_w0b, &ix->w_b_idx, &ix->w_b_idxb,
                        &ix->w_b_keep, &ix->w_b_keeps, &ix->w_b_rows, &ix->w_b_rowss, &ix->w_b_redo_pos, &ix->w_b_s, &ix->w_b_tab,
-                       &ix->w_cand, &ix->rec[0].buf, &ix->rec[1].buf, &ix->w_score, &ix->w_score_io, &ix->w_score_tmp, &ix->w_arena, &ix->w_arena_meta, &ix->w_nchunk, &ix->w_shq, &ix->w_sh_meta,
+                       &ix->w_cand, &ix->rec[0].buf, &ix->rec[1].buf, &ix->rec[0].prb_b, &ix->rec[1].prb_b, &ix->rec[0].prb_a[0].buf, &ix->rec[0].prb_a[1].buf,
+                       &ix->rec[1].prb_a[0].buf, &ix->rec[1].prb_a[1].buf, &ix->w_score, &ix->w_score_io, &ix->w_score_tmp, &ix->w_arena, &ix->w_arena_meta, &ix->w_nchunk, &ix->w_shq, &ix->w_sh_meta,
                        &ix->w_cls, &ix->w_desc, &ix->w_sched, &ix->w_t_plan, &ix->w_t_tiles, &ix->w_t_buckets, &ix->w_t_chunkof, &ix->w_t_big, &ix->w_t_rel, &ix->w_t_tab, &ix->w_t_excl, &ix->w_t_spill, &ix->w_b_redo_pos2,
                        &ix->w_text_in, &ix->w_text_tmp, &ix->w_text_hex, &ix->w_text, &ix->w_text_spec, &ix->w_text_goff,
                        &ix->w_bgzf_in, &ix->w_bgzf_tmp, &ix->w_bgzf_out};
diff --git a/guidescan-cli_amd/csrc/gs_kernels.h b/guidescan-cli_amd/csrc/gs_kernels.h
--- a/guidescan-cli_amd/csrc/gs_kernels.h
+++ b/guidescan-cli_amd/csrc/gs_kernels.h
@@ -68,6 +68,7 @@
   uint32_t n_rec_full, n_rec_a, n_rec_b;
   const uint2 *rec_a8;
   uint32_t n_rec_a8;
+  const uint2 *prb_b, *prb_a[2];
   gs_pairtab_dev pt[2][2];
   uint32_t n_pt;
   uint32_t bdeep, x_len;
@@ -143,6 +144,60 @@
 #define DSC_LO 27u
 #define DSC_EXC 30u
 
+#define SEED_VQ VQ_CAP
+#define SEED_COPIES 16u
+#define SEED_LDS (SEED_VQ + 32 + SEED_COPIES + 6)
+#define SEED_PB 7u
+#define SEED_PSG (50u + SEED_PB)
+#define SEED_PSP (49u + SEED_PB)
+__host__ __device__ inline uint32_t gs_recipe_delta(const uint64_t w, const uint32_t nst) {
+  uint32_t delta = 0;
+  uint64_t f = w >> 12;
+  for (uint32_t i = 0; i < 7u; ++i) {
+    const uint32_t fld = (uint32_t)f & 127u, s = fld >> 2, d = fld & 3u;
+    f >>= 7;
+    if (s < nst) delta ^= ((d + 1u) & 3u) << (2u * (nst - 1u - s));
+  }
+  return delta;
+}
+__host__ __device__ inline uint32_t gs_rot_index(const uint32_t pidx, const uint32_t k, const uint32_t rs) {
+  const uint32_t sh = 2u * (k - 1u - rs);
+  const uint32_t top = sh + 2u >= 32u ? 0u : (pidx >> (sh + 2u)) << (sh + 2u);
+  return top | ((pidx & ((1u << sh) - 1u)) << 2) | ((pidx >> sh) & 3u);
+}
+__host__ __device__ inline uint2 gs_probe_b(const uint64_t w, const uint32_t nst) {
+  const uint32_t jb = (uint32_t)w & 7u, lo = (uint32_t)(w >> 3) & 7u;
+  return make_uint2(gs_recipe_delta(w, nst), (jb << 14) | (lo << DSC_LO) | jb);
+}
+__host__ __device__ inline uint2 gs_probe_a(const uint64_t w, const uint32_t k, const uint32_t rot_first) {
+  const uint32_t kk = (uint32_t)w & 7u, rs = (uint32_t)(w >> 7) & 31u;
+  const bool rot = ((uint32_t)w & 64u) != 0u && rs >= rot_first && rs + 2u < k;
+  const uint32_t delta = gs_recipe_delta(w, k);
+  return make_uint2(rot ? gs_rot_index(delta, k, rs) : delta, (kk << 14) | ((rot ? rs - rot_first + 1u : 0u) << 4) | kk);
+}
+__host__ __device__ inline uint64_t gs_seed_path(const uint64_t w, const uint32_t sid, const bool side_b, const uint64_t q, const uint32_t L,
+                                                 const uint32_t P, const uint32_t pam0, const uint32_t pam1, const uint32_t pam2,
+                                                 const uint32_t pam3) {
+  const uint32_t n = (uint32_t)w & 7u;
+  uint64_t f = w >> 12;
+  uint64_t path = 0;
+  for (uint32_t i = 0; i < n; ++i) {
+    const uint32_t fld = (uint32_t)f & 127u, s = fld >> 2, d = fld & 3u;
+    f >>= 7;
+    const uint32_t t = side_b ? L - 1u - s : s;
+    const uint32_t qc = (uint32_t)(q >> (2u * t)) & 3u;
+    const uint32_t sym = qc ^ ((d + 1u) & 3u);
+    path |= (uint64_t)(1u + sym - (sym > qc ? 1u : 0u)) << (SEED_PSG - 2u * t);
+  }
+  if (side_b) {
+    const uint32_t bx = (sid >> 24) & 3u, pj = (sid >> 26) & 3u;
+    const uint32_t pw = pj == 0 ? pam0 : pj == 1 ? pam1 : pj == 2 ? pam2 : pam3;
+    path |= (uint64_t)(bx != 0u ? 3u - bx : 4u) << (SEED_PSP - 2u * L);
+    for (uint32_t u = 1; u < P; ++u) path |= (uint64_t)(((pw >> (3u * u)) & 7u) < 3u ? ((pw >> (3u * u)) & 7u) : 4u) << (SEED_PSP - 2u * L - 3u * u);
+  }
+  return path;
+}
+
 #define VERIFY_MAX_DEFAULT 1023u
 #define DTAB 88u
 
@@ -359,3 +414,4 @@
                      double verify_b = 1.9);
 gs_status gs_recipes_for(gs_index *ix, uint32_t L, uint32_t P, uint32_t m, uint32_t v_rem, const uint32_t *astar, bool deep,
                          hipStream_t st);
+gs_status gs_probes_attach(gs_index *ix, gs_search_args &sa, hipStream_t st);
diff --git a/guidescan-cli_amd/csrc/gs_recipes.hip b/guidescan-cli_amd/csrc/gs_recipes.hip
--- a/guidescan-cli_amd/csrc/gs_recipes.hip
+++ b/guidescan-cli_amd/csrc/gs_recipes.hip
@@ -228,6 +228,15 @@
   R.a_rot_first = 31;
   for (size_t i = n_full + n_a + n_b; i < n_full + n_a + n_b + n_a8; i++)
     if (all[i] & 64u) R.a_rot_first = std::min(R.a_rot_first, (uint32_t)(all[i] >> 7) & 31u);
+  R.host_ba.assign(all.begin() + (n_full + n_a), all.end());
+  for (auto &pa : R.prb_a) pa.valid = false;
+  if (n_b) {
+    std::vector<uint2> pb(n_b);
+    for (size_t i = 0; i < n_b; i++) pb[i] = gs_probe_b(R.host_ba[i], L - v_rem);
+    if ((rc = gs_reserve(R.prb_b, 8 * n_b + 64)) != GS_OK) return rc;
+    GS_HIP(hipMemcpyAsync(R.prb_b.p, pb.data(), 8 * n_b, hipMemcpyHostToDevice, st));
+    GS_HIP(hipStreamSynchronize(st));
+  }
   R.key[0] = key[0];
   R.key[1] = key[1];
   R.valid = true;
@@ -236,3 +245,71 @@
     fprintf(stderr, "[gs] seed recipes: %zu one-sided, %zu + %zu two-sided (%.1f MB)\n", n_full, n_a, n_b, 8e-6 * all.size());
   return GS_OK;
 }
+
+gs_status gs_probes_attach(gs_index *ix, gs_search_args &sa, hipStream_t st) {
+  gs_recipe_set &R = ix->rec[ix->rec_cur];
+  sa.prb_b = nullptr;
+  sa.prb_a[0] = sa.prb_a[1] = nullptr;
+  if (!R.valid || !sa.bidir || R.host_ba.size() != (size_t)R.n_b + R.n_a8 + R.n_a8s) return GS_ERR_ARG;
+  const uint2 *a8 = (const uint2 *)R.buf.p + R.n_full + R.n_a + R.n_b;
+  const size_t off = sa.rec_a8 == a8 ? 0 : R.n_a8;
+  if (sa.rec_a8 != a8 + off || sa.rec_b != a8 - R.n_b) return GS_ERR_ARG;
+  sa.prb_b = (const uint2 *)R.prb_b.p;
+  const size_t n_a = (size_t)R.n_a8 + R.n_a8s;
+  int used = -1;
+  for (uint32_t i = 0; i < sa.n_pt && i < 2u; i++) {
+    const uint32_t rf = sa.pt[i][0].rot_first;
+    if (sa.pt[i][1].rot_first != rf) return GS_ERR_ARG;
+    int e = -1;
+    for (int j = 0; j < 2; j++)
+      if (R.prb_a[j].valid && R.prb_a[j].rot_first == rf) e = j;
+    if (e < 0) {
+      e = used == 0 ? 1 : used == 1 ? 0 : !R.prb_a[0].valid ? 0 : !R.prb_a[1].valid ? 1 : 0;
+      std::vector<uint2> pa(n_a);
+      for (size_t r = 0; r < n_a; r++) pa[r] = gs_probe_a(R.host_ba[R.n_b + r], sa.pt_k, rf);
+      R.prb_a[e].valid = false;
+      const gs_status rc = gs_reserve(R.prb_a[e].buf, 8 * n_a + 64);
+      if (rc != GS_OK) return rc;
+      GS_HIP(hipMemcpyAsync(R.prb_a[e].buf.p, pa.data(), 8 * n_a, hipMemcpyHostToDevice, st));
+      GS_HIP(hipStreamSynchronize(st));
+      R.prb_a[e].rot_first = rf;
+      R.prb_a[e].valid = true;
+    }
+    used = e;
+    sa.prb_a[i] = (const uint2 *)R.prb_a[e].buf.p + off;
+  }
+  return GS_OK;
+}
+
+extern "C" gs_status gs_debug_seed_probes(uint32_t k, uint32_t L, uint32_t P, uint32_t m, uint32_t n_x, const uint32_t *astar, uint32_t side,
+                                          uint32_t rot_first, uint32_t *out, uint64_t cap, uint64_t *count) {
+  if (k < 4 || k > 16 || L < k || L > 31 || m > 7 || n_x + 1 > k || !astar || !count || side > 2) return GS_ERR_ARG;
+  try {
+    std::vector<uint64_t> all;
+    if (side == 0)
+      build_recipes_b(all, k, L, P, m, n_x, astar, true, true);
+    else
+      build_recipes_a(all, k, m, n_x, astar, true, true, side == 2);
+    *count = all.size();
+    for (uint64_t i = 0; i < all.size() && i < cap && out; i++) {
+      const uint2 p = side == 0 ? gs_probe_b(all[i], L - n_x) : gs_probe_a(all[i], k, rot_first);
+      out[2 * i] = p.x;
+      out[2 * i + 1] = p.y;
+    }
+  } catch (const std::bad_alloc &) {
+    return GS_ERR_NOMEM;
+  }
+  return GS_OK;
+}
+extern "C" gs_status gs_debug_seed_path(uint64_t q, const uint32_t pam[4], uint64_t word, uint32_t sid, uint32_t side_b, uint32_t L, uint32_t P,
+                                        uint32_t nst, uint64_t out[2]) {
+  if (!pam || !out || L < 1 || L > 31 || P > 8 || nst < 1 || nst > 16) return GS_ERR_ARG;
+  out[0] = gs_seed_path(word, sid, side_b != 0, q, L, P, pam[0], pam[1], pam[2], pam[3]);
+  out[1] = gs_recipe_delta(word, nst);
+  return GS_OK;
+}
+extern "C" gs_status gs_debug_rot_index(uint32_t pidx, uint32_t k, uint32_t rs, uint32_t *out) {
+  if (!out || k < 2 || k > 16 || rs + 1 > k) return GS_ERR_ARG;
+  *out = gs_rot_index(pidx, k, rs);
+  return GS_OK;
+}
diff --git a/guidescan-cli_amd/csrc/gs_seed.hip b/guidescan-cli_amd/csrc/gs_seed.hip
--- a/guidescan-cli_amd/csrc/gs_seed.hip
+++ b/guidescan-cli_amd/csrc/gs_seed.hip
@@ -1,7 +1,4 @@
 #include "gs_kernels.h"
-
-#define SEED_VQ VQ_CAP
-#define SEED_LDS (SEED_VQ + 32 + 24 + 6)
 
 __device__ __forceinline__ uint32_t seed_xcc_id() {
   return (uint32_t)__builtin_amdgcn_s_getreg(20 | (0 << 6) | ((4 - 1) << 11)) & 7u;
@@ -209,14 +206,14 @@
 template <bool CNT, int SIDE>
 __device__ __forceinline__ void k_seed_body(const gs_search_args &a, uint4 *lds) {
   constexpr bool modeB = SIDE == 0;
-  constexpr uint32_t PB = 7u, KSH = 61u, PSG = 50u + PB, PSP = 49u + PB;
+  constexpr uint32_t PB = SEED_PB, KSH = 61u, PSG = SEED_PSG, PSP = SEED_PSP;
   constexpr uint64_t PMASK = (1ull << (52u + PB)) - 1ull;
   const uint32_t lane = lane_id();
   uint4 *const vq = lds;
   uint2 *const own2 = (uint2 *)(vq + SEED_VQ);
   uint32_t *const own = (uint32_t *)own2;
-  uint32_t *const dtab = (uint32_t *)(vq + SEED_VQ + 32);
-  uint32_t *const wmisc = dtab + 96;
+  uint4 *const ctab = vq + SEED_VQ + 32;
+  uint32_t *const wmisc = (uint32_t *)(ctab + SEED_COPIES);
   const uint32_t L = a.L, P = a.P, m = a.m, k = a.pt_k, sx = a.x_len;
   const bool k_arena = a.arena != nullptr;
   const bool k_append = modeB ? a.append != 0u : true;
@@ -378,24 +375,7 @@
     const uint32_t nrec = modeB ? a.n_rec_b : a.n_rec_a8;
     auto seed_path = [&](const uint32_t sid) __attribute__((always_inline)) -> uint64_t {
       const uint2 rc = recs[sid & 0xFFFFFFu];
-      const uint32_t n = rc.x & 7u;
-      uint64_t f = (((uint64_t)rc.y << 32) | rc.x) >> 12;
-      uint64_t path = 0;
-      for (uint32_t i = 0; i < n; ++i) {
-        const uint32_t fld = (uint32_t)f & 127u, s = fld >> 2, d = fld & 3u;
-        f >>= 7;
-        const uint32_t t = modeB ? L - 1u - s : s;
-        const uint32_t qc = (uint32_t)(gr_q >> (2u * t)) & 3u;
-        const uint32_t sym = (qc + 1u + d) & 3u;
-        path |= (uint64_t)(1u + sym - (sym > qc ? 1u : 0u)) << (PSG - 2u * t);
-      }
-      if (modeB) {
-        const uint32_t bx = (sid >> 24) & 3u, pj = (sid >> 26) & 3u;
-        const uint32_t pw = pj == 0 ? gr_pam0 : pj == 1 ? gr_pam1 : pj == 2 ? gr_pam2 : gr_pam3;
-        path |= (uint64_t)(bx != 0u ? 3u - bx : 4u) << (PSP - 2u * L);
-        for (uint32_t u = 1; u < P; ++u) path |= (uint64_t)(((pw >> (3u * u)) & 7u) < 3u ? ((pw >> (3u * u)) & 7u) : 4u) << (PSP - 2u * L - 3u * u);
-      }
-      return path;
+      return gs_seed_path(((uint64_t)rc.y << 32) | rc.x, sid, modeB, gr_q, L, P, gr_pam0, gr_pam1, gr_pam2, gr_pam3);
     };
 
     const uint16_t *v16 = modeB ? seed_sgprs(sv.ctx16) : nullptr;
@@ -599,27 +579,6 @@
         break;
       }
     };
-    auto fill_dtab = [&]() __attribute__((always_inline)) {
-      const uint32_t nst = modeB ? L - sx : k;
-      for (uint32_t e = lane; e < 4u * nst; e += WAVE) {
-        const uint32_t s = e >> 2, d = e & 3u;
-        const uint32_t t = modeB ? L - 1u - s : s;
-        const uint32_t qc = (uint32_t)(gr_q >> (2u * t)) & 3u;
-        const uint32_t sym = (qc + 1u + d) & 3u;
-        dtab[e] = d == 3u ? 0u : (qc ^ sym) << (2u * (nst - 1u - s));
-      }
-      __builtin_amdgcn_fence(__ATOMIC_RELEASE, "wavefront");
-      __builtin_amdgcn_fence(__ATOMIC_ACQUIRE, "wavefront");
-    };
-    auto apply_recipe = [&](const uint2 rc, uint32_t pidx) __attribute__((always_inline)) -> uint32_t {
-      const uint32_t w0 = __builtin_amdgcn_alignbit(rc.y, rc.x, 12);
-      pidx ^= dtab[w0 & 127u] ^ dtab[(w0 >> 7) & 127u] ^ dtab[(w0 >> 14) & 127u];
-      if (m > 3u && __ballot((rc.x & 7u) > 3u) != 0ull) {
-        const uint32_t w1 = rc.y >> 1;
-        pidx ^= dtab[w1 & 127u] ^ dtab[(w1 >> 7) & 127u] ^ dtab[(w1 >> 14) & 127u] ^ dtab[(w1 >> 21) & 127u];
-      }
-      return pidx;
-    };
     const uint32_t keep = (a.dbg_skip & 3u) ? 0u : 0xFFFFFFFFu;
 
     if constexpr (modeB) {
@@ -671,9 +630,9 @@
       }
       const uint32_t pidxg = dp[8], bsel_z = dp[10], bsel_w = dp[11], n_bpairs = (meta >> 5) & 7u;
       const uint32_t nlanes = 4u * nrec;
-      fill_dtab();
+      const uint2 *const prb = seed_sgprs(a.prb_b);
       uint2 rc_next = make_uint2(0u, 0u);
-      if (lane < nlanes) rc_next = recs[lane >> 2];
+      if (lane < nlanes) rc_next = prb[lane >> 2];
       for (uint32_t bpj = 0; bpj < npams && !bailed; ++bpj) {
         const uint32_t bslot = (meta >> (8u + bpj)) & 1u, bxset = (meta >> (12u + 4u * bpj)) & 15u;
         const uint4 *bdeep = seed_sgprs(a.pt[bslot][strand ^ 1u].deep);
@@ -684,11 +643,11 @@
           {
             const uint32_t nidx = (bc0 + WAVE >= nlanes ? 0u : bc0 + WAVE) + lane;
             rc_next = make_uint2(0u, 0u);
-            if (nidx < nlanes) rc_next = recs[nidx >> 2];
-          }
-          count_lines(c_rec, idx < nlanes, recs + ri);
-          const uint32_t jb = rc.x & 7u, lo = (rc.x >> 3) & 7u;
-          const uint32_t pidx = apply_recipe(rc, pidxg);
+            if (nidx < nlanes) rc_next = prb[nidx >> 2];
+          }
+          count_lines(c_rec, idx < nlanes, prb + ri);
+          const uint32_t jb = rc.y & 7u;
+          const uint32_t pidx = pidxg ^ rc.x;
           const uint4 *ep = bdeep + ((size_t)pidx << 2) + bx;
           uint4 ent = make_uint4(0u, 0u, 0u, 0u);
           if (act) ent = *ep;
@@ -696,7 +655,7 @@
           const uint32_t need = n_bpairs > m - jb ? n_bpairs - (m - jb) : 0u;
           const uint32_t intact = (uint32_t)__popc(ent.z & bsel_z) + (uint32_t)__popc(ent.w & bsel_w);
           const uint32_t y = ((int32_t)ent.y < 0 || intact >= need) ? ent.y & keep : 0u;
-          queue_step(y & 0x7FFFFFFFu, ent.x, (jb << 14) | (lo << DSC_LO) | ((y >> 31) << DSC_EXC), ri | (bx << 24) | (bpj << 26),
+          queue_step(y & 0x7FFFFFFFu, ent.x, (rc.y & ~7u) | ((y >> 31) << DSC_EXC), ri | (bx << 24) | (bpj << 26),
                      bc0 + WAVE >= nlanes && bpj + 1u == npams);
           if (bailed) break;
         }
@@ -719,43 +678,65 @@
         }
         if constexpr (CNT) c_tab += (pslots & 1u) + (pslots >> 1);
       }
-      fill_dtab();
-      uint2 rc_ahead = make_uint2(0u, 0u);
-      if (lane < nrec) rc_ahead = recs[lane];
+      auto step_after = [&](const uint32_t p0) __attribute__((always_inline)) -> uint32_t { return p0 + WAVE >= nrec ? 0u : p0 + WAVE; };
+      auto probe_of = [&](const uint2 *const list, const uint32_t p0) __attribute__((always_inline)) -> uint2 {
+        uint2 r = make_uint2(0u, 0u);
+        if (p0 + lane < nrec) r = list[p0 + lane];
+        return r;
+      };
+      uint2 rc_n1, rc_n2;
+      {
+        const uint2 *const first_list = seed_sgprs(a.prb_a[(pslots & 1u) ? 0u : 1u]);
+        rc_n1 = probe_of(first_list, 0u);
+        rc_n2 = probe_of(nrec > WAVE || pslots != 3u ? first_list : seed_sgprs(a.prb_a[1]), step_after(0u));
+      }
       while (pslots != 0u && !bailed) {
         const uint32_t s = (pslots & 1u) ? 0u : 1u;
         pslots &= ~(1u << s);
         const gs_pairtab_dev &p = a.pt[s][strand];
-        const uint2 *atab8 = seed_sgprs(p.tab), *arot8 = seed_sgprs(p.rot);
-        const uint32_t arot_first = p.rot_first;
+        const uint2 *const prb = seed_sgprs(a.prb_a[s]);
+        const uint2 *const prb_after = pslots != 0u ? seed_sgprs(a.prb_a[1]) : prb;
+        {
+          const uint32_t arot_first = p.rot_first;
+          const uint32_t ncopy = arot_first + 2u < k ? k - 1u - arot_first : 1u;
+          if (lane < ncopy && lane < SEED_COPIES) {
+            const uint2 *base = p.tab;
+            uint32_t pi = pidx0;
+            if (lane != 0u) {
+              base = p.rot + ((size_t)(lane - 1u) << (2u * k));
+              pi = gs_rot_index(pidx0, k, arot_first + lane - 1u);
+            }
+            ctab[lane] = make_uint4((uint32_t)(uintptr_t)base, (uint32_t)((uintptr_t)base >> 32), pi, 0u);
+          }
+          __builtin_amdgcn_fence(__ATOMIC_RELEASE, "wavefront");
+          __builtin_amdgcn_fence(__ATOMIC_ACQUIRE, "wavefront");
+        }
         v16 = seed_sgprs(p.c16);
         vctx = seed_sgprs(p.ctx);
         arow = seed_sgprs(p.rowid);
-        for (uint32_t spos = 0; spos < nrec; spos += WAVE) {
-          const uint32_t l = spos + lane;
-          const bool act = l < nrec;
-          const uint2 rc = rc_ahead;
-          {
-            const uint32_t nl = (spos + WAVE >= nrec ? 0u : spos + WAVE) + lane;
-            rc_ahead = make_uint2(0u, 0u);
-            if (nl < nrec) rc_ahead = recs[nl];
-          }
-          count_lines(c_rec, act, recs + l);
-          const uint32_t kk = rc.x & 7u;
-          const uint32_t pidx = apply_recipe(rc, pidx0);
-          const uint2 *ep = atab8 + pidx;
-          const uint32_t rs = (rc.x >> 7) & 31u;
-          const bool rot = (rc.x & 64u) != 0u && rs >= arot_first;
-          if (__ballot(rot) != 0ull) {
-            if (rot) {
-              const uint32_t sh = 2u * (k - 1u - rs);
-              const uint32_t ridx = ((pidx >> (sh + 2u)) << (sh + 2u)) | ((pidx & ((1u << sh) - 1u)) << 2) | ((pidx >> sh) & 3u);
-              ep = arot8 + (((size_t)(rs - arot_first) << (2u * k)) + ridx);
-            }
-          }
+        auto entry_of = [&](const uint32_t p0, const uint2 pr) __attribute__((always_inline)) -> uint2 {
+          const bool act = p0 + lane < nrec;
+          const uint4 cp = *(const uint4 *)((const char *)ctab + (pr.y & 0xF0u));
+          const uint2 *ep = (const uint2 *)(const uint2 __attribute__((address_space(1))) *)(((uint64_t)cp.y << 32) | cp.x) + (cp.z ^ pr.x);
           uint2 e8 = make_uint2(0u, 0u);
           if (act) e8 = *ep;
           count_lines(c_tab, act, ep);
+          return e8;
+        };
+        uint2 e8_n1 = entry_of(0u, rc_n1);
+        for (uint32_t spos = 0; spos < nrec; spos += WAVE) {
+          const uint32_t l = spos + lane;
+          const bool act = l < nrec, last = spos + WAVE >= nrec;
+          const uint32_t ry = rc_n1.y;
+          const uint2 e8 = e8_n1;
+          rc_n1 = rc_n2;
+          if (!last) e8_n1 = entry_of(spos + WAVE, rc_n1);
+          {
+            const uint32_t s1 = step_after(spos), s2 = step_after(s1);
+            rc_n2 = probe_of(last || s2 < s1 ? prb_after : prb, s2);
+          }
+          count_lines(c_rec, act, prb + l);
+          const uint32_t kk = ry & 7u;
           uint32_t first = e8.x, ecnt = e8.y & 63u;
           const uint32_t filt = e8.y >> 6, bl = m - kk;
           const uint32_t xf = (filt ^ qrem) & gmask13;
@@ -769,7 +750,7 @@
             if constexpr (CNT) c_isa += (uint32_t)__popcll(__ballot(true));
           }
           const uint32_t rem = hopeless ? 0u : ecnt & keep;
-          queue_step(rem, first, kk << 14, l, spos + WAVE >= nrec);
+          queue_step(rem, first, ry & (7u << 14), l, last);
           if (bailed) break;
         }
       }
diff --git a/include/guidescan_amd.h b/include/guidescan_amd.h
--- a/include/guidescan_amd.h
+++ b/include/guidescan_amd.h
@@ -109,6 +109,11 @@
                                 double verify_a, double verify_b, uint32_t astar[8]);
 gs_status gs_debug_seed_recipes_a8(uint32_t k, uint32_t m, uint32_t n_x, const uint32_t *astar, uint32_t trimmed, uint64_t *out,
                                    uint64_t cap, uint64_t *count);
+gs_status gs_debug_seed_probes(uint32_t k, uint32_t L, uint32_t P, uint32_t m, uint32_t n_x, const uint32_t *astar, uint32_t side,
+                               uint32_t rot_first, uint32_t *out, uint64_t cap, uint64_t *count);
+gs_status gs_debug_seed_path(uint64_t q, const uint32_t pam[4], uint64_t word, uint32_t sid, uint32_t side_b, uint32_t L, uint32_t P,
+                             uint32_t nst, uint64_t out[2]);
+gs_status gs_debug_rot_index(uint32_t pidx, uint32_t k, uint32_t rs, uint32_t *out);
 gs_status gs_debug_spaced_rows(gs_index *ix, uint32_t slot, int strand, uint32_t key, uint32_t *out, uint64_t cap, uint64_t *n,
                                uint32_t info[8]);
 gs_status gs_debug_guide_descriptor(uint64_t q, const uint32_t pam[4], uint32_t npams, uint32_t valid, uint32_t L, uint32_t P,
```

Result: faster. 64.83 million (median of 6 runs) (+2.2%).
